# AssemblyAI-Community/MinImagen

Measured on AMD Instinct MI355X. Metric: denoising-steps/sec (images/sec x T), base 64^2 + SR 64->256 cascade, higher is better.
Workload: dtype f32; 1 GPU; cascade64_256: unet_0 params @64x64 + unet_1 params (lowres_cond) @256x256, T=100/stage, cond_scale=3.0 (2 U-Net evals/step), dynamic thresholding 0.9, fp32 storage / accumulate / softmax / statistics, contractions as 3-term fp16-split (hi*hi + hi*lo + lo*hi) MFMA products; per_gpu_batch=32, global_batch=32, parallelism=dp1

## Files before the change

include/minimagen_hip.h:

```cpp
#ifndef MINIMAGEN_HIP_H
#define MINIMAGEN_HIP_H

#include <stdint.h>

#ifdef __cplusplus
extern "C" {
#endif

#define MI_ABI_VERSION 12

enum mi_status {
    MI_OK = 0,
    MI_ERR_INVALID = -1,
    MI_ERR_LAUNCH = -2,
    MI_ERR_UNSUPPORTED = -3
};

int mi_abi_version(void);
const char* mi_last_error(void);
const char* mi_backend(void);
int mi_struct_size(int which);

typedef struct mi_act {
    const float* data;
    int C;
    const double* stats;
    int nt;
    float scale;
    int bmod;
    int st;
} mi_act;

typedef struct mi_conv_params {
    int B, H, W;
    mi_act in0, in1;
    int Cout;
    int ksize, stride, up2;
    const float* w;
    const float* bias;
    int gn_groups;
    const float* gn_gamma;
    const float* gn_beta;
    float gn_eps;
    const float* scale_shift;
    int ss_stride, ss_off;
    mi_act res0, res1;
    const float* res_w;
    const float* res_b;
    float* out;
    int out_st;
    double* out_stats;
    int tile_cfg;
    const void* w_rp;
    const void* res_w_rp;
    int w_rp_exp, res_w_rp_exp;
    float* gn_coef;
    int* gn_exps;
    void* act_prep; long long act_prep_bytes;
} mi_conv_params;
#define MI_CONV_SPLIT16 0x100
#define MI_CONV_SPLIT8  0x800
#define MI_CONV_HALF    0x400
#define MI_CONV_REVERSE 0x200
#define MI_CONV_RP_FIRST 6

int mi_conv_tile_shape(int tile_cfg, int* th, int* tw);
int mi_conv_stripe_rows(const mi_conv_params* p);
int mi_conv_prep_fwd(const mi_conv_params* p, void* stream);
long long mi_conv_prep_bytes(int B, int Cin, int Cres, int H, int W);
int mi_conv_cout_tile(int Cout);
int mi_conv_fwd(const mi_conv_params* p, void* stream);
int mi_gn_coef_fwd(const mi_conv_params* p, void* stream);

typedef struct mi_crossembed_params {
    int B, H, W;
    const float* in0; int C0;
    const float* in1; int C1;
    int in1_batch_mod;
    int in0_batch_mod;
    int n_kernels;
    int ksize[3];
    int cout[3];
    const float* w[3];
    const float* bias[3];
    float* out; double* out_stats;
    int out_st;
    int tile_cfg;
    const float* addend;
    const void* w_mfma;
    int w_mfma_exp[3];
} mi_crossembed_params;
int mi_crossembed_fwd(const mi_crossembed_params* p, void* stream);

typedef struct mi_init_down_params {
    int B, H, W;
    const float* in0; int C0;
    const float* in1; int C1;
    int in0_batch_mod;
    int n_kernels;
    int ksize[3];
    int cout[3];
    int Cout;
    const void* w_tab;
    int w_exp;
    const float* bias9;
    float* out; double* out_stats;
    int out_st;
    int tile_cfg;
    const float* addend;
} mi_init_down_params;
int mi_init_down_tiles(int tile_cfg, int H, int W);
int mi_init_down_fwd(const mi_init_down_params* p, void* stream);

typedef struct mi_linear {
    const float* w; const float* b; int in, out;
} mi_linear;

typedef struct mi_text_cond_params {
    int B2, B, L, E, cd, tcd, max_len;
    const float* text_embeds;
    const uint8_t* text_mask;
    const uint8_t* keep;
    mi_linear text_to_cond;
    const float* null_text_embed;
    const float* ln_w; const float* ln_b;
    mi_linear h1, h2;
    const float* null_text_hidden;
    const float* norm_w; const float* norm_b;
    float* c_text;
    float* text_hiddens;
} mi_text_cond_params;
int mi_text_cond_fwd(const mi_text_cond_params* p, void* stream);

typedef struct mi_cond_step_params {
    int B2, B, dim, cd, tcd, ntok;
    const int64_t* time;
    const int64_t* lowres_time;
    const float* freq;
    mi_linear th, tc, tt;
    mi_linear lth, ltc, ltt;
    const float* text_hiddens;
    const float* norm_w; const float* norm_b;
    mi_linear time_mlps;
    float* ss;
    float* c_time;
    float* t_out;
    float* silu_out;
} mi_cond_step_params;
int mi_cond_step_fwd(const mi_cond_step_params* p, void* stream);

#define MI_ATTN_MAX_BLOCKS 8
typedef struct mi_attn_fold_params {
    int B2, C, cd, heads, JT;
    const float* c_rows;
    int c_stride_b;
    int row0, nrows;
    int write_null;
    int frag_f16;
    int n_blocks;
    struct {
        const float* mg;
        const float* mv;
        const float* g0;
        const float* v0;
        float* gv;
        float* table;
        int g_exp, v_exp;
    } blk[MI_ATTN_MAX_BLOCKS];
    int mode;
    const int* t_state;
    int t_off;
    const float* ss_all; float* ss; int ss_n;
} mi_attn_fold_params;
int mi_attn_fold_rows(const mi_attn_fold_params* p, void* stream);
int mi_attn_fragment_floats(int C);

typedef struct mi_cross_attn_params {
    int B2, C, HW, heads, J;
    mi_act x;
    const float* gv;
    const float* n1_g; const float* n1_b;
    const float* n2_g; const float* n2_b;
    float* out; double* out_stats;
    int out_st;
    int x_exp, g_exp, v_exp;
    int variant;
    const float* head_tab;
} mi_cross_attn_params;
int mi_cross_attn_fwd(const mi_cross_attn_params* p, void* stream);

typedef struct mi_attn_cond_params {
    int B2, cd, JT;
    const float* c_rows;
    int c_stride_b;
    int row0, nrows;
    int write_null;
    int c_exp, i_exp;
    float* frag;
    const int* t_state; int t_off;
    const float* ss_all; float* ss; int ss_n;
} mi_attn_cond_params;
int mi_attn_cond_rows(const mi_attn_cond_params* p, void* stream);
int mi_attn_cond_frag_floats(int JT);
int mi_attn_cond_head_floats(void);
#define MI_ATTN_TOKENS_PER_WG 128

typedef struct mi_cfg_x0_params {
    int B, n;
    const float* pred2;
    int two;
    float cond_scale;
    const float* x_t;
    const float* coef; const int* t_state;
    float* pred_out;
    float* x0;
    unsigned* hist0;
    int t_off;
} mi_cfg_x0_params;
int mi_cfg_x0_fwd(const mi_cfg_x0_params* p, void* stream);

#define MI_Q_BINS 2048
typedef struct mi_quantile_params {
    int B, n;
    const float* x0;
    int k_lo, k_hi; float w;
    unsigned* hist;
    float* s_out;
    float* v_out;
    int pass0_done;
    int self_cleaning;
} mi_quantile_params;
int mi_quantile_fwd(const mi_quantile_params* p, void* stream);

typedef struct mi_posterior_params {
    int B, n, T;
    const float* x0; const float* s_q;
    float* x;
    const float* coef; const int* t_state;
    const float* noise;
    uint64_t seed; int sample0; int stream_base;
    const uint64_t* seed_dev;
    int t_off;
} mi_posterior_params;
int mi_posterior_fwd(const mi_posterior_params* p, void* stream);

#define MI_SAMPLER_SMALL_N 16384
int mi_sampler_step_small_fwd(const mi_cfg_x0_params* c, const mi_quantile_params* q, const mi_posterior_params* pp, void* stream);

int mi_sampler_group_size(int n);
long long mi_sampler_group_sync_bytes(int B, int n);
int mi_sampler_step_group_fwd(const mi_cfg_x0_params* c, const mi_quantile_params* q, const mi_posterior_params* pp, void* sync, void* stream);

int mi_step_advance(int* t_state, int64_t* times, int B, void* stream);
int mi_step_advance_by(int* t_state, int64_t* times, int B, int n, void* stream);
int mi_step_set(int* t_state, int64_t* times, int B, int value, void* stream);

typedef struct mi_sampler_ext_params {
    const int* t_map;
    float* x0_prev;
    long long reserved[2];
} mi_sampler_ext_params;
int mi_posterior_ext_fwd(const mi_posterior_params* p, const mi_sampler_ext_params* e, void* stream);
int mi_sampler_step_small_ext_fwd(const mi_cfg_x0_params* c, const mi_quantile_params* q, const mi_posterior_params* pp, const mi_sampler_ext_params* e, void* stream);
int mi_sampler_step_group_ext_fwd(const mi_cfg_x0_params* c, const mi_quantile_params* q, const mi_posterior_params* pp, const mi_sampler_ext_params* e, void* sync,
                                  void* stream);
int mi_step_set_mapped(int* t_state, int64_t* times, int B, int value, const mi_sampler_ext_params* e, void* stream);
int mi_step_advance_mapped(int* t_state, int64_t* times, int B, const mi_sampler_ext_params* e, void* stream);
int mi_step_advance_by_mapped(int* t_state, int64_t* times, int B, int n, const mi_sampler_ext_params* e, void* stream);

typedef struct mi_inpaint_params {
    const float* known;
    const unsigned char* mask;
    int hw;
    int known_stream;
    const float* known_noise;
    long long reserved[2];
} mi_inpaint_params;
int mi_posterior_inpaint_fwd(const mi_posterior_params* p, const mi_sampler_ext_params* e, const mi_inpaint_params* ip, void* stream);
int mi_sampler_step_small_inpaint_fwd(const mi_cfg_x0_params* c, const mi_quantile_params* q, const mi_posterior_params* pp, const mi_sampler_ext_params* e,
                                      const mi_inpaint_params* ip, void* stream);
int mi_sampler_step_group_inpaint_fwd(const mi_cfg_x0_params* c, const mi_quantile_params* q, const mi_posterior_params* pp, const mi_sampler_ext_params* e,
                                      const mi_inpaint_params* ip, void* sync, void* stream);
int mi_inpaint_blend0_fwd(float* x, int B, int n, const mi_inpaint_params* ip, float a, float b, uint64_t seed, int sample0, void* stream);
int mi_inpaint_prepare_fwd(const float* img, float* known, int B, int n, int normalize, const unsigned char* mask_in, int Hin, int Win, unsigned char* mask_out,
                           int size, void* stream);

int mi_randn_fill(float* out, int B, int n, uint64_t seed, int sample0, int stream_id, void* stream);

int mi_finalize_images(const float* x, float* out, int64_t total, int unnormalize, void* stream);

typedef struct mi_resize_params {
    int planes, Hin, Win, Hout, Wout, KH, KW;
    const float* in; float* out;
    const int* idx_h; const float* w_h;
    const int* idx_w; const float* w_w;
} mi_resize_params;
int mi_resize_fwd(const mi_resize_params* p, void* stream);

int mi_lowres_augment(const float* img, const float* noise, float* out, int64_t total, float a, float b, int normalize, void* stream);

int mi_ln_tokens_fwd(const mi_act* x, int B, int HW, const float* gamma, const float* beta, float* out, void* stream);
typedef struct mi_self_attn_params {
    int B2, C, HW, heads, J;
    mi_act x;
    const float* gv;
    const float* n1_g; const float* n1_b;
    const float* n2_g; const float* n2_b;
    float* out; double* out_stats;
} mi_self_attn_params;
int mi_self_attn_fwd(const mi_self_attn_params* p, void* stream);
typedef struct mi_chan_ff_params {
    int B, C, Chid, HW;
    mi_act x;
    const float* g1; const float* w1;
    const float* g2; const float* w2;
    float* out; double* out_stats;
} mi_chan_ff_params;
int mi_chan_ff_fwd(const mi_chan_ff_params* p, void* stream);

typedef struct mi_flash_attn_params {
    int B, HW, heads, kv_heads;
    const float* q; float q_scale;
    const float* null_k; const float* null_v;
    const float* k0; const float* v0; int n0, ld0; long long bs0;
    const float* k1; const float* v1; int n1, ld1; long long bs1;
    float* out;
    void* kv_prep; long long kv_prep_bytes;
} mi_flash_attn_params;
int mi_flash_attn_fwd(const mi_flash_attn_params* p, void* stream);
long long mi_flash_kv_prep_bytes(int B, int J);
typedef struct mi_tokens_to_nchw_params {
    int B, HW, C;
    const float* tokens;
    const float* gamma; const float* beta; float eps;
    mi_act res;
    float* out; double* out_stats;
} mi_tokens_to_nchw_params;
int mi_tokens_to_nchw_fwd(const mi_tokens_to_nchw_params* p, void* stream);
int mi_ln_rows_fwd(const float* x, const float* gamma, const float* beta, float* y, int rows, int dim, float eps, void* stream);

int mi_gemm_f32(const float* A, const float* W, const float* gate, const float* R, float* Cout, int M, int N, int K, int act, void* stream);
int mi_gemm_rms_f32(const float* A, const float* W, const float* gate, const float* R, float* Cout, int M, int N, int K, int act,
                    const float* rowsq_in, int nparts, float eps, float* rowsq_out, void* stream);
int mi_rmsnorm(const float* x, const float* w, float* y, int rows, int dim, float eps, const uint8_t* zero_mask, void* stream);
int mi_embed_rows(const int64_t* ids, const float* table, float* out, int rows, int dim, void* stream);
int mi_embed_rows_sq(const int64_t* ids, const float* table, float* out, float* rowsq, int nparts, int rows, int dim, void* stream);
// ... 162 lines not shown
```

minimagen_amd/_lib.py:

```python
from __future__ import annotations

import ctypes as C
import os

import torch

_HERE = os.path.dirname(os.path.abspath(__file__))
DEFAULT_LIB = os.environ.get("MINIMAGEN_HIP_LIB") or os.path.join(_HERE, "libminimagen_hip.so")

c_float_p = C.c_void_p


class MiAct(C.Structure):
    _fields_ = [("data", C.c_void_p), ("C", C.c_int), ("stats", C.c_void_p), ("nt", C.c_int), ("scale", C.c_float), ("bmod", C.c_int),
                ("st", C.c_int)]


class MiConvParams(C.Structure):
    _fields_ = [
        ("B", C.c_int), ("H", C.c_int), ("W", C.c_int),
        ("in0", MiAct), ("in1", MiAct),
        ("Cout", C.c_int), ("ksize", C.c_int), ("stride", C.c_int), ("up2", C.c_int),
        ("w", C.c_void_p), ("bias", C.c_void_p),
        ("gn_groups", C.c_int), ("gn_gamma", C.c_void_p), ("gn_beta", C.c_void_p), ("gn_eps", C.c_float),
        ("scale_shift", C.c_void_p), ("ss_stride", C.c_int), ("ss_off", C.c_int),
        ("res0", MiAct), ("res1", MiAct), ("res_w", C.c_void_p), ("res_b", C.c_void_p),
        ("out", C.c_void_p), ("out_st", C.c_int), ("out_stats", C.c_void_p), ("tile_cfg", C.c_int),
        ("w_rp", C.c_void_p), ("res_w_rp", C.c_void_p), ("w_rp_exp", C.c_int), ("res_w_rp_exp", C.c_int),
        ("gn_coef", C.c_void_p), ("gn_exps", C.c_void_p),
        ("act_prep", C.c_void_p), ("act_prep_bytes", C.c_longlong),
    ]


class MiCrossEmbedParams(C.Structure):
    _fields_ = [
        ("B", C.c_int), ("H", C.c_int), ("W", C.c_int),
        ("in0", C.c_void_p), ("C0", C.c_int), ("in1", C.c_void_p), ("C1", C.c_int),
        ("in1_batch_mod", C.c_int), ("in0_batch_mod", C.c_int), ("n_kernels", C.c_int),
        ("ksize", C.c_int * 3), ("cout", C.c_int * 3), ("w", C.c_void_p * 3), ("bias", C.c_void_p * 3),
        ("out", C.c_void_p), ("out_stats", C.c_void_p), ("out_st", C.c_int), ("tile_cfg", C.c_int), ("addend", C.c_void_p),
        ("w_mfma", C.c_void_p), ("w_mfma_exp", C.c_int * 3),
    ]


class MiInitDownParams(C.Structure):
    _fields_ = [
        ("B", C.c_int), ("H", C.c_int), ("W", C.c_int),
        ("in0", C.c_void_p), ("C0", C.c_int), ("in1", C.c_void_p), ("C1", C.c_int),
        ("in0_batch_mod", C.c_int), ("n_kernels", C.c_int), ("ksize", C.c_int * 3), ("cout", C.c_int * 3), ("Cout", C.c_int),
        ("w_tab", C.c_void_p), ("w_exp", C.c_int), ("bias9", C.c_void_p),
        ("out", C.c_void_p), ("out_stats", C.c_void_p), ("out_st", C.c_int), ("tile_cfg", C.c_int), ("addend", C.c_void_p),
    ]


class MiLinear(C.Structure):
    _fields_ = [("w", C.c_void_p), ("b", C.c_void_p), ("in_", C.c_int), ("out", C.c_int)]


class MiTextCondParams(C.Structure):
    _fields_ = [
        ("B2", C.c_int), ("B", C.c_int), ("L", C.c_int), ("E", C.c_int), ("cd", C.c_int), ("tcd", C.c_int), ("max_len", C.c_int),
        ("text_embeds", C.c_void_p), ("text_mask", C.c_void_p), ("keep", C.c_void_p),
        ("text_to_cond", MiLinear), ("null_text_embed", C.c_void_p), ("ln_w", C.c_void_p), ("ln_b", C.c_void_p),
        ("h1", MiLinear), ("h2", MiLinear), ("null_text_hidden", C.c_void_p), ("norm_w", C.c_void_p), ("norm_b", C.c_void_p),
        ("c_text", C.c_void_p), ("text_hiddens", C.c_void_p),
    ]


class MiCondStepParams(C.Structure):
    _fields_ = [
        ("B2", C.c_int), ("B", C.c_int), ("dim", C.c_int), ("cd", C.c_int), ("tcd", C.c_int), ("ntok", C.c_int),
        ("time", C.c_void_p), ("lowres_time", C.c_void_p), ("freq", C.c_void_p),
        ("th", MiLinear), ("tc", MiLinear), ("tt", MiLinear), ("lth", MiLinear), ("ltc", MiLinear), ("ltt", MiLinear),
        ("text_hiddens", C.c_void_p), ("norm_w", C.c_void_p), ("norm_b", C.c_void_p), ("time_mlps", MiLinear),
        ("ss", C.c_void_p), ("c_time", C.c_void_p), ("t_out", C.c_void_p), ("silu_out", C.c_void_p),
    ]


class MiAttnFoldBlk(C.Structure):
    _fields_ = [("mg", C.c_void_p), ("mv", C.c_void_p), ("g0", C.c_void_p), ("v0", C.c_void_p), ("gv", C.c_void_p), ("table", C.c_void_p),
                ("g_exp", C.c_int), ("v_exp", C.c_int)]


class MiAttnFoldParams(C.Structure):
    _fields_ = [
        ("B2", C.c_int), ("C", C.c_int), ("cd", C.c_int), ("heads", C.c_int), ("JT", C.c_int),
        ("c_rows", C.c_void_p), ("c_stride_b", C.c_int), ("row0", C.c_int), ("nrows", C.c_int), ("write_null", C.c_int), ("frag_f16", C.c_int),
        ("n_blocks", C.c_int), ("blk", MiAttnFoldBlk * 8),
        ("mode", C.c_int), ("t_state", C.c_void_p), ("t_off", C.c_int), ("ss_all", C.c_void_p), ("ss", C.c_void_p), ("ss_n", C.c_int),
    ]


class MiCrossAttnParams(C.Structure):
    _fields_ = [
        ("B2", C.c_int), ("C", C.c_int), ("HW", C.c_int), ("heads", C.c_int), ("J", C.c_int),
        ("x", MiAct), ("gv", C.c_void_p), ("n1_g", C.c_void_p), ("n1_b", C.c_void_p), ("n2_g", C.c_void_p), ("n2_b", C.c_void_p),
        ("out", C.c_void_p), ("out_stats", C.c_void_p), ("out_st", C.c_int), ("x_exp", C.c_int), ("g_exp", C.c_int), ("v_exp", C.c_int), ("variant", C.c_int),
        ("head_tab", C.c_void_p),
    ]


class MiAttnCondParams(C.Structure):
    _fields_ = [
        ("B2", C.c_int), ("cd", C.c_int), ("JT", C.c_int), ("c_rows", C.c_void_p), ("c_stride_b", C.c_int), ("row0", C.c_int), ("nrows", C.c_int),
        ("write_null", C.c_int), ("c_exp", C.c_int), ("i_exp", C.c_int), ("frag", C.c_void_p),
        ("t_state", C.c_void_p), ("t_off", C.c_int), ("ss_all", C.c_void_p), ("ss", C.c_void_p), ("ss_n", C.c_int),
    ]


class MiSelfAttnParams(C.Structure):
    _fields_ = [("B2", C.c_int), ("C", C.c_int), ("HW", C.c_int), ("heads", C.c_int), ("J", C.c_int), ("x", MiAct), ("gv", C.c_void_p),
                ("n1_g", C.c_void_p), ("n1_b", C.c_void_p), ("n2_g", C.c_void_p), ("n2_b", C.c_void_p), ("out", C.c_void_p), ("out_stats", C.c_void_p)]


class MiChanFFParams(C.Structure):
    _fields_ = [("B", C.c_int), ("C", C.c_int), ("Chid", C.c_int), ("HW", C.c_int), ("x", MiAct), ("g1", C.c_void_p), ("w1", C.c_void_p),
                ("g2", C.c_void_p), ("w2", C.c_void_p), ("out", C.c_void_p), ("out_stats", C.c_void_p)]


class MiFlashAttnParams(C.Structure):
    _fields_ = [("B", C.c_int), ("HW", C.c_int), ("heads", C.c_int), ("kv_heads", C.c_int), ("q", C.c_void_p), ("q_scale", C.c_float),
                ("null_k", C.c_void_p), ("null_v", C.c_void_p),
                ("k0", C.c_void_p), ("v0", C.c_void_p), ("n0", C.c_int), ("ld0", C.c_int), ("bs0", C.c_longlong),
                ("k1", C.c_void_p), ("v1", C.c_void_p), ("n1", C.c_int), ("ld1", C.c_int), ("bs1", C.c_longlong), ("out", C.c_void_p),
                ("kv_prep", C.c_void_p), ("kv_prep_bytes", C.c_longlong)]


class MiTokensToNchwParams(C.Structure):
    _fields_ = [("B", C.c_int), ("HW", C.c_int), ("C", C.c_int), ("tokens", C.c_void_p), ("gamma", C.c_void_p), ("beta", C.c_void_p),
                ("eps", C.c_float), ("res", MiAct), ("out", C.c_void_p), ("out_stats", C.c_void_p)]


class MiCfgX0Params(C.Structure):
    _fields_ = [("B", C.c_int), ("n", C.c_int), ("pred2", C.c_void_p), ("two", C.c_int), ("cond_scale", C.c_float),
                ("x_t", C.c_void_p), ("coef", C.c_void_p), ("t_state", C.c_void_p), ("pred_out", C.c_void_p), ("x0", C.c_void_p),
                ("hist0", C.c_void_p), ("t_off", C.c_int)]


class MiQuantileParams(C.Structure):
    _fields_ = [("B", C.c_int), ("n", C.c_int), ("x0", C.c_void_p), ("k_lo", C.c_int), ("k_hi", C.c_int), ("w", C.c_float),
                ("hist", C.c_void_p), ("s_out", C.c_void_p), ("v_out", C.c_void_p), ("pass0_done", C.c_int), ("self_cleaning", C.c_int)]


class MiPosteriorParams(C.Structure):
    _fields_ = [("B", C.c_int), ("n", C.c_int), ("T", C.c_int), ("x0", C.c_void_p), ("s_q", C.c_void_p), ("x", C.c_void_p),
                ("coef", C.c_void_p), ("t_state", C.c_void_p), ("noise", C.c_void_p),
                ("seed", C.c_uint64), ("sample0", C.c_int), ("stream_base", C.c_int), ("seed_dev", C.c_void_p), ("t_off", C.c_int)]


class MiSamplerExtParams(C.Structure):
    _fields_ = [("t_map", C.c_void_p), ("x0_prev", C.c_void_p), ("reserved", C.c_longlong * 2)]


class MiInpaintParams(C.Structure):
    _fields_ = [("known", C.c_void_p), ("mask", C.c_void_p), ("hw", C.c_int), ("known_stream", C.c_int), ("known_noise", C.c_void_p),
                ("reserved", C.c_longlong * 2)]


class MiResizeParams(C.Structure):
    _fields_ = [("planes", C.c_int), ("Hin", C.c_int), ("Win", C.c_int), ("Hout", C.c_int), ("Wout", C.c_int), ("KH", C.c_int), ("KW", C.c_int),
                ("in_", C.c_void_p), ("out", C.c_void_p), ("idx_h", C.c_void_p), ("w_h", C.c_void_p), ("idx_w", C.c_void_p), ("w_w", C.c_void_p)]


class MiConvWgradParams(C.Structure):
    _fields_ = [("B", C.c_int), ("Cin", C.c_int), ("Cout", C.c_int), ("H", C.c_int), ("W", C.c_int), ("a", C.c_void_p), ("dy", C.c_void_p),
                ("dw", C.c_void_p), ("db", C.c_void_p), ("partial", C.c_void_p), ("nwg", C.c_int),
                ("a_stats", C.c_void_p), ("a_nt", C.c_int), ("gamma", C.c_void_p), ("beta", C.c_void_p), ("groups", C.c_int), ("eps", C.c_float),
                ("ss", C.c_void_p), ("ss_stride", C.c_int), ("ss_off", C.c_int)]


class MiBlockBwdParams(C.Structure):
    _fields_ = [("B", C.c_int), ("C", C.c_int), ("HW", C.c_int), ("groups", C.c_int), ("nt", C.c_int), ("nchunk", C.c_int), ("eps", C.c_float),
                ("x", C.c_void_p), ("da", C.c_void_p), ("x_stats", C.c_void_p), ("gamma", C.c_void_p), ("beta", C.c_void_p),
                ("ss", C.c_void_p), ("ss_stride", C.c_int), ("ss_off", C.c_int), ("uv", C.c_void_p), ("dx", C.c_void_p),
                ("dgamma", C.c_void_p), ("dbeta", C.c_void_p), ("dss", C.c_void_p), ("dx_stats", C.c_void_p)]


class MiCrossEmbedWgradParams(C.Structure):
    _fields_ = [("B", C.c_int), ("Cin", C.c_int), ("H", C.c_int), ("W", C.c_int), ("x", C.c_void_p), ("dy", C.c_void_p),
                ("n_kernels", C.c_int), ("ksize", C.c_int * 3), ("cout", C.c_int * 3), ("dw", C.c_void_p * 3), ("db", C.c_void_p * 3),
                ("partial", C.c_void_p), ("nwg", C.c_int)]


class MiFoldedAttnParams(C.Structure):
    _fields_ = [("B", C.c_int), ("n", C.c_int), ("H", C.c_int), ("J", C.c_int), ("C", C.c_int), ("nchunk", C.c_int), ("q", C.c_void_p),
                ("kf", C.c_void_p), ("vf", C.c_void_p), ("mask", C.c_void_p), ("out", C.c_void_p), ("lse", C.c_void_p), ("dout", C.c_void_p),
                ("dsum", C.c_void_p), ("dq", C.c_void_p), ("dkf", C.c_void_p), ("dvf", C.c_void_p), ("oh", C.c_void_p)]


class MiFlashAttnTrainParams(C.Structure):
    _fields_ = [("B", C.c_int), ("n", C.c_int), ("heads", C.c_int), ("kv_heads", C.c_int), ("J", C.c_int), ("q", C.c_void_p), ("q_scale", C.c_float),
                ("k", C.c_void_p), ("v", C.c_void_p), ("mask", C.c_void_p), ("out", C.c_void_p), ("lse", C.c_void_p), ("dout", C.c_void_p),
                ("dq", C.c_void_p), ("dk", C.c_void_p), ("dv", C.c_void_p), ("work", C.c_void_p), ("work_bytes", C.c_longlong)]


class MiAdamTensor(C.Structure):
    _fields_ = [("p", C.c_void_p), ("g", C.c_void_p), ("m", C.c_void_p), ("v", C.c_void_p), ("n", C.c_longlong)]


class MiAdamParams(C.Structure):
    _fields_ = [("tensors", C.c_void_p), ("chunk_tensor", C.c_void_p), ("chunk_off", C.c_void_p), ("nchunks", C.c_int), ("chunk", C.c_int),
                ("lr", C.c_float), ("beta1", C.c_float), ("beta2", C.c_float), ("eps", C.c_float), ("weight_decay", C.c_float),
                ("bias_correction1", C.c_float), ("bias_correction2", C.c_float), ("one_minus_beta1", C.c_float), ("one_minus_beta2", C.c_float),
                ("grad_scale", C.c_void_p)]


class MiEmaTensor(C.Structure):
    _fields_ = [("e", C.c_void_p), ("p", C.c_void_p), ("n", C.c_longlong)]


class MiEmaParams(C.Structure):
    _fields_ = [("tensors", C.c_void_p), ("chunk_tensor", C.c_void_p), ("chunk_off", C.c_void_p), ("nchunks", C.c_int), ("chunk", C.c_int),
                ("w", C.c_float), ("reserved", C.c_int)]


class MiDiffuseParams(C.Structure):
    _fields_ = [("B", C.c_int), ("n", C.c_int), ("T", C.c_int), ("normalize", C.c_int), ("target_kind", C.c_int),
                ("x", C.c_void_p), ("noise", C.c_void_p), ("times", C.c_void_p), ("table", C.c_void_p), ("x_t", C.c_void_p), ("target", C.c_void_p),
                ("reserved", C.c_longlong * 2)]


class MiObjectiveLossParams(C.Structure):
    _fields_ = [("B", C.c_int), ("n", C.c_int), ("loss_type", C.c_int), ("T", C.c_int),
                ("pred", C.c_void_p), ("target", C.c_void_p), ("times", C.c_void_p), ("weights", C.c_void_p), ("partials", C.c_void_p),
                ("loss", C.c_void_p), ("grad", C.c_void_p), ("reserved", C.c_longlong * 2)]


class MiPackConv3Desc(C.Structure):
    _fields_ = [("w", C.c_void_p), ("frag", C.c_void_p), ("generic", C.c_void_p), ("Cout", C.c_int), ("Cin", C.c_int), ("adjoint", C.c_int),
                ("exp", C.c_int), ("cout_pad", C.c_int), ("reserved", C.c_int)]


_STRUCTS = {0: MiAct, 1: MiConvParams, 2: MiCrossEmbedParams, 3: MiLinear, 4: MiTextCondParams, 5: MiCondStepParams,
            6: MiAttnFoldParams, 7: MiCrossAttnParams, 8: MiCfgX0Params, 9: MiQuantileParams, 10: MiPosteriorParams,
            11: MiResizeParams, 12: MiSelfAttnParams, 13: MiChanFFParams, 14: MiFlashAttnParams, 15: MiTokensToNchwParams, 16: MiConvWgradParams, 17: MiBlockBwdParams, 18: MiCrossEmbedWgradParams, 19: MiFoldedAttnParams, 20: MiAdamTensor, 21: MiAdamParams, 22: MiPackConv3Desc,
            23: MiFlashAttnTrainParams, 24: MiSamplerExtParams, 25: MiInpaintParams, 26: MiInitDownParams, 27: MiAttnCondParams,
            28: MiEmaTensor, 29: MiEmaParams, 31: MiDiffuseParams, 32: MiObjectiveLossParams}

_lib = None
_backend = None


class MinImagenHipError(RuntimeError):
    pass


def _bind(lib):
    lib.mi_abi_version.restype = C.c_int
    lib.mi_last_error.restype = C.c_char_p
    lib.mi_backend.restype = C.c_char_p
    lib.mi_struct_size.argtypes = [C.c_int]
    vp, i32, i64, u64, f32 = C.c_void_p, C.c_int, C.c_int64, C.c_uint64, C.c_float
    for name in ("mi_conv_fwd", "mi_gn_coef_fwd", "mi_crossembed_fwd", "mi_text_cond_fwd", "mi_cond_step_fwd", "mi_attn_fold_rows", "mi_cross_attn_fwd",
                 "mi_cfg_x0_fwd", "mi_quantile_fwd", "mi_posterior_fwd", "mi_resize_fwd", "mi_self_attn_fwd", "mi_chan_ff_fwd",
                 "mi_flash_attn_fwd", "mi_conv_prep_fwd", "mi_tokens_to_nchw_fwd", "mi_conv_wgrad", "mi_block_bwd", "mi_crossembed_wgrad", "mi_folded_attn_fwd", "mi_folded_attn_bwd", "mi_adam_step",
                 "mi_flash_attn_train_fwd", "mi_flash_attn_train_bwd", "mi_init_down_fwd", "mi_attn_cond_rows", "mi_ema_update", "mi_ema_swap"):
        getattr(lib, name).argtypes = [vp, vp]
        getattr(lib, name).restype = i32
    lib.mi_adam_ema_step.argtypes = [vp, vp, vp]
    lib.mi_adam_ema_step.restype = i32
    lib.mi_grad_sumsq.argtypes = [vp, vp, vp]
    lib.mi_grad_clip_coef.argtypes = [vp, C.c_longlong, vp, f32, vp, vp]
    lib.mi_grad_scale.argtypes = [vp, vp]
    for name in ("mi_grad_sumsq", "mi_grad_clip_coef", "mi_grad_scale"):
        getattr(lib, name).restype = i32
    lib.mi_diffuse_fwd.argtypes = [vp, vp]
    lib.mi_objective_loss_fwd.argtypes = [vp, vp]
    lib.mi_objective_loss_bwd.argtypes = [vp, vp, vp, C.c_longlong, vp]
    lib.mi_objective_chunks.argtypes = [i32]
    for name in ("mi_diffuse_fwd", "mi_objective_loss_fwd", "mi_objective_loss_bwd", "mi_objective_chunks"):
        getattr(lib, name).restype = i32
    lib.mi_conv_prep_bytes.argtypes = [i32, i32, i32, i32, i32]
    lib.mi_conv_prep_bytes.restype = C.c_longlong
    lib.mi_flash_kv_prep_bytes.argtypes = [i32, i32]
    lib.mi_flash_kv_prep_bytes.restype = C.c_longlong
    lib.mi_flash_attn_train_workspace.argtypes = [i32, i32, i32, i32, i32, i32]
    lib.mi_flash_attn_train_workspace.restype = C.c_longlong
    lib.mi_step_advance.argtypes = [vp, vp, i32, vp]
    lib.mi_step_advance_by.argtypes = [vp, vp, i32, i32, vp]
    lib.mi_sampler_step_small_fwd.argtypes = [vp, vp, vp, vp]
    lib.mi_sampler_step_small_fwd.restype = i32
    lib.mi_sampler_step_group_fwd.argtypes = [vp, vp, vp, vp, vp]
    lib.mi_sampler_step_group_fwd.restype = i32
    lib.mi_sampler_group_size.argtypes = [i32]
    lib.mi_sampler_group_sync_bytes.argtypes = [i32, i32]
    lib.mi_sampler_group_sync_bytes.restype = C.c_longlong
    lib.mi_step_set.argtypes = [vp, vp, i32, i32, vp]
    lib.mi_posterior_ext_fwd.argtypes = [vp, vp, vp]
    lib.mi_sampler_step_small_ext_fwd.argtypes = [vp, vp, vp, vp, vp]
    lib.mi_sampler_step_group_ext_fwd.argtypes = [vp, vp, vp, vp, vp, vp]
    lib.mi_step_set_mapped.argtypes = [vp, vp, i32, i32, vp, vp]
    lib.mi_step_advance_mapped.argtypes = [vp, vp, i32, vp, vp]
    lib.mi_step_advance_by_mapped.argtypes = [vp, vp, i32, i32, vp, vp]
    lib.mi_posterior_inpaint_fwd.argtypes = [vp, vp, vp, vp]
    lib.mi_sampler_step_small_inpaint_fwd.argtypes = [vp, vp, vp, vp, vp, vp]
    lib.mi_sampler_step_group_inpaint_fwd.argtypes = [vp, vp, vp, vp, vp, vp, vp]
    lib.mi_inpaint_blend0_fwd.argtypes = [vp, i32, i32, vp, f32, f32, u64, i32, vp]
    lib.mi_inpaint_prepare_fwd.argtypes = [vp, vp, i32, i32, i32, vp, i32, i32, vp, i32, vp]
    lib.mi_randn_fill.argtypes = [vp, i32, i32, u64, i32, i32, vp]
    lib.mi_finalize_images.argtypes = [vp, vp, i64, i32, vp]
    lib.mi_lowres_augment.argtypes = [vp, vp, vp, i64, f32, f32, i32, vp]
    lib.mi_gemm_f32.argtypes = [vp, vp, vp, vp, vp, i32, i32, i32, i32, vp]
    lib.mi_rmsnorm.argtypes = [vp, vp, vp, i32, i32, f32, vp, vp]
    lib.mi_embed_rows.argtypes = [vp, vp, vp, i32, i32, vp]
    lib.mi_embed_rows_sq.argtypes = [vp, vp, vp, vp, i32, i32, i32, vp]
    lib.mi_gemm_rms_f32.argtypes = [vp, vp, vp, vp, vp, i32, i32, i32, i32, vp, i32, f32, vp, vp]
    lib.mi_t5_attention.argtypes = [vp, vp, vp, vp, i32, i32, i32, vp]
    lib.mi_ln_tokens_fwd.argtypes = [vp, i32, i32, vp, vp, vp, vp]
    lib.mi_ln_rows_fwd.argtypes = [vp, vp, vp, vp, i32, i32, f32, vp]
    lib.mi_graph_begin.argtypes = [vp]
    lib.mi_graph_end.argtypes = [vp, C.POINTER(vp)]
    lib.mi_graph_launch.argtypes = [vp, vp]
    lib.mi_graph_destroy.argtypes = [vp]
    lib.mi_conv_tile_shape.argtypes = [i32, C.POINTER(i32), C.POINTER(i32)]
    lib.mi_conv_stripe_rows.argtypes = [vp]
    lib.mi_conv_stripe_rows.restype = i32
    lib.mi_conv_cout_tile.argtypes = [i32]
    lib.mi_init_down_tiles.argtypes = [i32, i32, i32]
    lib.mi_init_down_tiles.restype = i32
    lib.mi_conv_wgrad_workspace.argtypes = [i32, i32, i32]
    lib.mi_conv_wgrad_workspace.restype = C.c_longlong
    lib.mi_crossembed_wgrad_workspace.argtypes = [i32, i32, i32]
    lib.mi_crossembed_wgrad_workspace.restype = C.c_longlong
    lib.mi_chan_stats_fwd.argtypes = [vp, vp, i32, i32, vp]
    lib.mi_layernorm_fwd.argtypes = [vp, vp, vp, vp, vp, i32, i32, C.c_float, vp]
    lib.mi_layernorm_bwd_nwg.argtypes = [i32, i32]
    lib.mi_layernorm_bwd_nwg.restype = i32
# ... 70 lines not shown
```

minimagen_amd/csrc/conv.hip:

```cpp
#include "common.hip.h"

#ifdef MI_TRACE
__device__ unsigned long long mi_trace_conv_buf[1024 * 8];
extern "C" int mi_debug_read_trace_conv(void* dst, size_t bytes) { return (int)hipMemcpyFromSymbol(dst, HIP_SYMBOL(mi_trace_conv_buf), bytes); }
#define MI_TSTART() unsigned long long mi_t_last = clock64(), mi_t_acc[8] = {0, 0, 0, 0, 0, 0, 0, 0}
#define MI_TPHASE(k) do { const unsigned long long mi_t_now = clock64(); mi_t_acc[k] += mi_t_now - mi_t_last; mi_t_last = mi_t_now; } while (0)
#define MI_TEND() do { if (threadIdx.x == 0) { const int wg = blockIdx.y * gridDim.x + blockIdx.x; if (wg < 1024) for (int k = 0; k < 8; ++k) mi_trace_conv_buf[wg * 8 + k] = mi_t_acc[k]; } } while (0)
#else
#define MI_TSTART() do { } while (0)
#define MI_TPHASE(k) do { } while (0)
#define MI_TEND() do { } while (0)
#endif

namespace {

template <int NT_, int TW_, int COUT_T_, int KS_, int S_, bool UP2_, bool VEC_, bool GN_>
struct ConvCfg {
    static constexpr int NT = NT_, TW = TW_, COUT_T = COUT_T_, KS = KS_, S = S_;
    static constexpr bool UP2 = UP2_, VEC = VEC_, GN = GN_;
    static constexpr int TXN = TW / 4;
    static constexpr int TH = NT / TXN;
    static constexpr int IH = TH * S + KS - S;
    static constexpr int IW = TW * S + KS - S;
    static constexpr int SW = UP2_ ? TW_ / 2 + 8 : TW_ * S_ + 8;
// ... 94 lines not shown
                    } else {
                        o[e] = xe[e] * P.x;
                    }
                }
                if constexpr (S == 2) {
                    if (mdst[u] >= 0) {
                        *reinterpret_cast<float2*>(&smem[mdst[u] + 2]) = make_float2(o[0], o[2]);
                        smem[mdst[u] + CFG::PE + 3] = o[1];
                        smem[mdst[u] + CFG::PE + 4] = o[3];
                    }
                } else {
                    if (mdst[u] >= 0) *reinterpret_cast<float4*>(&smem[mdst[u]]) = make_float4(o[0], o[1], o[2], o[3]);
                }
            }
        } else {
            constexpr int TOT = CK * IH * IW, U = 8;
#pragma unroll 1
            for (int it = 0; it < TOT; it += U * NT) {
                float xs[U];
#pragma unroll
                for (int u = 0; u < U; ++u) {
                    const int idx = it + tid + u * NT;
                    const int ix = idx % IW, r = idx / IW;
                    const int iy = r % IH, ck = r / IH;
                    const int c = c0 + ck;
                    const int gy = iy0 + iy, gx = ix0 + ix;
                    const bool inimg = idx < TOT && c < Cin && gy >= 0 && gy < Hv && gx >= 0 && gx < Wv;
                    const int sy = UP2 ? (gy >> 1) : gy, sx = UP2 ? (gx >> 1) : gx;
                    const bool second = inimg && c >= C0;
                    const float* base = second ? p.in1.data : p.in0.data;
                    const int cc = second ? (b1 * C1 + (c - C0)) : (b0 * C0 + c);
                    const unsigned off = inimg ? (unsigned)((cc * Hin + sy) * Win + sx) : 0u;
                    xs[u] = mi_ldg(base + off);
                }
#pragma unroll
                for (int u = 0; u < U; ++u) {
                    const int idx = it + tid + u * NT;
                    const int ix = idx % IW, r = idx / IW;
                    const int iy = r % IH, ck = r / IH;
                    const int c = c0 + ck;
                    const int gy = iy0 + iy, gx = ix0 + ix;
                    const bool inimg = idx < TOT && c < Cin && gy >= 0 && gy < Hv && gx >= 0 && gx < Wv;
                    float v = 0.0f;
                    if (inimg) { const float4 P = chP[c]; v = gn ? mi_silu(fmaf(xs[u], P.x, P.y)) : xs[u] * P.x; }
                    if (idx < TOT) smem[(ck * IH + iy) * IWP + ix] = v;
                }
            }
        }
    };

    MI_TPHASE(0);
    stage_load(0);
    MI_TPHASE(1);

    if constexpr (CFG::GN) {
        __syncthreads();
        const int cpg = Cin / p.gn_groups;
        for (int g = tid; g < p.gn_groups; g += NT)
            mi_gn_group_moments(chS, chQ, g * cpg, (g + 1) * cpg, (double)cpg * (double)Hin * (double)Win, p.gn_eps, gMean[g], gRstd[g]);
        __syncthreads();
        for (int c = tid; c < Cin; c += NT) {
            const int g = c / cpg;
            float A = gRstd[g] * p.gn_gamma[c];
            float Bc = p.gn_beta[c] - gMean[g] * A;
            if (p.scale_shift) {
                const float* ss = p.scale_shift + (size_t)b * p.ss_stride + p.ss_off;
                const float sc = ss[c] + 1.0f, sh = ss[Cin + c];
                A *= sc;
                Bc = Bc * sc + sh;
            }
            if (c >= C0) A *= p.in1.scale; else A *= p.in0.scale;
            chP[c] = make_float4(A, Bc, A * -1.44269504088896340736f, Bc * -1.44269504088896340736f);
        }
    } else {
        for (int c = tid; c < Cin; c += NT) chP[c] = make_float4((c >= C0) ? p.in1.scale : p.in0.scale, 0.0f, 0.0f, 0.0f);
    }
    if (tid == 0) chP[MI_MAX_CIN] = make_float4(0.0f, 0.0f, 0.0f, 0.0f);

    for (int c0 = 0; c0 < Cin; c0 += CK) {
        MI_TPHASE(c0 == 0 ? 2 : 5);
        __syncthreads();
        MI_TPHASE(3);
        stage_write(c0);
        MI_TPHASE(4);
        __syncthreads();
        MI_TPHASE(3);
        if (c0 + CK < Cin) stage_load(c0 + CK);
        MI_TPHASE(1);
        const int nck = (Cin - c0) < CK ? (Cin - c0) : CK;
        for (int ck = 0; ck < nck; ++ck) {
            const float* wc = wts + (size_t)(c0 + ck) * KS * KS * CoutPad + co0;
#pragma unroll
            for (int ky = 0; ky < KS; ++ky) {
                float in[NIN];
                if constexpr (VEC && UP2) {
                    const float* row = &smem[(ck * IHS + ((ty + ky - 1) >> 1) + 1) * IWP + 2 * tx + 3];
                    const float s0 = row[0];
                    const float2 s12 = *reinterpret_cast<const float2*>(row + 1);
                    const float s3 = row[3];
                    in[0] = s0; in[1] = s12.x; in[2] = s12.x; in[3] = s12.y; in[4] = s12.y; in[5] = s3;
                } else if constexpr (VEC && S == 2) {
                    const float* rowE = &smem[(ck * IHS + ty * 2 + ky) * IWP + 4 * tx + 4];
                    const float* rowO = rowE + CFG::PE;
                    const float4 e4 = *reinterpret_cast<const float4*>(rowE), o4 = *reinterpret_cast<const float4*>(rowO);
                    in[0] = o4.x; in[1] = e4.x; in[2] = o4.y; in[3] = e4.y; in[4] = o4.z; in[5] = e4.z; in[6] = o4.w; in[7] = e4.w;
                    in[8] = rowO[4];
                    in[9] = rowE[4];
                } else if constexpr (VEC) {
                    const float* row = &smem[(ck * IHS + ty + ky) * IWP + tx * 4 + XOFF];
                    in[0] = row[0];
                    const float4 m4 = *reinterpret_cast<const float4*>(row + 1);
                    in[1] = m4.x; in[2] = m4.y; in[3] = m4.z; in[4] = m4.w;
                    in[5] = row[5];
                } else {
                    const float* row = &smem[(ck * IH + ty * S + ky) * IWP + tx * 4 * S];
#pragma unroll
                    for (int j = 0; j < NIN; ++j) in[j] = row[j];
                }
#pragma unroll
                for (int kx = 0; kx < KS; ++kx) {
                    const float* wk = wc + (ky * KS + kx) * CoutPad;
                    float wv[COUT_T];
#pragma unroll
                    for (int co = 0; co < COUT_T; ++co) wv[co] = wk[co];
#pragma unroll
                    for (int px = 0; px < 4; ++px)
#pragma unroll
                        for (int co = 0; co < COUT_T; ++co) acc[px][co] = fmaf(in[px * S + kx], wv[co], acc[px][co]);
                }
            }
        }
    }

    MI_TPHASE(5);
    const int oy = oy0 + ty, ox = ox0 + tx * 4;
    const bool row_ok = oy < p.H;
    const int Cres0 = p.res0.data ? p.res0.C : 0, Cres1 = (p.res0.data && p.res1.data) ? p.res1.C : 0;
#pragma unroll
    for (int co = 0; co < COUT_T; ++co) {
        const float bv = (p.bias && (co0 + co) < p.Cout) ? p.bias[co0 + co] : 0.0f;
#pragma unroll
        for (int px = 0; px < 4; ++px) acc[px][co] += bv;
    }
    if (p.res0.data && row_ok) {
        if (p.res_w) {
            for (int cr = 0; cr < Cres0 + Cres1; ++cr) {
                const bool second = cr >= Cres0;
                const float* src = second ? p.res1.data + ((size_t)(br1 * Cres1 + (cr - Cres0)) * p.H + oy) * p.W
                                          : p.res0.data + ((size_t)(br0 * Cres0 + cr) * p.H + oy) * p.W;
                const float sc = second ? p.res1.scale : p.res0.scale;
                float rv[4];
                if (ox + 3 < p.W && (p.W & 3) == 0) {
                    const float4 t4 = mi_ldg4(src + ox);
                    rv[0] = t4.x * sc; rv[1] = t4.y * sc; rv[2] = t4.z * sc; rv[3] = t4.w * sc;
                } else {
#pragma unroll
                    for (int px = 0; px < 4; ++px) rv[px] = (ox + px < p.W) ? mi_ldg(src + ox + px) * sc : 0.0f;
                }
                const float* wr = res_wts + (size_t)cr * CoutPad + co0;
#pragma unroll
                for (int co = 0; co < COUT_T; ++co) {
                    const float wv = wr[co];
#pragma unroll
                    for (int px = 0; px < 4; ++px) acc[px][co] = fmaf(rv[px], wv, acc[px][co]);
                }
            }
#pragma unroll
            for (int co = 0; co < COUT_T; ++co) {
                const float bv = (p.res_b && (co0 + co) < p.Cout) ? p.res_b[co0 + co] : 0.0f;
#pragma unroll
                for (int px = 0; px < 4; ++px) acc[px][co] += bv;
            }
        } else {
#pragma unroll
            for (int co = 0; co < COUT_T; ++co) {
                if (co0 + co < p.Cout) {
                    const float* src = p.res0.data + ((size_t)(br0 * Cres0 + co0 + co) * p.H + oy) * p.W;
                    if (ox + 3 < p.W && (p.W & 3) == 0) {
                        const float4 t4 = mi_ldg4(src + ox);
                        acc[0][co] += t4.x * p.res0.scale; acc[1][co] += t4.y * p.res0.scale;
                        acc[2][co] += t4.z * p.res0.scale; acc[3][co] += t4.w * p.res0.scale;
                    } else {
#pragma unroll
                        for (int px = 0; px < 4; ++px)
                            if (ox + px < p.W) acc[px][co] += mi_ldg(src + ox + px) * p.res0.scale;
                    }
                }
            }
        }
    }
    double ssum[COUT_T], ssq[COUT_T];
#pragma unroll
    for (int co = 0; co < COUT_T; ++co) {
        double s = 0.0, q = 0.0;
        if (row_ok && (co0 + co) < p.Cout) {
            float* dst = p.out + ((size_t)(b * p.Cout + co0 + co) * p.H + oy) * p.W + ox;
            if (ox + 3 < p.W && (p.W & 3) == 0) {
                mi_stg4(dst, make_float4(acc[0][co], acc[1][co], acc[2][co], acc[3][co]));
#pragma unroll
                for (int px = 0; px < 4; ++px) { const double v = (double)acc[px][co]; s += v; q = fma(v, v, q); }
            } else {
#pragma unroll
                for (int px = 0; px < 4; ++px)
                    if (ox + px < p.W) { mi_stg(dst + px, acc[px][co]); const double v = (double)acc[px][co]; s += v; q = fma(v, v, q); }
            }
        }
        ssum[co] = s;
        ssq[co] = q;
    }
    if (p.out_stats) {
        static_assert(NT % 64 == 0 && 2 * COUT_T <= NT, "statistics reduction: whole waves");
        constexpr int NW = NT / 64;
        static_assert(2 * COUT_T * NW * 2 <= CFG::SMEM_FLOATS, "statistics staging fits the tile buffer");
        __syncthreads();
        double* const redd = reinterpret_cast<double*>(smem);
#pragma unroll
        for (int co = 0; co < COUT_T; ++co) {
            double s = ssum[co], q = ssq[co];
#pragma unroll
            for (int o = 32; o > 0; o >>= 1) { s += __shfl_xor(s, o); q += __shfl_xor(q, o); }
            if ((tid & 63) == 0) { redd[(2 * co) * NW + (tid >> 6)] = s; redd[(2 * co + 1) * NW + (tid >> 6)] = q; }
        }
        __syncthreads();
        if (tid < 2 * COUT_T) {
            double a = 0.0;
            for (int w = 0; w < NW; ++w) a += redd[tid * NW + w];
            const int co = co0 + (tid >> 1);
            if (co < p.Cout) {
                const int nt = gridDim.x;
                p.out_stats[((size_t)(b * p.Cout + co) * nt + tile) * 2 + (tid & 1)] = a;
            }
        }
    }
    MI_TPHASE(6);
    MI_TEND();
}

template <int NT, int TW, int COUT_T, int KS, int S, bool UP2, bool VEC, bool GN>
int launch_conv_g(const mi_conv_params& p, hipStream_t st) {
    using CFG = ConvCfg<NT, TW, COUT_T, KS, S, UP2, VEC, GN>;
    const int tiles = ((p.H + CFG::TH - 1) / CFG::TH) * ((p.W + TW - 1) / TW);
    const int cz = (p.Cout + COUT_T - 1) / COUT_T;
    hipLaunchKernelGGL(HIP_KERNEL_NAME(conv_tile_kernel<CFG>), dim3(tiles, p.B, cz), dim3(NT), 0, st, p, cz * COUT_T, p.w, p.res_w);
    return mi_check_launch("conv_tile_kernel");
}

template <int NT, int TW, int COUT_T, int KS, int S, bool UP2, bool VEC>
int launch_conv_v(const mi_conv_params& p, hipStream_t st) {
    if constexpr (KS == 3 && S == 1 && !UP2) {
        if (p.gn_groups > 0) return launch_conv_g<NT, TW, COUT_T, KS, S, UP2, VEC, true>(p, st);
    } else {
        if (p.gn_groups > 0) { mi_set_error("mi_conv_fwd: GroupNorm prologue is only built for the k3 s1 family"); return MI_ERR_UNSUPPORTED; }
    }
    return launch_conv_g<NT, TW, COUT_T, KS, S, UP2, VEC, false>(p, st);
}

template <int NT, int TW, int COUT_T, int KS, int S, bool UP2>
int launch_conv(const mi_conv_params& p, hipStream_t st) {
    const int Cin = p.in0.C + (p.in1.data ? p.in1.C : 0);
    const int Win = UP2 ? p.W / 2 : p.W * S;
    constexpr int CKv = (S == 2) ? 2 : 4;
    if ((Win & 3) == 0 && (Cin % CKv) == 0 && (p.in0.C % CKv) == 0 &&
        (size_t)p.B * (p.in0.C > p.in1.C ? p.in0.C : p.in1.C) * p.H * p.W * S * S < (1ull << 31))
        return launch_conv_v<NT, TW, COUT_T, KS, S, UP2, true>(p, st);
    return launch_conv_v<NT, TW, COUT_T, KS, S, UP2, false>(p, st);
}

template <int COUT_T, int KS, int S, bool UP2>
int dispatch_tile(const mi_conv_params& p, hipStream_t st) {
    switch (p.tile_cfg & 0xff) {
        case 0: return launch_conv<256, 64, COUT_T, KS, S, UP2>(p, st);
        case 1: return launch_conv<256, 32, COUT_T, KS, S, UP2>(p, st);
        case 2: return launch_conv<64, 32, COUT_T, KS, S, UP2>(p, st);
    }
    mi_set_error("mi_conv_fwd: bad tile_cfg %d", p.tile_cfg);
    return MI_ERR_INVALID;
}

}

extern "C" int mi_conv_tile_shape(int tile_cfg, int* th, int* tw) {
    switch (tile_cfg & 0xff) {
        case 6: *th = 8; *tw = 64; return MI_OK;
        case 7: *th = 8; *tw = 32; return MI_OK;
        case 10: *th = 16; *tw = 16; return MI_OK;
        case 11: *th = 8; *tw = 16; return MI_OK;
        case 0: *th = 16; *tw = 64; return MI_OK;
        case 1: *th = 32; *tw = 32; return MI_OK;
        case 2: *th = 8; *tw = 32; return MI_OK;
        case 8: *th = 32; *tw = 64; return MI_OK;
        case 9: *th = 16; *tw = 32; return MI_OK;
    }
    return MI_ERR_INVALID;
}

extern "C" int mi_conv_cout_tile(int Cout) { return Cout <= 4 ? 4 : (Cout % 16 == 0 ? 16 : 8); }

extern "C" int mi_conv_fwd(const mi_conv_params* pp, void* stream) {
    const mi_conv_params& p = *pp;
    hipStream_t st = (hipStream_t)stream;
    const int Cin = p.in0.C + (p.in1.data ? p.in1.C : 0);
    const bool any16 = p.in0.st || (p.in1.data && p.in1.st) || (p.res0.data && p.res0.st) || (p.res1.data && p.res1.st) || p.out_st;
    if (any16 && !(p.w_rp && (p.tile_cfg & 0x400))) { mi_set_error("mi_conv_fwd: bf16 activation storage is read / written by the single-term row-paired kernels only (w_rp, tile_cfg | 0x400)"); return MI_ERR_UNSUPPORTED; }
    if (p.w_rp) {
        if (p.gn_groups > MI_MAX_GROUPS || (p.gn_groups > 0 && (Cin % p.gn_groups) != 0)) { mi_set_error("mi_conv_fwd: Cin %d / groups %d", Cin, p.gn_groups); return MI_ERR_INVALID; }
        if (p.gn_groups > 0 && (!p.in0.stats || (p.in1.data && !p.in1.stats))) { mi_set_error("mi_conv_fwd: GroupNorm input without channel statistics"); return MI_ERR_INVALID; }
        if (p.res0.data && !p.res_w && p.res0.C != p.Cout) { mi_set_error("mi_conv_fwd: identity residual needs Cres == Cout"); return MI_ERR_INVALID; }
        if (p.B <= 0 || p.H <= 0 || p.W <= 0 || p.Cout <= 0) { mi_set_error("mi_conv_fwd: empty problem"); return MI_ERR_INVALID; }
        if ((p.tile_cfg & 0xff) == 11) return mi_conv_wide_launch(p, st);
        if ((p.tile_cfg & 0xff) == 12) return mi_conv_stripe_launch(p, st);
        return mi_conv_rp_launch(p, st);
    }
    if (Cin > MI_MAX_CIN || p.gn_groups > MI_MAX_GROUPS) { mi_set_error("mi_conv_fwd: Cin %d / groups %d too large for the direct-conv family", Cin, p.gn_groups); return MI_ERR_UNSUPPORTED; }
    if (p.gn_groups > 0 && (Cin % p.gn_groups) != 0) { mi_set_error("mi_conv_fwd: Cin %d not divisible by groups %d", Cin, p.gn_groups); return MI_ERR_INVALID; }
    if (p.gn_groups > 0 && (!p.in0.stats || (p.in1.data && !p.in1.stats))) { mi_set_error("mi_conv_fwd: GroupNorm input without channel statistics"); return MI_ERR_INVALID; }
    if (p.res0.data && !p.res_w && p.res0.C != p.Cout) { mi_set_error("mi_conv_fwd: identity residual needs Cres == Cout"); return MI_ERR_INVALID; }
    if (p.B <= 0 || p.H <= 0 || p.W <= 0 || p.Cout <= 0) { mi_set_error("mi_conv_fwd: empty problem"); return MI_ERR_INVALID; }
    if (p.up2 && ((p.H | p.W) & 1)) { mi_set_error("mi_conv_fwd: up2 needs even output size"); return MI_ERR_INVALID; }
    const int ct = mi_conv_cout_tile(p.Cout);
    const bool split8 = (p.tile_cfg & MI_CONV_SPLIT8) && ct == 8 && p.Cout == 8;
    if (p.ksize == 3 && p.stride == 1 && !p.up2) {
        if (ct == 4 || split8) return dispatch_tile<4, 3, 1, false>(p, st);
        if (ct == 8 || (p.tile_cfg & MI_CONV_SPLIT16)) return dispatch_tile<8, 3, 1, false>(p, st);
        return dispatch_tile<16, 3, 1, false>(p, st);
    }
    if (p.ksize == 3 && p.stride == 1 && p.up2) {
        if (ct == 16) return dispatch_tile<16, 3, 1, true>(p, st);
        if (ct == 8 && !split8) return dispatch_tile<8, 3, 1, true>(p, st);
        return dispatch_tile<4, 3, 1, true>(p, st);
    }
    if (p.ksize == 4 && p.stride == 2 && !p.up2) {
        if (ct == 16) return dispatch_tile<8, 4, 2, false>(p, st);
        if (ct == 8 && !split8) return dispatch_tile<8, 4, 2, false>(p, st);
        return dispatch_tile<4, 4, 2, false>(p, st);
    }
    mi_set_error("mi_conv_fwd: unsupported conv k%d s%d up%d", p.ksize, p.stride, p.up2);
    return MI_ERR_UNSUPPORTED;
}
```

minimagen_amd/csrc/conv_stripe.hip:

```cpp
#include "rp_common.hip.h"

#ifdef ST_TRACE
__device__ unsigned long long mi_trace_st_buf[1024 * 32];
extern "C" int mi_debug_read_trace_st(void* dst, size_t bytes) { return (int)hipMemcpyFromSymbol(dst, HIP_SYMBOL(mi_trace_st_buf), bytes); }
#define ST_STAMP(k) do { if (lane == 0 && blockIdx.x < 1024) mi_trace_st_buf[blockIdx.x * 32 + (k)] = clock64(); } while (0)
#else
#define ST_STAMP(k) do { } while (0)
#endif

#ifndef ST_ABL
#define ST_ABL 0
#endif
#ifndef ST_BREG
#define ST_BREG 1
#endif
#ifndef ST_HALF_OCTETS
#define ST_HALF_OCTETS 1
#endif
#ifndef ST_NB_HS
#define ST_NB_HS 2
#endif
#ifndef ST_LDG2
#define ST_LDG2 1
#endif
#ifndef ST_LOOKAHEAD
#define ST_LOOKAHEAD 2
#endif
#ifndef ST_RO4
#define ST_RO4 1
#endif
#ifndef ST_LOADER_DELAY
#define ST_LOADER_DELAY 56
#endif

namespace {

template <int W_, int KO_, int NJ_, bool GN_, int OM_, int RO_ = 0>
struct StCfg {
    static constexpr int W = W_, KO = KO_, NJ = NJ_, OM = OM_, RO = RO_;
    static constexpr bool GN = GN_;
    static constexpr bool UP = OM_ == 3, DS = OM_ == 4;
    static constexpr int NTAP = DS ? 4 : 3, NCO = DS ? 16 : 8, OPS = DS ? 1 : 2;
    static constexpr int WS = DS ? 2 * W_ : (UP ? W_ / 2 : W_), RPS = UP ? 1 : 2, NPR = UP ? 3 : 4;
    static constexpr bool HS = W_ < 256 && ST_HALF_OCTETS;
    static constexpr int NCH = HS ? 4 : 8;
    static constexpr int NB = (HS && W_ >= 64) ? ST_NB_HS : 2;
    static constexpr int QPR = WS / 4, UNITS = RPS * QPR * KO * (HS ? 2 : 1), NLWC = (UNITS + 63) / 64;
    static constexpr int LA = W_ <= 128 ? ((NJ_ == 2 && KO_ == 2 && OM_ == 1 && ST_LOOKAHEAD > 1) ? 1 : ST_LOOKAHEAD) : 0;
    static constexpr int LDG = (ST_LDG2 && GN_ && RO_ == 0 && W_ >= 64 && W_ <= 128 && NLWC <= 2) ? 2 : 1;
    static constexpr int NLC = NLWC * LDG;
    static constexpr int UNITS_R = 2 * QPR * RO, NLWR = (UNITS_R + 63) / 64, NLW = NLC + NLWR;
    static constexpr int NG = W_ / 16, NCW = NG >= 4 ? 4 : NG, GPW = NG / NCW;
    static constexpr int NT = (NLW + NCW) * 64;
    static constexpr int PWH = WS / 2 + 2;
    static constexpr int PW = DS ? 2 * PWH : WS + 8, RING = 6, RINGR = 4, PLANE = (KO * RING + RO * RINGR) * PW;
    static constexpr int SR0 = W_ / 8;
    static constexpr int WCH = NTAP * NJ * 128, WTOT = KO * WCH + RO * NJ * 128;
    static constexpr bool BREG = ST_BREG && KO == 1 && NJ == 1 && RO == 0 && !DS && !(LDG == 2 && OM_ == 1);
    static_assert(RO == 0 || (OM_ == 0 && GN_), "a 1x1 residual conv comes with a Block and replaces the identity residual");
    static constexpr int WPE = ((RO > 0 && W_ == 128) || LDG == 2) ? 4 : 1;
    static constexpr bool PHS = HS && 2 * NPR * QPR * KO <= NCW * 64;
    static constexpr int PCH = PHS ? 4 : 8, PU = NPR * QPR * KO * (PHS ? 2 : 1);
    static_assert(PU <= NCW * 64, "the MFMA waves transform the first four rows in one pass");
    static_assert(!DS || (LA > 0 && !GN_ && RO_ == 0 && W_ <= 128), "the stride-2 member is a plain conv, at most 128 output columns");
};

__device__ __forceinline__ bool st_totals_issue(const mi_act& in0, const mi_act& in1, int C0, int Cin, int b, int lane, int nlanes, bool have, mi_stats_regs& r) {
    int TPC = 1;
    while (TPC < 64 && TPC * 2 * Cin <= nlanes) TPC *= 2;
    const int nt_max = (Cin > C0 && in1.nt > in0.nt) ? in1.nt : in0.nt;
    const bool covers = have && TPC * Cin <= nlanes && nt_max <= MI_STATS_K * TPC;
    const int c = lane / TPC, sub = lane % TPC;
    const bool live = covers && c < Cin;
    const bool second = live && c >= C0;
    const int cc = live ? (second ? c - C0 : c) : 0;
    const int nt = second ? in1.nt : in0.nt, CC = second ? in1.C : in0.C;
    const double* sp = second ? in1.stats : in0.stats;
    const int ba = mi_row_of(b, second ? in1.bmod : in0.bmod);
    const mi_gptr<const double> st = live ? mi_global(sp) + ((size_t)(ba * CC + cc) * nt) * 2 : mi_global(reinterpret_cast<const double*>(in0.data));
#pragma unroll
    for (int k = 0; k < MI_STATS_K; ++k) {
        const int t = sub + k * TPC;
        const bool ok = live && t < nt;
        const double x = st[2 * (ok ? t : 0)], y = st[2 * (ok ? t : 0) + 1];
        r.v[k] = make_double2(ok ? x : 0.0, ok ? y : 0.0);
    }
    r.c = live ? c : -1;
    r.tpc = TPC;
    r.scale = second ? in1.scale : in0.scale;
    return covers;
}

template <class CFG>
__global__ __launch_bounds__(CFG::NT, CFG::WPE) void conv_stripe_kernel(const mi_conv_params p, const uint4* __restrict__ wrp, const uint4* __restrict__ rwrp, const int nblk) {
    constexpr int W = CFG::W, KO = CFG::KO, NJ = CFG::NJ, QPR = CFG::QPR, UNITS = CFG::UNITS, NLT = CFG::NLW, NLWC = CFG::NLWC, NLC = CFG::NLC, LDG = CFG::LDG, RO = CFG::RO, RINGR = CFG::RINGR;
    constexpr int NCW = CFG::NCW, GPW = CFG::GPW, PW = CFG::PW, RING = CFG::RING, SR0 = CFG::SR0, WCH = CFG::WCH, WTOT = CFG::WTOT, PU = CFG::PU;
    constexpr bool GN = CFG::GN, BREG = CFG::BREG, UP = CFG::UP, DS = CFG::DS;
    constexpr int NTAP = CFG::NTAP, NCO = CFG::NCO, OPS = CFG::OPS, PWH = CFG::PWH;
    constexpr int WS = CFG::WS, RPS = CFG::RPS, NPR = CFG::NPR;
    __shared__ __attribute__((aligned(16))) uint4 actH[CFG::PLANE];
    __shared__ __attribute__((aligned(16))) uint4 actL[CFG::PLANE];
    __shared__ __attribute__((aligned(16))) uint4 wl[BREG ? 1 : WTOT];
    __shared__ __attribute__((aligned(16))) float4 chP[RP_MAXC];
    __shared__ double chS[RP_MAXC], chQ[RP_MAXC], chS2[RO ? RP_MAXC : 1], chQ2[RO ? RP_MAXC : 1];
    __shared__ double red[NCW][2 * NCO * NJ];
    __shared__ int sExp[4];

    const int tid = threadIdx.x, wave = tid >> 6, lane = tid & 63, lq = lane & 15, lg = lane >> 4;
    const int H = p.H, HW = H * W;
    const int Hs = UP ? H / 2 : (DS ? 2 * H : H), HWs = UP ? HW / 4 : (DS ? 4 * HW : HW);
    const int nt = H / SR0;
    const int wgs = nt / nblk;
    int b, sidx;
    if ((p.B & 7) == 0 && !(ST_ABL & 1)) {
        const int L = blockIdx.x;
        int k = L >> 3;
        if (p.tile_cfg & MI_CONV_REVERSE) k = (int)(gridDim.x >> 3) - 1 - k;
        b = (L & 7) + 8 * (k / wgs);
        sidx = k % wgs;
    } else {
        b = blockIdx.x / wgs;
        sidx = blockIdx.x % wgs;
    }
    const int blk0 = sidx * nblk, y0 = blk0 * SR0, RS = nblk * SR0, NSTEP = RS / OPS;
    const int ys0 = UP ? y0 / 2 : (DS ? 2 * y0 : y0);
    const int C0 = p.in0.C, C1 = p.in1.data ? p.in1.C : 0, Cin = C0 + C1;
    const bool have_stats = !(ST_ABL & 4) && (GN || p.in0.stats != nullptr);
    const int Cr0 = RO ? p.res0.C : 0, Cr1 = (RO && p.res1.data) ? p.res1.C : 0, Cres = Cr0 + Cr1;
    const bool res_stats = RO > 0 && p.res0.stats != nullptr && (Cr1 == 0 || p.res1.stats != nullptr);
    const float* const img0 = p.in0.data + (size_t)mi_row_of(b, p.in0.bmod) * C0 * HWs;
    const float* const img1 = C1 ? p.in1.data + (size_t)mi_row_of(b, p.in1.bmod) * C1 * HWs : img0;
    auto octet_base = [&](int oct) {
        const int c0 = 8 * oct;
        const float* a0 = img0 + (size_t)c0 * HWs;
        const float* a1 = img1 + (size_t)(c0 - C0) * HWs;
        return mi_global(c0 >= C0 ? a1 : a0);
    };
    auto transform_quad = [&](auto nc_tag, const f32x4* raw, const float4* P, bool inimg, bool live, int oct, int half, int slot, int q) {
        constexpr int NC = decltype(nc_tag)::value;
#pragma unroll
        for (int px = 0; px < 4; ++px) {
            float y[NC];
#pragma unroll
            for (int j = 0; j < NC; ++j) {
                const float x = raw[j][px];
                if constexpr (GN) {
                    const float a = fmaf(x, P[j].x, P[j].y);
                    const float ex = __builtin_amdgcn_exp2f(fmaf(x, P[j].z, P[j].w));
                    y[j] = a * __builtin_amdgcn_rcpf(1.0f + ex);
                } else {
                    y[j] = x * P[j].x;
                }
            }
            unsigned h[NC / 2], l[NC / 2];
#pragma unroll
            for (int i = 0; i < NC / 2; ++i) {
                const rp_f32x2 v = {y[2 * i], y[2 * i + 1]};
                h[i] = __builtin_bit_cast(unsigned, __builtin_convertvector(v, rp_f16x2));
                l[i] = mi_split_lo2(h[i], y[2 * i], y[2 * i + 1]);
            }
            if (!inimg) {
#pragma unroll
                for (int i = 0; i < NC / 2; ++i) { h[i] = 0u; l[i] = 0u; }
            }
            if (live) {
                const int idx = (oct * RING + slot) * PW + (DS ? (px & 1) * PWH + 2 * q + (px >> 1) + 1 : 1 + 4 * q + px);
                if constexpr (NC == 8) {
                    actH[idx] = make_uint4(h[0], h[1], h[2], h[3]);
                    actL[idx] = make_uint4(l[0], l[1], l[2], l[3]);
                } else {
                    reinterpret_cast<uint2*>(&actH[idx])[half] = make_uint2(h[0], h[1]);
                    reinterpret_cast<uint2*>(&actL[idx])[half] = make_uint2(l[0], l[1]);
                }
            }
        }
    };

    if (RO > 0 && wave >= NLC && wave < NLT) {
        const int u = (wave - NLC) * 64 + lane;
        const bool live = u < CFG::UNITS_R;
        const int uu = live ? u : 0;
        const int oct = uu / (2 * QPR), lrow = (uu / QPR) & 1, q = uu % QPR;
        const float* const rimg0 = p.res0.data + (size_t)mi_row_of(b, p.res0.bmod) * Cr0 * HW;
        const float* const rimg1 = Cr1 ? p.res1.data + (size_t)mi_row_of(b, p.res1.bmod) * Cr1 * HW : rimg0;
        const bool second = 8 * oct >= Cr0;
        const mi_gptr<const float> base = mi_global(second ? rimg1 + (size_t)(8 * oct - Cr0) * HW : rimg0 + (size_t)(8 * oct) * HW);
        f32x4 raw[2][8];
        auto issue = [&](int s, auto buf_tag) {
            constexpr int buf = decltype(buf_tag)::value;
            const int y = y0 + 2 * (s < NSTEP ? s : NSTEP - 1) + lrow;
            const unsigned off = (unsigned)(y * W + 4 * q);
#pragma unroll
            for (int j = 0; j < 8; ++j) raw[buf][j] = *reinterpret_cast<mi_gptr<const f32x4>>(base + (size_t)j * HW + off);
        };
        constexpr std::integral_constant<int, 0> B0{};
        constexpr std::integral_constant<int, 1> B1{};
        {
            mi_stats_regs sr2;
            const int rt = (wave - NLC) * 64 + lane;
            const bool fast2 = st_totals_issue(p.res0, p.res1, Cr0, Cres, b, rt, CFG::NLWR * 64, res_stats, sr2);
            if (fast2) mi_gn_totals_finish(sr2, rt, chS2, chQ2);
            else if (res_stats) mi_gn_channel_totals(p.res0, p.res1, Cr0, Cres, b, rt, CFG::NLWR * 64, chS2, chQ2);
        }
        issue(0, B0);
        issue(1, B1);
        if (have_stats) __syncthreads();
        __syncthreads();
        const float rsc = ldexpf(second ? p.res1.scale : p.res0.scale, sExp[1]);
        uint4* const dstH = &actH[(KO * RING + oct * RINGR + lrow) * PW + 1 + 4 * q];
        uint4* const dstL = &actL[(KO * RING + oct * RINGR + lrow) * PW + 1 + 4 * q];
        auto transform = [&](auto buf_tag) {
            constexpr int buf = decltype(buf_tag)::value;
#pragma unroll
            for (int px = 0; px < 4; ++px) {
                float y[8];
#pragma unroll
                for (int j = 0; j < 8; ++j) y[j] = raw[buf][j][px] * rsc;
                uint4 hv, lv;
                rp_split8(y, hv, lv);
                if (live) { dstH[2 * buf * PW + px] = hv; dstL[2 * buf * PW + px] = lv; }
            }
        };
        transform(B0);
        issue(2, B0);
        __syncthreads();
        for (int it = 0; it < NSTEP; it += 2) {
            transform(B1);
            issue(it + 3, B1);
            __syncthreads();
            transform(B0);
            issue(it + 4, B0);
            __syncthreads();
        }
    } else if (wave < NLT) {
        constexpr int NCH = CFG::NCH, HSM = CFG::HS ? 2 : 1;
        const int grp = LDG > 1 ? wave / NLWC : 0;
        const int u = (wave - grp * NLWC) * 64 + lane;
        const bool live = u < UNITS;
        const int uu = live ? u : 0;
        const int oct = uu / (RPS * QPR * HSM), half = HSM == 2 ? (uu / (RPS * QPR)) & 1 : 0, lrow = RPS == 2 ? (uu / QPR) & 1 : 0, q = uu % QPR;
        const mi_gptr<const float> base = octet_base(oct) + (size_t)(NCH * half) * HWs;
        constexpr int NB = CFG::NB;
        f32x4 raw[NB][NCH];
        bool inimg[NB];
        auto issue = [&](int s, auto buf_tag) {
            constexpr int buf = decltype(buf_tag)::value;
            int y = UP ? ys0 + s + 1 : ys0 + 2 * s + 1 + lrow;
            const int ylast = UP ? (y0 + RS) / 2 : (DS ? 2 * (y0 + RS) : y0 + RS);
            y = y > ylast ? ylast : y;
            const bool ok = y < Hs;
            inimg[buf] = ok;
            const unsigned off = ok ? (unsigned)(y * WS + 4 * q) : 0u;
#pragma unroll
            for (int j = 0; j < NCH; ++j) raw[buf][j] = *reinterpret_cast<mi_gptr<const f32x4>>(base + (size_t)j * HWs + off);
        };
        float4 P[NCH];
        auto transform = [&](int s, auto buf_tag) {
            constexpr int buf = decltype(buf_tag)::value;
            transform_quad(std::integral_constant<int, NCH>{}, raw[buf], P, inimg[buf], live, oct, half, (UP ? s + 2 : 2 * s + 2 + lrow) % RING, q);
        };
        auto run = [&](auto grp_tag) {
            constexpr int g = decltype(grp_tag)::value;
            if (wave == 0) ST_STAMP(10);
#if ST_LOADER_DELAY && !defined(HIPEMU)
            if constexpr (W <= 128) __builtin_amdgcn_s_sleep(ST_LOADER_DELAY);
#endif
            rp_for_rounds(std::make_integer_sequence<int, NB>{}, [&](auto j) { issue(1 + g + LDG * decltype(j)::value, j); });
            if (wave == 0) ST_STAMP(11);
            if (have_stats) __syncthreads();
            __syncthreads();
            if (wave == 0) ST_STAMP(12);
#pragma unroll
            for (int j = 0; j < NCH; ++j) P[j] = chP[8 * oct + NCH * half + j];
            __syncthreads();
            if (wave == 0) ST_STAMP(14);
            for (int it = 0; it < NSTEP; it += NB * LDG) {
                rp_for_rounds(std::make_integer_sequence<int, NB * LDG>{}, [&](auto jh) {
                    constexpr int j = decltype(jh)::value / LDG, h = decltype(jh)::value % LDG;
                    if constexpr (h == g) {
                        const int t = it + j * LDG + h;
                        if (wave == 0 && t == 2) ST_STAMP(20);
                        transform(t + 1, std::integral_constant<int, j>{});
                        if (wave == 0 && t == 2) ST_STAMP(21);
                        issue(t + 1 + NB * LDG, std::integral_constant<int, j>{});
                        if (wave == 0 && t == 2) ST_STAMP(22);
                    }
                    __syncthreads();
                    if (wave == 0 && it + j * LDG + h == 2) ST_STAMP(23);
                });
            }
        };
        if (LDG == 1 || grp == 0) run(std::integral_constant<int, 0>{});
        else run(std::integral_constant<int, LDG - 1>{});
        if (wave == 0) ST_STAMP(15);
    } else {
        const int cw = wave - NLT, ct = tid - NLT * 64;
        constexpr int NCT = NCW * 64;
        if (cw == 0) ST_STAMP(0);
        mi_stats_regs sr;
        const bool fast = st_totals_issue(p.in0, p.in1, C0, Cin, b, ct, NCT, have_stats, sr);
        float pg = 0.f, pb = 0.f, ld_s1 = 0.f, ld_s2 = 0.f, ld_b[NJ], ld_rb[RO ? NJ : 1];
        if constexpr (GN) {
            const int c = lane < Cin ? lane : 0;
            pg = p.gn_gamma[c];
            pb = p.gn_beta[c];
            const float* ss = p.scale_shift ? p.scale_shift + (size_t)b * p.ss_stride + p.ss_off : p.gn_gamma;
            ld_s1 = ss[p.scale_shift ? c : 0];
            ld_s2 = ss[p.scale_shift ? Cin + c : 0];
        }
#pragma unroll
        for (int jt = 0; jt < NJ; ++jt) {
            const int co = NCO * jt + (DS ? lq : (lq & 7));
            const bool hb = p.bias != nullptr && co < p.Cout;
            ld_b[jt] = (hb ? p.bias : p.in0.data)[hb ? co : 0];
            if constexpr (RO > 0) { const bool hr = p.res_b != nullptr && co < p.Cout; ld_rb[jt] = (hr ? p.res_b : p.in0.data)[hr ? co : 0]; }
        }
        constexpr int WPER = BREG ? 1 : (WTOT + NCT - 1) / NCT;
        uint4 wreg[WPER];
        rp_f16x8 breg[BREG ? 6 : 1];
        if constexpr (BREG) {
#pragma unroll
            for (int k = 0; k < 6; ++k) breg[k] = __builtin_bit_cast(rp_f16x8, mi_ldg4u(wrp + 128 * (k >> 1) + 2 * lane + (k & 1)));
        } else {
#pragma unroll
            for (int i = 0; i < WPER; ++i) {
                const int k = ct + i * NCT;
                const int kc = k < WTOT ? k : 0;
                wreg[i] = (RO > 0 && kc >= KO * WCH) ? mi_ldg4u(rwrp + (kc - KO * WCH)) : mi_ldg4u(wrp + kc);
            }
        }
        constexpr int PCH = CFG::PCH, PHM = CFG::PHS ? 2 : 1;
        const bool plive = ct < PU;
        const int pu = plive ? ct : 0;
        const int poct = pu / (NPR * QPR * PHM), phalf = PHM == 2 ? (pu / (NPR * QPR)) & 1 : 0, prow = (pu / QPR) % NPR, pq = pu % QPR;
        f32x4 praw[PCH];
        const int py = ys0 - 1 + prow;
        const bool pin = py >= 0 && py < Hs;
        {
            const mi_gptr<const float> pbase = octet_base(poct) + (size_t)(PCH * phalf) * HWs;
            const unsigned off = pin ? (unsigned)(py * WS + 4 * pq) : 0u;
#pragma unroll
            for (int j = 0; j < PCH; ++j) praw[j] = *reinterpret_cast<mi_gptr<const f32x4>>(pbase + (size_t)j * HWs + off);
        }
        for (int k = ct; k < KO * RING * 2; k += NCT) {
            const int r = k >> 1, c = DS ? ((k & 1) ? WS / 2 + 1 : PWH) : ((k & 1) ? WS + 1 : 0);
            actH[r * PW + c] = make_uint4(0u, 0u, 0u, 0u);
            actL[r * PW + c] = make_uint4(0u, 0u, 0u, 0u);
        }
        double inv_n = 1.0;
        if constexpr (GN) inv_n = 1.0 / ((double)(Cin / p.gn_groups) * (double)HW);
        float psc = 1.0f, psh = 0.0f, An = 0.f, Bn = 0.f;
        int ka = 0;
        if constexpr (GN) {
            if (cw == 0) {
                psc = p.scale_shift ? ld_s1 + 1.0f : 1.0f;
                psh = p.scale_shift ? ld_s2 : 0.0f;
                float m = 0.f;
                if (lane < Cin) {
                    An = pg; Bn = pb;
                    if (p.scale_shift) { An *= psc; Bn = Bn * psc + psh; }
                    m = 4.0f * fabsf(An) + fabsf(Bn);
                }
                m = mi_wave_max(m);
                ka = (m > 0.f) ? rp_clamp_exp(4 - rp_exponent(m)) : 0;
            }
        }
        if constexpr (!BREG) {
#pragma unroll
            for (int i = 0; i < WPER; ++i) {
                const int k = ct + i * NCT;
                if (k < WTOT) wl[rp_wl_index(k)] = wreg[i];
            }
        }
        if (fast) mi_gn_totals_finish(sr, ct, chS, chQ);
        else if (have_stats) mi_gn_channel_totals(p.in0, p.in1, C0, Cin, b, ct, NCT, chS, chQ);
        if (cw == 0) ST_STAMP(1);
        if (have_stats) __syncthreads();
        if (cw == 0) ST_STAMP(2);
        int kr = 0, Eall = 0;
        if (cw == 0) {
            const int c = lane;
            if constexpr (RO > 0) {
                float mr = 4.0f;
                if (res_stats) {
                    double qq = (c < Cres) ? chQ2[c] : 0.0;
#pragma unroll
                    for (int o = 32; o > 0; o >>= 1) qq += __shfl_xor(qq, o);
                    mr = 4.0f * sqrtf((float)(qq / ((double)Cres * (double)HW)));
                }
                const int kr_max = (mr > 0.f) ? rp_clamp_exp(4 - rp_exponent(mr)) : 0;
                int E = ka + p.w_rp_exp;
                const int Er = kr_max + p.res_w_rp_exp;
                if (Er < E) E = Er;
                ka = E - p.w_rp_exp;
                kr = E - p.res_w_rp_exp;
                Eall = E;
            }
            if constexpr (GN) {
                if (c < Cin) {
                    const int cpg = Cin / p.gn_groups, g = c / cpg;
                    float mean, rstd;
                    if (ST_ABL & 4) { mean = 0.3f; rstd = 0.6f; }
                    else {
                        double gs = 0.0, gq = 0.0;
                        for (int cc = g * cpg; cc < (g + 1) * cpg; ++cc) { gs += chS[cc]; gq += chQ[cc]; }
                        const double mean_d = gs * inv_n;
                        double var = gq * inv_n - mean_d * mean_d;
                        var = var > 0.0 ? var : 0.0;
                        mean = (float)mean_d;
                        rstd = 1.0f / sqrtf((float)(var + (double)p.gn_eps));
                    }
                    float A = rstd * pg;
                    float Bc = pb - mean * A;
                    if (p.scale_shift) {
                        A *= psc;
                        Bc = Bc * psc + psh;
                    }
                    A *= (c >= C0) ? p.in1.scale : p.in0.scale;
                    chP[c] = make_float4(ldexpf(A, ka), ldexpf(Bc, ka), A * -1.44269504088896340736f, Bc * -1.44269504088896340736f);
                }
            } else {
                float m = 0.f;
                if (have_stats) {
                    double qq = (c < Cin) ? chQ[c] : 0.0;
#pragma unroll
                    for (int o = 32; o > 0; o >>= 1) qq += __shfl_xor(qq, o);
                    m = 4.0f * sqrtf((float)(qq / ((double)Cin * (double)HWs)));
                }
                ka = (m > 0.f) ? rp_clamp_exp(4 - rp_exponent(m)) : 0;
                if (c < Cin) chP[c] = make_float4(ldexpf((c >= C0) ? p.in1.scale : p.in0.scale, ka), 0.f, 0.f, 0.f);
            }
            if (lane == 0) { sExp[0] = ka; sExp[1] = kr; sExp[2] = RO > 0 ? Eall : ka + p.w_rp_exp; }
        }
        if (cw == 0) ST_STAMP(3);
        if (cw == 0) ST_STAMP(4);
        __syncthreads();
        if (cw == 0) ST_STAMP(5);
        {
            float4 PP[PCH];
#pragma unroll
            for (int j = 0; j < PCH; ++j) PP[j] = chP[8 * poct + PCH * phalf + j];
            transform_quad(std::integral_constant<int, PCH>{}, praw, PP, pin, plive, poct, phalf, prow, pq);
        }

        float bvv[NJ];
#pragma unroll
        for (int jt = 0; jt < NJ; ++jt) {
            const int cob = NCO * jt + (DS ? lq : (lq & 7));
            bvv[jt] = (p.bias != nullptr && cob < p.Cout) ? ld_b[jt] : 0.0f;
            if constexpr (RO > 0) bvv[jt] += (p.res_b != nullptr && cob < p.Cout) ? ld_rb[jt] : 0.0f;
        }
        const int perm = ((lg & 1) << 1) | (lg >> 1);
        const int dy = DS ? 0 : lq >> 3;
        constexpr bool idres = CFG::OM == 1, MASKC = CFG::OM == 2 || DS;
        const mi_gptr<float> obuf = mi_global(p.out + (size_t)b * p.Cout * HW);
        const mi_gptr<const float> rbuf = mi_global(idres ? p.res0.data + (size_t)mi_row_of(b, p.res0.bmod) * p.res0.C * HW : p.out);
        const float unscale = ldexpf(1.0f, -sExp[2]);
        const float rs = idres ? p.res0.scale : 0.0f;
        f32x4 rv[2][idres ? GPW : 1][idres ? NJ : 1];
        auto issue_res = [&](int it, auto buf_tag) {
            constexpr int buf = decltype(buf_tag)::value;
            if constexpr (idres) {
                const int itc = it < NSTEP ? it : NSTEP - 1;
#pragma unroll
                for (int g = 0; g < GPW; ++g)
#pragma unroll
                    for (int jt = 0; jt < NJ; ++jt) {
                        const int co = 8 * jt + (lq & 7);
                        const int oy = y0 + 2 * itc + dy, ox = 16 * (cw * GPW + g) + 4 * lg;
                        rv[buf][g][jt] = *reinterpret_cast<mi_gptr<const f32x4>>(rbuf + (unsigned)(co * HW + oy * W + ox));
                    }
            }
        };
        float csum[NJ], csq[NJ], cshift[NJ];
        auto compute = [&](int it, auto buf_tag, bool first_of_block) {
            constexpr int buf = decltype(buf_tag)::value;
            f32x4 acc[GPW][NJ];
#pragma unroll
            for (int g = 0; g < GPW; ++g)
#pragma unroll
                for (int jt = 0; jt < NJ; ++jt) acc[g][jt] = (f32x4){0.f, 0.f, 0.f, 0.f};
            if (cw == 0 && it == 2) ST_STAMP(16);
            const int slot = (UP ? it + 1 + ((perm - 1) >> 1) : (DS ? 2 * it + lg : 2 * it + perm)) % RING;
            if constexpr (CFG::LA > 0) {
                constexpr int LA = CFG::LA, NS = NTAP * KO + RO, NBUF = LA + 1;
                rp_f16x8 sah[NBUF][GPW], sal[NBUF][GPW], sbh[NBUF][NJ], sbl[NBUF][NJ];
                const int rslot = RO > 0 ? 2 * (it & 1) + (perm >> 1) : 0;
                auto load = [&](auto st_tag) {
                    constexpr int st = decltype(st_tag)::value, bi = st % NBUF;
                    if constexpr (st < NTAP * KO) {
                        constexpr int o = st / NTAP, t = st % NTAP;
                        if constexpr (!BREG) {
#pragma unroll
                            for (int jt = 0; jt < NJ; ++jt) {
                                sbh[bi][jt] = __builtin_bit_cast(rp_f16x8, wl[o * WCH + (t * NJ + jt) * 128 + lane]);
                                sbl[bi][jt] = __builtin_bit_cast(rp_f16x8, wl[o * WCH + (t * NJ + jt) * 128 + 64 + lane]);
                            }
                        }
#pragma unroll
                        for (int g = 0; g < GPW; ++g) {
                            const int col = 16 * (cw * GPW + g) + lq + t;
                            const int idx = (o * RING + slot) * PW + (DS ? ((t + 1) & 1) * PWH + 16 * (cw * GPW + g) + lq + ((t + 1) >> 1) : (UP ? ((col - 1) >> 1) + 1 : col));
                            sah[bi][g] = __builtin_bit_cast(rp_f16x8, actH[idx]);
                            sal[bi][g] = __builtin_bit_cast(rp_f16x8, actL[idx]);
                        }
                    } else {
                        constexpr int o = st - NTAP * KO;
#pragma unroll
                        for (int jt = 0; jt < NJ; ++jt) {
                            sbh[bi][jt] = __builtin_bit_cast(rp_f16x8, wl[KO * WCH + (o * NJ + jt) * 128 + lane]);
                            sbl[bi][jt] = __builtin_bit_cast(rp_f16x8, wl[KO * WCH + (o * NJ + jt) * 128 + 64 + lane]);
                        }
#pragma unroll
                        for (int g = 0; g < GPW; ++g) {
                            const int idx = (KO * RING + o * RINGR + rslot) * PW + 16 * (cw * GPW + g) + lq + 1;
                            sah[bi][g] = __builtin_bit_cast(rp_f16x8, actH[idx]);
                            sal[bi][g] = __builtin_bit_cast(rp_f16x8, actL[idx]);
                        }
                    }
                };
                auto mult = [&](auto st_tag) {
                    constexpr int st = decltype(st_tag)::value, bi = st % NBUF;
                    rp_f16x8 bh[NJ], bl[NJ];
#pragma unroll
                    for (int jt = 0; jt < NJ; ++jt) {
                        if constexpr (BREG) { bh[jt] = breg[2 * (st % 3)]; bl[jt] = breg[2 * (st % 3) + 1]; }
                        else { bh[jt] = sbh[bi][jt]; bl[jt] = sbl[bi][jt]; }
                    }
#pragma unroll
                    for (int g = 0; g < GPW; ++g)
#pragma unroll
                        for (int jt = 0; jt < NJ; ++jt) acc[g][jt] = __builtin_amdgcn_mfma_f32_16x16x32_f16(sal[bi][g], bh[jt], acc[g][jt], 0, 0, 0);
#pragma unroll
                    for (int g = 0; g < GPW; ++g)
#pragma unroll
                        for (int jt = 0; jt < NJ; ++jt) acc[g][jt] = __builtin_amdgcn_mfma_f32_16x16x32_f16(sah[bi][g], bl[jt], acc[g][jt], 0, 0, 0);
#pragma unroll
                    for (int g = 0; g < GPW; ++g)
#pragma unroll
                        for (int jt = 0; jt < NJ; ++jt) acc[g][jt] = __builtin_amdgcn_mfma_f32_16x16x32_f16(sah[bi][g], bh[jt], acc[g][jt], 0, 0, 0);
                };
                rp_for_rounds(std::make_integer_sequence<int, (LA < NS ? LA : NS)>{}, load);
                rp_for_rounds(std::make_integer_sequence<int, NS>{}, [&](auto st_tag) {
                    constexpr int st = decltype(st_tag)::value;
                    if constexpr (st + LA < NS) load(std::integral_constant<int, st + LA>{});
                    __builtin_amdgcn_sched_barrier(0);
                    mult(st_tag);
                    __builtin_amdgcn_sched_barrier(0);
                });
            } else {
    #pragma unroll
                for (int o = 0; o < KO; ++o) {
    #pragma unroll
                    for (int s = 0; s < 3; ++s) {
                        rp_f16x8 bh[NJ], bl[NJ];
    #pragma unroll
                        for (int jt = 0; jt < NJ; ++jt) {
                            if constexpr (BREG) { bh[jt] = breg[2 * s]; bl[jt] = breg[2 * s + 1]; }
                            else {
                                bh[jt] = __builtin_bit_cast(rp_f16x8, wl[o * WCH + (s * NJ + jt) * 128 + lane]);
                                bl[jt] = __builtin_bit_cast(rp_f16x8, wl[o * WCH + (s * NJ + jt) * 128 + 64 + lane]);
                            }
                        }
    #pragma unroll
                        for (int g = 0; g < GPW; ++g) {
                            const int col = 16 * (cw * GPW + g) + lq + s;
                            const int idx = (o * RING + slot) * PW + (UP ? ((col - 1) >> 1) + 1 : col);
                            const rp_f16x8 ah = __builtin_bit_cast(rp_f16x8, actH[idx]);
                            const rp_f16x8 al = __builtin_bit_cast(rp_f16x8, actL[idx]);
    #pragma unroll
                            for (int jt = 0; jt < NJ; ++jt) {
                                acc[g][jt] = __builtin_amdgcn_mfma_f32_16x16x32_f16(al, bh[jt], acc[g][jt], 0, 0, 0);
                                acc[g][jt] = __builtin_amdgcn_mfma_f32_16x16x32_f16(ah, bl[jt], acc[g][jt], 0, 0, 0);
                            }
    #pragma unroll
                            for (int jt = 0; jt < NJ; ++jt) acc[g][jt] = __builtin_amdgcn_mfma_f32_16x16x32_f16(ah, bh[jt], acc[g][jt], 0, 0, 0);
                        }
                    }
                }
                if constexpr (RO > 0) {
                    const int rslot = 2 * (it & 1) + (perm >> 1);
    #pragma unroll
                    for (int o = 0; o < RO; ++o) {
                        rp_f16x8 bh[NJ], bl[NJ];
    #pragma unroll
                        for (int jt = 0; jt < NJ; ++jt) {
                            bh[jt] = __builtin_bit_cast(rp_f16x8, wl[KO * WCH + (o * NJ + jt) * 128 + lane]);
                            bl[jt] = __builtin_bit_cast(rp_f16x8, wl[KO * WCH + (o * NJ + jt) * 128 + 64 + lane]);
                        }
    #pragma unroll
                        for (int g = 0; g < GPW; ++g) {
                            const int idx = (KO * RING + o * RINGR + rslot) * PW + 16 * (cw * GPW + g) + lq + 1;
                            const rp_f16x8 ah = __builtin_bit_cast(rp_f16x8, actH[idx]);
                            const rp_f16x8 al = __builtin_bit_cast(rp_f16x8, actL[idx]);
    #pragma unroll
                            for (int jt = 0; jt < NJ; ++jt) {
                                acc[g][jt] = __builtin_amdgcn_mfma_f32_16x16x32_f16(al, bh[jt], acc[g][jt], 0, 0, 0);
                                acc[g][jt] = __builtin_amdgcn_mfma_f32_16x16x32_f16(ah, bl[jt], acc[g][jt], 0, 0, 0);
                            }
    #pragma unroll
                            for (int jt = 0; jt < NJ; ++jt) acc[g][jt] = __builtin_amdgcn_mfma_f32_16x16x32_f16(ah, bh[jt], acc[g][jt], 0, 0, 0);
                        }
                    }
                }
            }
#ifdef ST_TRACE
            if (cw == 0 && it == 2) { if (acc[0][0][0] == 123.456f) ST_STAMP(31); ST_STAMP(17); }
#endif
#pragma unroll
            for (int jt = 0; jt < NJ; ++jt) {
                const int co = NCO * jt + (DS ? lq : (lq & 7));
                const float bv = bvv[jt];
                f32x4 yv[GPW];
#pragma unroll
                for (int g = 0; g < GPW; ++g) {
                    f32x4 y;
                    y[0] = fmaf(acc[g][jt][0], unscale, bv); y[1] = fmaf(acc[g][jt][1], unscale, bv);
                    y[2] = fmaf(acc[g][jt][2], unscale, bv); y[3] = fmaf(acc[g][jt][3], unscale, bv);
                    if constexpr (idres) { const f32x4 r = rv[buf][g][jt]; y[0] = fmaf(r[0], rs, y[0]); y[1] = fmaf(r[1], rs, y[1]); y[2] = fmaf(r[2], rs, y[2]); y[3] = fmaf(r[3], rs, y[3]); }
                    yv[g] = y;
                }
                if (first_of_block) {
                    cshift[jt] = __shfl(yv[0][0], DS ? lq : (lq & 7));
                    csum[jt] = 0.f; csq[jt] = 0.f;
                }
                const float cs_ = cshift[jt];
                const bool ok = !MASKC || co < p.Cout;
#pragma unroll
                for (int g = 0; g < GPW; ++g) {
                    const int oy = y0 + OPS * it + dy, ox = 16 * (cw * GPW + g) + 4 * lg;
                    const f32x4 y = yv[g];
                    if constexpr (MASKC) { if (ok) *reinterpret_cast<mi_gptr<f32x4>>(obuf + (unsigned)(co * HW + oy * W + ox)) = y; }
                    else *reinterpret_cast<mi_gptr<f32x4>>(obuf + (unsigned)(co * HW + oy * W + ox)) = y;
                    const float d0 = y[0] - cs_, d1 = y[1] - cs_, d2 = y[2] - cs_, d3 = y[3] - cs_;
                    csum[jt] += ok ? (d0 + d1) + (d2 + d3) : 0.0f;
                    csq[jt] += ok ? fmaf(d0, d0, fmaf(d1, d1, fmaf(d2, d2, d3 * d3))) : 0.0f;
                }
            }
            if (cw == 0 && it == 2) ST_STAMP(18);
        };
        auto flush = [&]() {
            if (!p.out_stats || (ST_ABL & 2)) return;
#pragma unroll
            for (int jt = 0; jt < NJ; ++jt) {
                float s_ = csum[jt], q_ = csq[jt];
                if constexpr (!DS) { s_ += __shfl_xor(s_, 8); q_ += __shfl_xor(q_, 8); }
                s_ += __shfl_xor(s_, 16); q_ += __shfl_xor(q_, 16);
                s_ += __shfl_xor(s_, 32); q_ += __shfl_xor(q_, 32);
                if (lane < NCO) {
                    mi_stat_acc a; a.c = cshift[jt]; a.s = s_; a.q = q_; a.n = GPW * 16 * SR0;
                    mi_stat_finish(a, red[cw][2 * (NCO * jt + lane)], red[cw][2 * (NCO * jt + lane) + 1]);
                }
            }
        };
        auto publish = [&](int blk) {
            if (!p.out_stats || cw != 0 || (ST_ABL & 2)) return;
            if (lane < 2 * NCO * NJ && (lane >> 1) < p.Cout) {
                double v = red[0][lane];
                if constexpr (NCW == 2) v = red[0][lane] + red[1][lane];
                if constexpr (NCW == 4) v = (red[0][lane] + red[1][lane]) + (red[2][lane] + red[3][lane]);
                p.out_stats[((size_t)(b * p.Cout + (lane >> 1)) * nt + blk) * 2 + (lane & 1)] = v;
            }
        };
        issue_res(0, std::integral_constant<int, 0>{});
        __syncthreads();
        if (cw == 0) ST_STAMP(6);
        constexpr int SPB = SR0 / OPS;
#pragma unroll 1
        for (int kb = 0; kb < nblk; ++kb) {
            const int it0 = kb * SPB;
#pragma unroll 1
            for (int i = 0; i < SPB; i += 2) {
                issue_res(it0 + i + 1, std::integral_constant<int, 1>{});
                compute(it0 + i, std::integral_constant<int, 0>{}, i == 0);
                if (cw == 0 && kb == 0 && i == 0) ST_STAMP(7);
                __syncthreads();
                if (cw == 0 && it0 + i == 2) ST_STAMP(19);
                issue_res(it0 + i + 2, std::integral_constant<int, 0>{});
                compute(it0 + i + 1, std::integral_constant<int, 1>{}, false);
                if (i + 2 == SPB) flush();
                __syncthreads();
            }
            if (cw == 0 && kb + 1 == nblk) ST_STAMP(8);
            publish(blk0 + kb);
        }
        if (cw == 0) ST_STAMP(9);
    }
}

template <int W, int KO, int NJ, bool GN, int OM, int RO = 0>
int launch_stripe(const mi_conv_params& p, hipStream_t st) {
    using CFG = StCfg<W, KO, NJ, GN, OM, RO>;
    const int nt = p.H / CFG::SR0;
    int nblk = (p.tile_cfg >> 12) & 0xf;
    if (nblk == 0) nblk = ((W <= 64 || OM == 2) && nt % 2 == 0 && (long long)p.B * (nt / 2) >= 256) ? 2 : 1;
    if (nblk > nt || nt % nblk) nblk = 1;
    hipLaunchKernelGGL(HIP_KERNEL_NAME(conv_stripe_kernel<CFG>), dim3(p.B * (nt / nblk)), dim3(CFG::NT), 0, st, p, (const uint4*)p.w_rp, (const uint4*)p.res_w_rp, nblk);
    return mi_check_launch("conv_stripe_kernel");
}

template <int W>
int launch_stripe_w(const mi_conv_params& p, hipStream_t st, int ko, int nj, bool gn) {
    const int om = p.ksize == 4 ? 4 : (p.up2 ? 3 : (p.Cout < 8 * nj ? 2 : ((p.res0.data && !p.res_w) ? 1 : 0)));
#define ST_BLOCK(KO, NJ) if (gn && ko == KO && nj == NJ) return om == 1 ? launch_stripe<W, KO, NJ, true, 1>(p, st) : launch_stripe<W, KO, NJ, true, 0>(p, st)
#define ST_PLAIN(KO, NJ, OMV) if (!gn && ko == KO && nj == NJ && om == OMV) return launch_stripe<W, KO, NJ, false, OMV>(p, st)
    if constexpr (W == 64 || W == 128) {
        if (gn && ko == 1 && nj == 1 && om == 0 && p.res0.data && p.res_w) return launch_stripe<W, 1, 1, true, 0, 2>(p, st);
    }
    if constexpr (W == 64) {
        if (gn && ko == 2 && nj == 2 && om == 0 && p.res0.data && p.res_w) return launch_stripe<W, 2, 2, true, 0, 4>(p, st);
    }
    if (om <= 1) {
        ST_BLOCK(1, 1);
        if constexpr (W <= 128) { ST_BLOCK(2, 1); }
        if constexpr (W <= 64) { ST_BLOCK(2, 2); ST_BLOCK(4, 2); ST_BLOCK(3, 2); }
    }
    ST_PLAIN(1, 1, 0);
    ST_PLAIN(1, 1, 2);
    if constexpr (W <= 64) { ST_PLAIN(1, 2, 0); }
    if constexpr (W >= 64 && W <= 128) { ST_PLAIN(1, 1, 3); ST_PLAIN(2, 1, 3); }
    if constexpr (W >= 64 && W <= 128) { ST_PLAIN(1, 1, 4); }
#undef ST_BLOCK
#undef ST_PLAIN
    return MI_ERR_UNSUPPORTED;
}

int stripe_block_rows(const mi_conv_params& p, int* ko_, int* nj_) {
    const bool ds = p.ksize == 4 && p.stride == 2;
    if (!((p.ksize == 3 && p.stride == 1) || ds) || !p.w_rp || p.gn_coef || (p.tile_cfg & MI_CONV_HALF) || p.out_st) return 0;
    if (p.in0.st || (p.in1.data && p.in1.st) || (p.res0.data && p.res0.st)) return 0;
    if (!(p.W == 32 || p.W == 64 || p.W == 128 || p.W == 256)) return 0;
    const int sr0 = p.W / 8;
    if (p.H % sr0 || p.H < sr0 || (size_t)p.H * p.W * 64 >= (1ull << 31)) return 0;
    const int C0 = p.in0.C, C1 = p.in1.data ? p.in1.C : 0;
    if ((C0 & 7) || (C1 & 7) || C0 + C1 > RP_MAXC || p.Cout > 16) return 0;
    const bool rconv = p.res0.data && p.res_w;
    if (rconv) {
        const int cres = p.res0.C + (p.res1.data ? p.res1.C : 0);
        const bool m8 = cres == 16 && C0 + C1 == 8 && p.Cout == 8 && (p.W == 64 || p.W == 128), m16 = ST_RO4 && cres == 32 && C0 + C1 == 16 && p.Cout == 16 && p.W == 64;
        if (!p.res_w_rp || (p.res0.C & 7) || (p.res1.data && (p.res1.C & 7)) || (p.res1.data && p.res1.st) || !(m8 || m16) || !p.gn_groups || p.up2) return 0;
    } else if (p.res0.data && p.res0.C != p.Cout) return 0;
    if (p.gn_groups > MI_MAX_GROUPS || (p.gn_groups > 0 && ((C0 + C1) % p.gn_groups))) return 0;
    if (p.gn_groups > 0 && (!p.in0.stats || (p.in1.data && !p.in1.stats))) return 0;
    const int ko = (C0 + C1) >> 3, nj = ds ? (p.Cout + 15) >> 4 : (p.Cout + 7) >> 3;
    const bool gn = p.gn_groups > 0;
    if (ds) {
        if (gn || p.res0.data || p.up2 || C1 || ko != 1 || nj != 1 || !(p.W == 64 || p.W == 128)) return 0;
        if (ko_) { *ko_ = ko; *nj_ = nj; }
        return sr0;
    }
    const int om = p.up2 ? 3 : (p.Cout < 8 * nj ? 2 : ((p.res0.data && !rconv) ? 1 : 0));
    if (om == 3) {
        if (gn || p.res0.data || nj != 1 || p.Cout != 8 || ko > 2 || p.W < 64 || p.W > 128 || (p.H & 1)) return 0;
        if (ko_) { *ko_ = ko; *nj_ = nj; }
        return sr0;
    }
    if ((om == 1 && !gn) || (om == 2 && (gn || nj != 1))) return 0;
    const bool common = (ko == 1 && nj == 1) || (p.W <= 128 && ko == 2 && nj == 1 && gn);
    const bool small = p.W <= 64 && ((ko == 2 && nj == 2 && gn) || (ko == 4 && nj == 2 && gn) || (ko == 1 && nj == 2 && !gn) || (ko == 3 && nj == 2 && gn));
    if (!common && !small) return 0;
    if (ko_) { *ko_ = ko; *nj_ = nj; }
    return sr0;
}

}

extern "C" int mi_conv_stripe_rows(const mi_conv_params* pp) { return stripe_block_rows(*pp, nullptr, nullptr); }

int mi_conv_stripe_launch(const mi_conv_params& p, hipStream_t st) {
    int ko = 0, nj = 0;
    if (!stripe_block_rows(p, &ko, &nj)) { mi_set_error("mi_conv_fwd: tile_cfg 12 (full-width stripes) does not take this launch (see mi_conv_stripe_rows)"); return MI_ERR_UNSUPPORTED; }
    const bool gn = p.gn_groups > 0;
    int rc = MI_ERR_UNSUPPORTED;
    switch (p.W) {
        case 32: rc = launch_stripe_w<32>(p, st, ko, nj, gn); break;
        case 64: rc = launch_stripe_w<64>(p, st, ko, nj, gn); break;
        case 128: rc = launch_stripe_w<128>(p, st, ko, nj, gn); break;
        case 256: rc = launch_stripe_w<256>(p, st, ko, nj, gn); break;
    }
    if (rc == MI_ERR_UNSUPPORTED) mi_set_error("mi_conv_fwd: stripe kernel not instantiated for this shape");
    return rc;
}
```

minimagen_amd/engine.py:

```python
from __future__ import annotations

import ctypes as C
import os
from types import SimpleNamespace
from typing import List, Optional

import torch
from torch import nn

from . import _lib as L
from . import packing as P
from .layers import Attention, CrossAttention, EinopsToAndFrom, Identity, Parallel, ResnetBlock, TransformerBlock

MAX_TEXT_LEN = 256
CONV_SPLIT8 = int(os.environ.get("MINIMAGEN_CONV_SPLIT8", "64"))
CONV_RP = int(os.environ.get("MINIMAGEN_CONV_RP", "2"))
CONV_WIDE_GEMM = os.environ.get("MINIMAGEN_CONV_WIDE_GEMM", "1") != "0"
COND_GEMM = int(os.environ.get("MINIMAGEN_COND_GEMM", "2048"))
FLASH_KV_PREP = os.environ.get("MINIMAGEN_FLASH_KV_PREP", "1") != "0"
CE_MFMA = os.environ.get("MINIMAGEN_CE_MFMA", "1") != "0"
ATTN_COND = os.environ.get("MINIMAGEN_ATTN_COND", "1") != "0"
INIT_DOWN = os.environ.get("MINIMAGEN_INIT_DOWN", "1") != "0"
CONV_REVERSE = int(os.environ.get("MINIMAGEN_CONV_REVERSE", "1"))
RP_NTILE = int(os.environ.get("MINIMAGEN_RP_NTILE", "0"))
RP_NTILE_BY = {k: int(os.environ.get("MINIMAGEN_RP_NTILE_" + k, "0")) for k in ("L", "M", "S")}
RP_NTILE_PIPE = {k: int(os.environ.get("MINIMAGEN_RP_NTILE_PIPE_" + k, d)) for k, d in (("L", "0"), ("M", "4"), ("S", "2"))}
CONV_STRIPE = os.environ.get("MINIMAGEN_CONV_STRIPE", "LMS").upper().replace("0", "").replace("1", "LMS")
ST_NBLK = {k: int(os.environ.get("MINIMAGEN_ST_NBLK_" + k, "0")) for k in ("L", "M", "S")}
ST_NBLK_PIPE = {k: int(os.environ.get("MINIMAGEN_ST_NBLK_PIPE_" + k, d)) for k, d in (("L", "0"), ("M", "0"), ("S", "4"))}
WEIGHT_FINGERPRINT = os.environ.get("MINIMAGEN_WEIGHT_FINGERPRINT", "1") != "0"
JT = 17


class Act:
    __slots__ = ("t", "stats", "nt", "C", "H", "W", "batch", "uses", "rev")

    def __init__(self, t, stats, nt, C_, H, W, batch):
        self.t, self.stats, self.nt, self.C, self.H, self.W, self.batch = t, stats, nt, C_, H, W, batch
        self.uses = 0
        self.rev = False

    @property
    def st(self) -> int:
        return 1 if self.t.dtype == torch.bfloat16 else 0

    def c(self, consumer_batch: int, scale: float = 1.0) -> L.MiAct:
        bmod = self.batch if self.batch != consumer_batch else 0
        self.uses += 1
        return L.MiAct(L.ptr(self.t), self.C, L.ptr(self.stats), self.nt, scale, bmod, self.st)


class _Store16Unsupported(Exception):
    """raised while a launch plan is built with bf16 activation storage and a layer needs a kernel that only reads fp32"""


def _lin(m: Optional[nn.Linear]) -> L.MiLinear:
    if m is None:
        return L.MiLinear(0, 0, 0, 0)
    return L.MiLinear(L.ptr(m.weight), L.ptr(m.bias) if m.bias is not None else 0, m.in_features, m.out_features)


class Workspace:

    def __init__(self):
        self.sampler_state = {}
        self.step_tables = {}
        self.prog_stage = None
        self.prog_stage_off = {}
        self.resize_tabs = {}


def _close_workspace(ws):
    for st in ws.sampler_state.values():
        st.close(ws.dev)


class UnetEngine:
    def __init__(self, unet):
        self.unet = unet
        self._pack = None
        self._pack_key = None
        self._pack_fp = None
        self._ws = {}
        self.precision = os.environ.get("MINIMAGEN_PRECISION", "fp32")

    def _param_key(self):
        ts = self._tensors()
        return (str(ts[0].device), tuple(t.data_ptr() for t in ts), sum(t._version for t in ts))

    def _tensors(self):
        ts = self.__dict__.get("_tensor_list")
        if ts is None:
            ts = self._tensor_list = list(self.unet.parameters()) + list(self.unet.buffers())
        return ts

    def _fingerprint(self):
        ts = [t.detach() for t in self._tensors() if t.is_floating_point()]
        return torch.stack(torch._foreach_norm(ts, 1) + torch._foreach_norm(ts, 2))

    def invalidate(self):
        for ws in self._ws.values():
            _close_workspace(ws)
        self._ws = {}
        self._pack = self._pack_key = self._pack_fp = None
        self.__dict__.pop("_tensor_list", None)

    def _check_params(self):
        for name, t in list(self.unet.named_parameters()) + list(self.unet.named_buffers()):
            if t.dtype != torch.float32:
                raise L.MinImagenHipError(f"parameter {name} is {t.dtype}; the HIP path computes in fp32 like the reference")
            if not t.is_contiguous():
                raise L.MinImagenHipError(f"parameter {name} is not contiguous")
        L.require_device(next(self.unet.parameters()))

    def pack(self):
        key = self._param_key()
        if not WEIGHT_FINGERPRINT:
            if self._pack is not None and key == self._pack_key:
                return self._pack
            fp = None
        else:
            fp = self._fingerprint()
            if self._pack is not None and key == self._pack_key and torch.equal(fp, self._pack_fp):
                return self._pack
        return self._repack(key, fp)

    def pack_identity(self):
        if self._pack is None or self._param_key() != self._pack_key:
            self.pack()

    def pack_begin(self):
        fresh = list(self.unet.parameters()) + list(self.unet.buffers())
        cached = self._tensors()
        if len(fresh) != len(cached) or any(a is not b for a, b in zip(fresh, cached)):
            self.__dict__.pop("_tensor_list", None)
            return (None, None, None)
        if not WEIGHT_FINGERPRINT or self._pack is None or self._pack_fp is None:
            return None
        fp = self._fingerprint()
        flag = self.__dict__.get("_fp_flag")
        if flag is None or flag.device != torch.device("cpu"):
            flag = self._fp_flag = torch.zeros(1, dtype=torch.int32).pin_memory() if fp.is_cuda else torch.zeros(1, dtype=torch.int32)
        flag.copy_((fp != self._pack_fp).any().to(torch.int32).reshape(1), non_blocking=True)
        ev = torch.cuda.current_stream(fp.device).record_event() if fp.is_cuda else None
        return (flag, ev, fp)

    def pack_changed(self, token) -> bool:
        if token is None:
            return False
        flag, ev, _ = token
        if flag is None:
            return True
        if ev is not None:
            ev.synchronize()
        return bool(flag.item())

    def _repack(self, key, fp):
        self.invalidate()
        self._pack_fp = fp
        self._check_params()
        u = self.unet
        dev = next(u.parameters()).device
        lib = L.lib()
        pk = SimpleNamespace()
        pk.keep = []
        pk.freq = P.sinusoid_freq(u.dim, dev)
        pk.conv = {}
        pk.conv_rp = {}
        pk.conv_ig = {}
        pk.attn = {}
        pk.attn_exp = {}
        pk.attn_cond = {}

        def conv_pack(mod: nn.Conv2d, w=None, b=None):
            w = mod.weight if w is None else w
            ct = lib.mi_conv_cout_tile(w.shape[0])
            wp = P.pack_conv_weight(w.to(dev), ct)
            pk.keep.append(wp)
            if w.shape[-1] in (3, 4) and w.shape[1] % 8 == 0:
                pk.conv_rp[id(wp)] = P.pack_conv_weight_rp(w.to(dev))
            if CONV_WIDE_GEMM and w.shape[-1] == 3 and w.shape[1] % 32 == 0 and w.shape[0] % 64 == 0:
                pk.conv_ig[id(wp)] = P.pack_conv_weight_ig(w.to(dev))
            return wp

        resblocks: List[ResnetBlock] = [m for m in u.modules() if isinstance(m, ResnetBlock)]
        rows, biases, off = [], [], 0
        pk.ss_off = {}
        for rb in resblocks:
            if rb.time_mlp is not None:
                lin = rb.time_mlp[1]
                pk.ss_off[id(rb)] = off
                rows.append(lin.weight.detach())
                biases.append(lin.bias.detach())
                off += lin.out_features
        pk.R = off
        pk.tm_w = torch.cat(rows, 0).contiguous() if rows else torch.zeros(1, u.time_cond_dim, device=dev)
        pk.tm_b = torch.cat(biases, 0).contiguous() if rows else torch.zeros(1, device=dev)
        for rb in resblocks:
            pk.conv[id(rb.block1.project)] = conv_pack(rb.block1.project)
            pk.conv[id(rb.block2.project)] = conv_pack(rb.block2.project)
            if isinstance(rb.res_conv, nn.Conv2d):
                ct = lib.mi_conv_cout_tile(rb.res_conv.weight.shape[0])
                rw = P.pack_conv_weight(rb.res_conv.weight, ct).reshape(rb.res_conv.weight.shape[1], -1).contiguous()
                pk.keep.append(rw)
                if rb.res_conv.weight.shape[1] % 8 == 0:
                    pk.conv_rp[id(rw)] = P.pack_conv_weight_rp(rb.res_conv.weight)
                if CONV_WIDE_GEMM and rb.res_conv.weight.shape[1] % 32 == 0 and rb.res_conv.weight.shape[0] % 64 == 0:
                    pk.conv_ig[id(rw)] = P.pack_conv_weight_ig(rb.res_conv.weight)
                pk.conv[id(rb.res_conv)] = rw
            if rb.cross_attn is not None:
                ca: CrossAttention = rb.cross_attn.fn
                Cc = ca.to_q.in_features
                if ca.dim_head != 64:
                    raise NotImplementedError("cross-attention with dim_head != 64")
                if Cc not in (8, 16, 32):
                    if Cc % 16 or u.cond_dim % 16:
                        raise NotImplementedError(f"cross-attention over {Cc} channels / {u.cond_dim}-wide context: the wide path needs multiples of 16")
                    continue
                if not isinstance(ca.norm_context, Identity):
                    raise NotImplementedError("norm_context=True cross-attention is not on the MinImagen hot path")
                mg, mv, g0, v0 = P.fold_cross_attention(ca.to_q.weight, ca.to_kv.weight, ca.to_out[0].weight, ca.null_kv, ca.heads, ca.dim_head)
                pk.attn[id(ca)] = (mg, mv, g0, v0)
                pk.attn_exp[id(ca)] = P.attn_f16_exponents(mg, mv, g0, v0, cmax=P.layernorm_bound(u.norm_cond.weight, u.norm_cond.bias, u.cond_dim),
                                                           xmax=P.layernorm_bound(ca.norm.gamma, ca.norm.beta, Cc))
                if ATTN_COND and Cc in (8, 16) and u.cond_dim <= 8 and ca.heads == 8:
                    ex = P.attn_cond_exponents(mg, mv, g0, v0, cmax=P.layernorm_bound(u.norm_cond.weight, u.norm_cond.bias, u.cond_dim),
                                               xmax=P.layernorm_bound(ca.norm.gamma, ca.norm.beta, Cc))
                    if ex is not None:
                        pk.attn_cond[id(ca)] = (ex, P.pack_cross_attn_cond(mg, mv, g0, v0, ex["f_exp"], ex["g0_exp"], ex["mv_exp"]))
        for m in u.modules():
            if isinstance(m, Attention):
                Cc = m.to_q.in_features
                dh = m.to_kv.out_features // 2
                if dh != 64:
                    raise NotImplementedError("self-attention with dim_head != 64")
                if Cc not in (8, 16, 32):
                    if Cc % 16:
                        raise NotImplementedError(f"self-attention over {Cc} channels: the wide path needs a multiple of 16")
                    continue
                kv = m.to_kv.weight.detach()
                kv_full = torch.cat((kv[:dh].repeat(m.heads, 1), kv[dh:].repeat(m.heads, 1)), 0)
                pk.attn[id(m)] = P.fold_cross_attention(m.to_q.weight, kv_full, m.to_out[0].weight, m.null_kv, m.heads, dh)
        for level in u.downs:
            pre, _, _, _, post = level
            if isinstance(pre, nn.Conv2d):
                pk.conv[id(pre)] = conv_pack(pre)
            if isinstance(post, nn.Conv2d):
                pk.conv[id(post)] = conv_pack(post)
            elif isinstance(post, Parallel):
                w, b = P.fold_parallel_1x1(post.fns[0].weight, post.fns[0].bias, post.fns[1].weight, post.fns[1].bias)
                b = b.contiguous()
                pk.keep.append(b)
                pk.conv[id(post)] = (conv_pack(None, w=w), b)
        for level in u.ups:
            up = level[3]
            if isinstance(up, nn.Sequential):
                pk.conv[id(up[1])] = conv_pack(up[1])
        pk.conv[id(u.final_conv)] = conv_pack(u.final_conv)
        pk.ce_w = [c.weight.detach().permute(1, 2, 3, 0).contiguous() for c in u.init_conv.convs]
        pk.ce_mfma = {}
        cvs = u.init_conv.convs
        if CE_MFMA and [c.kernel_size[0] for c in cvs] == [3, 7, 15] and [c.out_channels for c in cvs] == [4, 2, 2] and u.channels <= 4:
            for chan0 in range(0, cvs[0].in_channels, u.channels):
                pk.ce_mfma[chan0] = P.pack_crossembed_mfma([c.weight for c in cvs], chan0, u.channels)
        pk.init_down = {}
        pre0 = u.downs[0][0]
        pk.init_down_ok = INIT_DOWN and CE_MFMA and isinstance(pre0, nn.Conv2d) and pre0.kernel_size == (4, 4) and pre0.stride == (2, 2) \
            and pre0.padding == (1, 1) and pre0.out_channels == 8 and len(cvs) <= 3 and all(c.kernel_size[0] % 2 == 1 and c.kernel_size[0] <= 15 for c in cvs) \
            and sum(c.out_channels for c in cvs) <= 16 and u.channels <= 4 and not u.init_conv_to_final_conv_residual
        self._pack, self._pack_key = pk, key
        return pk

    def _init_down_tables(self, pk):
        if not pk.init_down:
            u = self.unet
            cvs, pre0 = u.init_conv.convs, u.downs[0][0]
            dev = pre0.weight.device
            for chan0 in range(0, cvs[0].in_channels, u.channels):
                x_half = chan0 == 0
                w9, b9 = P.compose_init_down([c.weight for c in cvs], [c.bias for c in cvs] if x_half else None, pre0.weight, pre0.bias, chan0, u.channels)
                tab, exp, b32 = P.pack_init_down_mfma(w9, b9)
                pk.init_down[chan0] = (tab.to(dev), exp, b32.to(dev) if x_half else None)
        return pk.init_down

    def packed(self):
        return self._pack if self._pack is not None else self.pack()

    def workspace(self, B: int, B2: int, H: int, W: int, precision: Optional[str] = None, has_text: bool = True, lane: int = 0,
                  pipelined: bool = False) -> Workspace:
        pk = self.packed()
        dev = next(self.unet.parameters()).device
        precision = self.precision if precision is None else precision
        assert precision in ("fp32", "half"), precision
        key = (B, B2, H, W, str(dev), precision, has_text) + ((lane,) if lane else ()) + (("pipe",) if pipelined else ())
        ws = self._ws.get(key)
        if ws is not None:
            return ws
        u = self.unet
        ws = Workspace()
        ws.B, ws.B2, ws.H, ws.W, ws.dev = B, B2, H, W, dev
        ws.pipelined = pipelined
        ws.half = precision == "half"
        f = lambda *shape: torch.zeros(*shape, dtype=torch.float32, device=dev)
        ws.x = f(B, u.channels, H, W)
        ws.lowres = f(B, u.channels, H, W) if u.lowres_cond else None
        ws.times = torch.zeros(B, dtype=torch.int64, device=dev)
        ws.lowres_times = torch.zeros(B, dtype=torch.int64, device=dev) if u.lowres_cond else None
        ws.keep = torch.ones(B2, dtype=torch.uint8, device=dev)
        ws.c_text = f(B2, MAX_TEXT_LEN, u.cond_dim)
        ws.text_hiddens = f(B2, u.time_cond_dim)
        ws.ntot = u.num_time_tokens * (2 if u.lowres_cond else 1)
        ws.has_text = has_text
        ws.J = 1 + ws.ntot + (MAX_TEXT_LEN if has_text else 0)
        ws.JT = -(-ws.J // 16)
        ws.ss = f(B2, max(pk.R, 1))
        ws.c_time = f(B2, ws.ntot, u.cond_dim)
        ws.t_out = f(B2, u.time_cond_dim)
        ws.gv = {}
        ws.tensors = []
        ws.text_L = None
        for store16 in ((True, False) if ws.half else (False,)):
            ws.store16 = store16
            ws.cfrag = None
            ws.gv, ws.tensors, ws.prog, ws.prog_text, ws.wide_attn = {}, [], [], [], False
            ws.ig_convs = []
            try:
                self._build_program(ws, pk)
                break
            except _Store16Unsupported:
                continue
        if ws.ig_convs:
            nbytes = max(n for _, n in ws.ig_convs)
            ws.ig_prep = torch.empty((nbytes + 3) // 4, dtype=torch.float32, device=dev)
            for p_, _ in ws.ig_convs:
                p_.act_prep, p_.act_prep_bytes = L.ptr(ws.ig_prep), nbytes
        self._ws[key] = ws
        return ws

    def _tile_cfg(self, H, W, batch=None, cz=1):
        lib = L.lib()
        best = 0 if (W >= 64 and H * W > 64 * 64) else 2
        th, tw = C.c_int(), C.c_int()
        lib.mi_conv_tile_shape(best, C.byref(th), C.byref(tw))
        return best, -(-H // th.value) * -(-W // tw.value)

    def _stripe_rows(self, batch, Ho, Wo, in0, in1, Cout, gn, res, up2=0, ksize=3, stride=1) -> int:
        q = L.MiConvParams()
        q.B, q.H, q.W, q.Cout, q.ksize, q.stride, q.up2 = batch, Ho, Wo, Cout, ksize, stride, int(bool(up2))
        q.in0 = L.MiAct(1, in0.C, 1 if in0.stats is not None else 0, in0.nt, 1.0, 0)
        if in1 is not None:
            q.in1 = L.MiAct(1, in1.C, 1 if in1.stats is not None else 0, in1.nt, 1.0, 0)
        q.w_rp = 1
        if gn is not None:
            q.gn_groups = gn.num_groups
        if res is not None:
            r0, r1, rw, _ = res
            q.res0 = L.MiAct(1, r0.C, 1 if r0.stats is not None else 0, r0.nt, 1.0, 0)
            if r1 is not None:
                q.res1 = L.MiAct(1, r1.C, 1 if r1.stats is not None else 0, r1.nt, 1.0, 0)
            if rw is not None:
                q.res_w, q.res_w_rp = 1, 1
        return int(L.lib().mi_conv_stripe_rows(C.byref(q)))

    def _new_act(self, ws, batch, Cc, H, W, nt, fp32: bool = False) -> Act:
        t = torch.empty(batch, Cc, H, W, dtype=torch.float32 if (fp32 or not ws.store16) else torch.bfloat16, device=ws.dev)
        st = torch.zeros(batch, Cc, max(nt, 1), 2, dtype=torch.float64, device=ws.dev) if nt else None
        ws.tensors += [t, st]
        return Act(t, st, nt, Cc, H, W, batch)

    def _emit_conv(self, ws, pk, in0: Act, in1: Optional[Act], *, wpack, bias, Cout, ksize=3, stride=1, up2=0,
                   gn: Optional[nn.GroupNorm] = None, ss_off: Optional[int] = None, res=None, conditioned=False,
                   want_stats=True, skip_scale=1.0, out_fp32=False) -> Act:
        lib = L.lib()
        Ho = in0.H * 2 if up2 else in0.H // stride
        Wo = in0.W * 2 if up2 else in0.W // stride
        if stride == 2 and ((in0.H | in0.W) & 1):
            raise NotImplementedError("stride-2 conv on an odd-sized image")
        ins = [a for a in (in0, in1) if a is not None] + ([r for r in res[:2] if r is not None] if res else [])
        batch = ws.B2 if (conditioned or any(a.batch == ws.B2 for a in ins)) else ws.B
        ct = lib.mi_conv_cout_tile(Cout)
        cfg, nt = self._tile_cfg(Ho, Wo, batch, -(-Cout // ct))
        cin_tot = in0.C + (in1.C if in1 is not None else 0)
        cres = 0 if (res is None or res[2] is None) else res[0].C + (res[1].C if res[1] is not None else 0)
        rp = bool(CONV_RP) and ((ksize == 3 and stride == 1) or (ksize == 4 and stride == 2 and not up2 and CONV_RP >= 2)) \
            and (not up2 or CONV_RP >= 2) and Wo % 4 == 0 and id(wpack) in pk.conv_rp \
            and in0.C % 8 == 0 and (in1 is None or in1.C % 8 == 0) \
            and (res is None or res[2] is None or (id(res[2]) in pk.conv_rp and res[0].C % 8 == 0 and (res[1] is None or res[1].C % 8 == 0)))
        narrow = cin_tot <= 64 and cres <= 64 and Cout <= (16 if stride == 2 else (8 if up2 else 32))
        wide = rp and not narrow
        stripe = False
        if rp:
            cfg = 6
            if Ho * Wo <= 64 * 64 and (Wo <= 32 or Cout <= 8):
                cfg = 7
            if Cout > 16:
                cfg = 7
            if up2:
                cfg = 6
            if stride == 2 or wide:
                cfg = 7
            if wide and stride == 1 and not up2 and Wo % 64 == 0 and Cout >= 32 and not ws.half:
                cfg = 6
            if wide and stride == 1 and not up2 and Wo <= 16 and Ho > 8 and Cout >= 32 and not ws.half:
                cfg = 10
            gemm = wide and ksize == 3 and stride == 1 and (not up2 or res is None) and not ws.half and cin_tot % 32 == 0 and cres % 32 == 0 and Cout % 64 == 0 \
                and id(wpack) in pk.conv_ig and (cres == 0 or id(res[2]) in pk.conv_ig)
            if gemm:
                cfg = 11
            th, tw = {6: (8, 64), 7: (8, 32), 10: (16, 16), 11: (8, 16)}[cfg]
            nt = -(-Ho // th) * -(-Wo // tw)
            cls = "L" if Ho * Wo > 128 * 128 else ("M" if Ho * Wo > 64 * 64 else "S")
            if narrow and ((ksize == 3 and stride == 1) or (ksize == 4 and stride == 2)) and not ws.half and cls in CONV_STRIPE:
                rows = self._stripe_rows(batch, Ho, Wo, in0, in1, Cout, gn, res, up2, ksize, stride)
                if rows:
                    cfg, nt, stripe = 12, Ho // rows, True
        if ws.store16 and (not rp or wide):
            raise _Store16Unsupported()
        out = self._new_act(ws, batch, Cout, Ho, Wo, nt if want_stats else 0, fp32=out_fp32)
        p = L.MiConvParams()
        p.B, p.H, p.W = batch, Ho, Wo
        p.in0 = in0.c(batch)
        if in1 is not None:
            p.in1 = in1.c(batch, skip_scale)
        p.Cout, p.ksize, p.stride, p.up2 = Cout, ksize, stride, up2
        p.w, p.bias = L.ptr(wpack), L.ptr(bias)
        if gn is not None:
            p.gn_groups, p.gn_gamma, p.gn_beta, p.gn_eps = gn.num_groups, L.ptr(gn.weight), L.ptr(gn.bias), gn.eps
            if ss_off is not None:
                p.scale_shift, p.ss_stride, p.ss_off = L.ptr(ws.ss), ws.ss.shape[1], ss_off
        if res is not None:
            r0, r1, rw, rb = res
            p.res0 = r0.c(batch)
            if r1 is not None:
                p.res1 = r1.c(batch, skip_scale)
            p.res_w, p.res_b = L.ptr(rw), L.ptr(rb)
        p.out_st = out.st
        p.out, p.out_stats, p.tile_cfg = L.ptr(out.t), L.ptr(out.stats), cfg | 0x100 | (0x400 if ws.half else 0) | (0x800 if (CONV_SPLIT8 and Ho * Wo <= CONV_SPLIT8 * CONV_SPLIT8) else 0)
        if wide:
            coef = torch.zeros(batch, cin_tot, 4, dtype=torch.float32, device=ws.dev)
            exps = torch.zeros(batch, 2, dtype=torch.int32, device=ws.dev)
            ws.tensors += [coef, exps]
            p.gn_coef, p.gn_exps = L.ptr(coef), L.ptr(exps)
        if rp:
            out.rev = bool(CONV_REVERSE) and batch % 8 == 0 and not in0.rev
            if out.rev:
                p.tile_cfg |= 0x200
            cls = "L" if Ho * Wo > 128 * 128 else ("M" if Ho * Wo > 64 * 64 else "S")
            nt_knob = RP_NTILE_BY[cls] or RP_NTILE
            if not nt_knob and ws.pipelined and RP_NTILE_PIPE[cls] and batch * nt // RP_NTILE_PIPE[cls] >= 256:
                nt_knob = RP_NTILE_PIPE[cls]
            if stripe:
                nt_knob = ST_NBLK[cls]
                if ws.pipelined and ST_NBLK_PIPE[cls] and nt % ST_NBLK_PIPE[cls] == 0 and batch * nt // ST_NBLK_PIPE[cls] >= 128 \
                        and self.unet.lowres_cond:
                    nt_knob = ST_NBLK_PIPE[cls]
                if nt_knob and (nt % nt_knob or nt_knob > 15):
                    nt_knob = 0
            p.tile_cfg |= (nt_knob & 0xf) << 12
            frags = pk.conv_ig if gemm else pk.conv_rp
            frag, p.w_rp_exp = frags[id(wpack)]
            p.w_rp = L.ptr(frag)
            if res is not None and res[2] is not None:
                rfrag, p.res_w_rp_exp = frags[id(res[2])]
                p.res_w_rp = L.ptr(rfrag)
        if wide:
            ws.prog.append((lib.mi_gn_coef_fwd, p, "gn_coef"))
            if gemm:
                ws.ig_convs.append((p, lib.mi_conv_prep_bytes(batch, cin_tot, cres, Ho, Wo)))
                ws.prog.append((lib.mi_conv_prep_fwd, p, "conv_prep"))
        ws.prog.append((lib.mi_conv_fwd, p, "conv"))
        return out

    def _emit_resnet(self, ws, pk, rb: ResnetBlock, in0: Act, in1: Optional[Act]) -> Act:
        u = self.unet
        s = u.skip_connect_scale
        Cout = rb.block1.project.out_channels
        has_cross = rb.cross_attn is not None
        h = self._emit_conv(ws, pk, in0, in1, wpack=pk.conv[id(rb.block1.project)], bias=rb.block1.project.bias, Cout=Cout,
                            gn=rb.block1.groupnorm, want_stats=not has_cross, skip_scale=s)
        if has_cross:
            h = self._emit_cross_attn(ws, pk, rb.cross_attn.fn, h)
        ss_off = pk.ss_off.get(id(rb))
        if isinstance(rb.res_conv, nn.Conv2d):
            res = (in0, in1, pk.conv[id(rb.res_conv)], rb.res_conv.bias)
        else:
            assert in1 is None
            res = (in0, None, None, None)
        return self._emit_conv(ws, pk, h, None, wpack=pk.conv[id(rb.block2.project)], bias=rb.block2.project.bias, Cout=Cout,
                               gn=rb.block2.groupnorm, ss_off=ss_off, res=res, conditioned=ss_off is not None, skip_scale=s)

    @staticmethod
    def _call(fn, name, *args):
        return (lambda _p, st, fn=fn, args=args: fn(*args, st)), None, name

    def _buf(self, ws, *shape):
        t = torch.empty(*shape, dtype=torch.float32, device=ws.dev)
        ws.tensors.append(t)
        return t

    def _emit_tokens_out(self, ws, tokens, batch, Cc, H, W, ln, res: Act, want_stats: bool) -> Act:
        if ws.store16:
            raise _Store16Unsupported()
        lib = L.lib()
        HW = H * W
        out = self._new_act(ws, batch, Cc, H, W, -(-HW // 64) if want_stats else 0)
        p = L.MiTokensToNchwParams()
        p.B, p.HW, p.C, p.tokens = batch, HW, Cc, L.ptr(tokens)
        if ln is not None:
            p.gamma, p.beta, p.eps = L.ptr(ln.gamma), L.ptr(ln.beta), 1e-5
        p.res = res.c(batch)
        p.out, p.out_stats = L.ptr(out.t), L.ptr(out.stats)
        ws.prog.append((lib.mi_tokens_to_nchw_fwd, p, "tokens_to_nchw"))
        return out

    def _emit_cross_attn_wide(self, ws, ca: CrossAttention, h: Act) -> Act:
        if ws.store16:
            raise _Store16Unsupported()
        lib, u = L.lib(), self.unet
        Cc, HW, B2, inner = h.C, h.H * h.W, ws.B2, ca.heads * 64
        xh, q, o, t = self._buf(ws, B2, HW, Cc), self._buf(ws, B2, HW, inner), self._buf(ws, B2, HW, inner), self._buf(ws, B2, HW, Cc)
        kv_time = self._buf(ws, B2, ws.ntot, 2 * inner)
        kv_text = self._buf(ws, B2, MAX_TEXT_LEN, 2 * inner) if ws.has_text else None
        xa = h.c(B2)
        ws.tensors.append(xa)
        ws.prog.append(self._call(lib.mi_ln_tokens_fwd, "ln_tokens", C.byref(xa), B2, HW, L.ptr(ca.norm.gamma), L.ptr(ca.norm.beta), L.ptr(xh)))
        ws.prog.append(self._call(lib.mi_gemm_f32, "gemm_q", L.ptr(xh), L.ptr(ca.to_q.weight), 0, 0, L.ptr(q), B2 * HW, inner, Cc, 0))
        ws.prog.append(self._call(lib.mi_gemm_f32, "gemm_kv_time", L.ptr(ws.c_time), L.ptr(ca.to_kv.weight), 0, 0, L.ptr(kv_time), B2 * ws.ntot, 2 * inner, u.cond_dim, 0))
        if ws.has_text:
            ws.prog_text.append(self._call(lib.mi_gemm_f32, "gemm_kv_text", L.ptr(ws.c_text), L.ptr(ca.to_kv.weight), 0, 0, L.ptr(kv_text), B2 * MAX_TEXT_LEN, 2 * inner, u.cond_dim, 0))
        p = L.MiFlashAttnParams()
        p.B, p.HW, p.heads, p.kv_heads, p.q, p.q_scale = B2, HW, ca.heads, ca.heads, L.ptr(q), 64 ** -0.5 * P.LOG2E
        p.null_k, p.null_v = L.ptr(ca.null_kv), L.ptr(ca.null_kv) + 4 * 64
        p.k0, p.v0, p.n0, p.ld0, p.bs0 = L.ptr(kv_time), L.ptr(kv_time) + 4 * inner, ws.ntot, 2 * inner, ws.ntot * 2 * inner
        if ws.has_text:
            p.k1, p.v1, p.n1, p.ld1, p.bs1 = L.ptr(kv_text), L.ptr(kv_text) + 4 * inner, MAX_TEXT_LEN, 2 * inner, MAX_TEXT_LEN * 2 * inner
        p.out = L.ptr(o)
        if FLASH_KV_PREP:
            nbytes = lib.mi_flash_kv_prep_bytes(B2 * ca.heads, 1 + ws.ntot + (MAX_TEXT_LEN if ws.has_text else 0))
            prep = self._buf(ws, (nbytes + 3) // 4)
            p.kv_prep, p.kv_prep_bytes = L.ptr(prep), nbytes
        ws.prog.append((lib.mi_flash_attn_fwd, p, "flash_attn"))
        ws.prog.append(self._call(lib.mi_gemm_f32, "gemm_out", L.ptr(o), L.ptr(ca.to_out[0].weight), 0, 0, L.ptr(t), B2 * HW, Cc, inner, 0))
        ws.wide_attn = True
        return self._emit_tokens_out(ws, t, B2, Cc, h.H, h.W, ca.to_out[1], h, True)

    def _emit_self_attn_wide(self, ws, at: Attention, x: Act, want_stats: bool) -> Act:
        if ws.store16:
            raise _Store16Unsupported()
        lib = L.lib()
        Cc, HW, batch, inner = x.C, x.H * x.W, x.batch, at.heads * 64
        xh, q, kv = self._buf(ws, batch, HW, Cc), self._buf(ws, batch, HW, inner), self._buf(ws, batch, HW, 128)
        o, t = self._buf(ws, batch, HW, inner), self._buf(ws, batch, HW, Cc)
        xa = x.c(batch)
        ws.tensors.append(xa)
        ws.prog.append(self._call(lib.mi_ln_tokens_fwd, "ln_tokens", C.byref(xa), batch, HW, L.ptr(at.norm.gamma), L.ptr(at.norm.beta), L.ptr(xh)))
        ws.prog.append(self._call(lib.mi_gemm_f32, "gemm_q", L.ptr(xh), L.ptr(at.to_q.weight), 0, 0, L.ptr(q), batch * HW, inner, Cc, 0))
        ws.prog.append(self._call(lib.mi_gemm_f32, "gemm_kv", L.ptr(xh), L.ptr(at.to_kv.weight), 0, 0, L.ptr(kv), batch * HW, 128, Cc, 0))
        p = L.MiFlashAttnParams()
        p.B, p.HW, p.heads, p.kv_heads, p.q, p.q_scale = batch, HW, at.heads, 1, L.ptr(q), 64 ** -0.5 * P.LOG2E
        p.null_k, p.null_v = L.ptr(at.null_kv), L.ptr(at.null_kv) + 4 * 64
        p.k0, p.v0, p.n0, p.ld0, p.bs0 = L.ptr(kv), L.ptr(kv) + 4 * 64, HW, 128, HW * 128
        p.out = L.ptr(o)
        if FLASH_KV_PREP and at.heads % 4 == 0:
            nbytes = lib.mi_flash_kv_prep_bytes(batch, HW + 1)
            prep = self._buf(ws, (nbytes + 3) // 4)
            p.kv_prep, p.kv_prep_bytes = L.ptr(prep), nbytes
        ws.prog.append((lib.mi_flash_attn_fwd, p, "flash_attn"))
        ws.prog.append(self._call(lib.mi_gemm_f32, "gemm_out", L.ptr(o), L.ptr(at.to_out[0].weight), 0, 0, L.ptr(t), batch * HW, Cc, inner, 0))
        return self._emit_tokens_out(ws, t, batch, Cc, x.H, x.W, at.to_out[1], x, want_stats)

    def _emit_chan_ff_wide(self, ws, tb: TransformerBlock, y: Act) -> Act:
        if ws.store16:
            raise _Store16Unsupported()
        lib = L.lib()
        Cc, HW, batch, Chid = y.C, y.H * y.W, y.batch, tb.ff[1].out_channels
        t0, h1, h2, t = self._buf(ws, batch, HW, Cc), self._buf(ws, batch, HW, Chid), self._buf(ws, batch, HW, Chid), self._buf(ws, batch, HW, Cc)
        zeros = torch.zeros(Cc, dtype=torch.float32, device=ws.dev)
        ya = y.c(batch)
        ws.tensors += [zeros, ya]
        ws.prog.append(self._call(lib.mi_ln_tokens_fwd, "ln_tokens", C.byref(ya), batch, HW, L.ptr(tb.ff[0].g), L.ptr(zeros), L.ptr(t0)))
        ws.prog.append(self._call(lib.mi_gemm_f32, "gemm_ff1", L.ptr(t0), L.ptr(tb.ff[1].weight), 0, 0, L.ptr(h1), batch * HW, Chid, Cc, 3))
        ws.prog.append(self._call(lib.mi_ln_rows_fwd, "ln_rows", L.ptr(h1), L.ptr(tb.ff[3].g), 0, L.ptr(h2), batch * HW, Chid, 1e-5))
        ws.prog.append(self._call(lib.mi_gemm_f32, "gemm_ff2", L.ptr(h2), L.ptr(tb.ff[4].weight), 0, 0, L.ptr(t), batch * HW, Cc, Chid, 0))
        return self._emit_tokens_out(ws, t, batch, Cc, y.H, y.W, None, y, True)

    def _emit_cross_attn(self, ws, pk, ca: CrossAttention, h: Act) -> Act:
        lib = L.lib()
        Cc, HW = h.C, h.H * h.W
        if Cc not in (8, 16, 32):
            return self._emit_cross_attn_wide(ws, ca, h)
        cond = pk.attn_cond.get(id(ca)) if (not ws.half and ws.JT == 17) else None
        if cond is not None:
            if ws.cfrag is None:
                ws.cfrag = torch.zeros(ws.B2, lib.mi_attn_cond_frag_floats(ws.JT), dtype=torch.float32, device=ws.dev)
                ws.cfrag_exp = (cond[0]["c_exp"], cond[0]["i_exp"])
            assert ws.cfrag_exp == (cond[0]["c_exp"], cond[0]["i_exp"])
            gv = ws.cfrag
        else:
            FR = lib.mi_attn_fragment_floats(Cc)
            jts = ws.JT + (ws.JT & 1)
            gv = torch.zeros(ws.B2, ca.heads, jts, 64, FR, dtype=torch.float32, device=ws.dev)
            ws.gv[id(ca)] = gv
        nt = -(-HW // 64)
        out = self._new_act(ws, ws.B2, Cc, h.H, h.W, nt)
        p = L.MiCrossAttnParams()
        p.B2, p.C, p.HW, p.heads, p.J = ws.B2, Cc, HW, ca.heads, ws.J
        p.x = h.c(ws.B2)
        p.gv = L.ptr(gv)
        p.n1_g, p.n1_b = L.ptr(ca.norm.gamma), L.ptr(ca.norm.beta)
        p.n2_g, p.n2_b = L.ptr(ca.to_out[1].gamma), L.ptr(ca.to_out[1].beta)
        p.out_st = out.st
        p.out, p.out_stats, p.variant = L.ptr(out.t), L.ptr(out.stats), (7 if ws.half else 6)
        p.x_exp, p.g_exp, p.v_exp = pk.attn_exp[id(ca)]
        if cond is not None:
            ex, tab = cond
            p.variant, p.head_tab = 8, L.ptr(tab)
            p.x_exp, p.g_exp, p.v_exp = ex["x_exp"], ex["f_exp"] + ex["c_exp"], ex["c_exp"] + ex["mv_exp"]
        ws.prog.append((lib.mi_cross_attn_fwd, p, "cross_attn"))
        return out

    def _emit_self_attn(self, ws, pk, at: Attention, x: Act, want_stats: bool) -> Act:
        if ws.store16:
            raise _Store16Unsupported()
        lib = L.lib()
        Cc, HW, batch = x.C, x.H * x.W, x.batch
        if Cc not in (8, 16, 32):
            return self._emit_self_attn_wide(ws, at, x, want_stats)
        xh = torch.empty(batch, HW, Cc, dtype=torch.float32, device=ws.dev)
        J = HW + 1
        jt = -(-J // 16)
        FR = lib.mi_attn_fragment_floats(Cc)
        gv = torch.zeros(batch, at.heads, jt, 64, FR, dtype=torch.float32, device=ws.dev)
        ws.tensors += [xh, gv]
        xa = x.c(batch)
        ws.tensors.append(xa)

        def ln_call(_p, st, xa=xa, xh=xh):
            return lib.mi_ln_tokens_fwd(C.byref(xa), batch, HW, L.ptr(at.norm.gamma), L.ptr(at.norm.beta), L.ptr(xh), st)
        ws.prog.append((lambda p_, st: ln_call(p_, st), None, "ln_tokens"))
        mg, mv, g0, v0 = pk.attn[id(at)]
        fp = L.MiAttnFoldParams()
        fp.B2, fp.C, fp.cd, fp.heads, fp.JT = batch, Cc, Cc, at.heads, jt
        fp.c_rows, fp.c_stride_b, fp.row0, fp.nrows, fp.write_null, fp.n_blocks = L.ptr(xh), HW * Cc, 1, HW, 1, 1
        fp.blk[0].mg, fp.blk[0].mv, fp.blk[0].g0, fp.blk[0].v0, fp.blk[0].gv = L.ptr(mg), L.ptr(mv), L.ptr(g0), L.ptr(v0), L.ptr(gv)
        ws.prog.append((lib.mi_attn_fold_rows, fp, "self_fold"))
        out = self._new_act(ws, batch, Cc, x.H, x.W, -(-HW // 64) if want_stats else 0)
        p = L.MiSelfAttnParams()
        p.B2, p.C, p.HW, p.heads, p.J = batch, Cc, HW, at.heads, J
        p.x, p.gv = xa, L.ptr(gv)
        p.n1_g, p.n1_b = L.ptr(at.norm.gamma), L.ptr(at.norm.beta)
        p.n2_g, p.n2_b = L.ptr(at.to_out[1].gamma), L.ptr(at.to_out[1].beta)
        p.out, p.out_stats = L.ptr(out.t), L.ptr(out.stats)
        ws.prog.append((lib.mi_self_attn_fwd, p, "self_attn"))
        return out

    def _emit_transformer_block(self, ws, pk, tb: TransformerBlock, x: Act) -> Act:
        if ws.store16:
            raise _Store16Unsupported()
        lib = L.lib()
        y = self._emit_self_attn(ws, pk, tb.attn.fn, x, want_stats=False)
        if y.C not in (8, 16, 32):
            return self._emit_chan_ff_wide(ws, tb, y)
        HW = y.H * y.W
        out = self._new_act(ws, y.batch, y.C, y.H, y.W, -(-HW // 256))
        p = L.MiChanFFParams()
        p.B, p.C, p.Chid, p.HW = y.batch, y.C, tb.ff[1].out_channels, HW
        p.x = y.c(y.batch)
        p.g1, p.w1, p.g2, p.w2 = L.ptr(tb.ff[0].g), L.ptr(tb.ff[1].weight), L.ptr(tb.ff[3].g), L.ptr(tb.ff[4].weight)
        p.out, p.out_stats = L.ptr(out.t), L.ptr(out.stats)
        ws.prog.append((lib.mi_chan_ff_fwd, p, "chan_ff"))
        return out

    def _fold_params(self, ws, pk, rows_t, stride_b, row0, nrows, write_null):
        lib = L.lib()
        calls = []
        cas = {id(m): m for m in self.unet.modules() if isinstance(m, CrossAttention)}
        by_c = {}
        for ca_id in ws.gv:
            if ca_id in cas:
                by_c.setdefault(cas[ca_id].to_q.in_features, []).append(ca_id)
        for _, ids in by_c.items():
            for i0 in range(0, len(ids), 8):
                chunk = ids[i0:i0 + 8]
                ca0 = cas[chunk[0]]
                p = L.MiAttnFoldParams()
                p.B2, p.C, p.cd, p.heads, p.JT = ws.B2, ca0.to_q.in_features, self.unet.cond_dim, ca0.heads, ws.JT
                p.c_rows, p.c_stride_b, p.row0, p.nrows, p.write_null = L.ptr(rows_t), stride_b, row0, nrows, write_null
                p.frag_f16 = 1
                p.n_blocks = len(chunk)
                for k, cid in enumerate(chunk):
                    mg, mv, g0, v0 = pk.attn[cid]
                    _, p.blk[k].g_exp, p.blk[k].v_exp = pk.attn_exp[cid]
                    p.blk[k].mg, p.blk[k].mv, p.blk[k].g0, p.blk[k].v0 = L.ptr(mg), L.ptr(mv), L.ptr(g0), L.ptr(v0)
                    p.blk[k].gv = L.ptr(ws.gv[cid])
                calls.append((lib.mi_attn_fold_rows, p, "fold"))
        if ws.cfrag is not None:
            p = L.MiAttnCondParams()
            p.B2, p.cd, p.JT = ws.B2, self.unet.cond_dim, ws.JT
            p.c_rows, p.c_stride_b, p.row0, p.nrows, p.write_null = L.ptr(rows_t), stride_b, row0, nrows, write_null
            p.c_exp, p.i_exp = ws.cfrag_exp
            p.frag = L.ptr(ws.cfrag)
            calls.append((lib.mi_attn_cond_rows, p, "fold_cond"))
        return calls

    def _build_program(self, ws, pk):
        u = self.unet
        lib = L.lib()
        B, B2, H, W = ws.B, ws.B2, ws.H, ws.W
        cp = L.MiCondStepParams()
        cp.B2, cp.B, cp.dim, cp.cd, cp.tcd, cp.ntok = B2, B, u.dim, u.cond_dim, u.time_cond_dim, u.num_time_tokens
        cp.time, cp.lowres_time, cp.freq = L.ptr(ws.times), L.ptr(ws.lowres_times), L.ptr(pk.freq)
        cp.th, cp.tc, cp.tt = _lin(u.to_time_hiddens[1]), _lin(u.to_time_cond[0]), _lin(u.to_time_tokens[0])
        if u.lowres_cond:
            cp.lth, cp.ltc, cp.ltt = _lin(u.to_lowres_time_hiddens[1]), _lin(u.to_lowres_time_cond[0]), _lin(u.to_lowres_time_tokens[0])
        cp.text_hiddens = L.ptr(ws.text_hiddens) if ws.has_text else 0
        cp.norm_w, cp.norm_b = L.ptr(u.norm_cond.weight), L.ptr(u.norm_cond.bias)
        cp.time_mlps = L.MiLinear(L.ptr(pk.tm_w), L.ptr(pk.tm_b), u.time_cond_dim, pk.R)
        cp.ss, cp.c_time, cp.t_out = L.ptr(ws.ss), L.ptr(ws.c_time), L.ptr(ws.t_out)
        ws.cond_params = cp
        ws.prog_cond = [(lib.mi_cond_step_fwd, cp, "cond_step")]
        if COND_GEMM and pk.R >= COND_GEMM and u.time_cond_dim % 32 == 0:
            cg = L.MiCondStepParams.from_buffer_copy(cp)
            ws.silu_t = self._buf(ws, B2, u.time_cond_dim)
            ws.tm_bias = pk.tm_b.unsqueeze(0).expand(B2, -1).contiguous()
            ws.tensors.append(ws.tm_bias)
            cg.ss, cg.silu_out = 0, L.ptr(ws.silu_t)
            ws.prog_cond = [(lib.mi_cond_step_fwd, cg, "cond_step"),
                            self._call(lib.mi_gemm_f32, "gemm_time_mlps", L.ptr(ws.silu_t), L.ptr(pk.tm_w), 0, L.ptr(ws.tm_bias), L.ptr(ws.ss), B2, pk.R, u.time_cond_dim, 0)]

        cin = u.init_conv.convs[0].in_channels
        assert cin == u.channels * (2 if u.lowres_cond else 1)
        cfg, nt = self._tile_cfg(H, W, B)
        ce_mfma = bool(pk.ce_mfma) and W % 4 == 0
        if ws.store16 and not ce_mfma:
            raise _Store16Unsupported()
        if ce_mfma:
            cfg = 8 if H * W >= 128 * 128 else 9
            th, tw = C.c_int(), C.c_int()
            lib.mi_conv_tile_shape(cfg, C.byref(th), C.byref(tw))
            nt = -(-H // th.value) * -(-W // tw.value)
        ctot = sum(u.init_conv.dim_scales)
        if len(u.init_conv.convs) > 3:
            raise NotImplementedError("CrossEmbedLayer with more than 3 kernel sizes")
        init_down = pk.init_down_ok and not ws.half and not ws.store16 and H >= 4 and W >= 4 and H % 2 == 0 and W % 4 == 0

        def ce_params(src, chan0, with_bias, out_t, out_stats, addend):
            ce = L.MiCrossEmbedParams()
            ce.B, ce.H, ce.W = B, H, W
            ce.in0, ce.C0 = L.ptr(src), u.channels
            ce.n_kernels = len(u.init_conv.convs)
            for i, cv in enumerate(u.init_conv.convs):
                k, co = cv.kernel_size[0], cv.out_channels
                ce.ksize[i], ce.cout[i] = k, co
                ce.w[i] = L.ptr(pk.ce_w[i]) + 4 * chan0 * k * k * co
                ce.bias[i] = L.ptr(cv.bias) if with_bias else 0
            ce.out, ce.out_stats, ce.tile_cfg, ce.addend = L.ptr(out_t), L.ptr(out_stats), cfg, L.ptr(addend)
            ce.out_st = 1 if ws.store16 else 0
            if ce_mfma:
                tab, exps = pk.ce_mfma[chan0]
                ce.w_mfma, ce.tile_cfg = L.ptr(tab), cfg | (0x400 if ws.half else 0)
                for i in range(3):
                    ce.w_mfma_exp[i] = exps[i]
            return ce

        def id_params(src, chan0, out_t, out_stats, addend, id_cfg):
            q = L.MiInitDownParams()
            q.B, q.H, q.W = B, H, W
            q.in0, q.C0 = L.ptr(src), u.channels
            q.n_kernels = len(u.init_conv.convs)
            for i, cv in enumerate(u.init_conv.convs):
                q.ksize[i], q.cout[i] = cv.kernel_size[0], cv.out_channels
            tab, q.w_exp, b9 = pk.init_down[chan0]
            q.Cout, q.w_tab, q.bias9 = 8, L.ptr(tab), L.ptr(b9)
            q.out, q.out_stats, q.tile_cfg, q.addend = L.ptr(out_t), L.ptr(out_stats), id_cfg, L.ptr(addend)
            return q

        ws.prog_pre = []
        if init_down:
            self._init_down_tables(pk)
            id_cfg = 0 if W // 2 >= 64 else 1
            cur = self._new_act(ws, B, 8, H // 2, W // 2, lib.mi_init_down_tiles(id_cfg, H, W))
            fn = lib.mi_init_down_fwd
            if u.lowres_cond:
                ws.ce_lr = torch.zeros(B, 8, H // 2, W // 2, dtype=torch.float32, device=ws.dev)
                ws.prog_pre.append((fn, id_params(ws.lowres, u.channels, ws.ce_lr, None, None, id_cfg), "crossembed_lowres"))
            ws.prog.append((fn, id_params(ws.x, 0, cur.t, cur.stats, ws.ce_lr if u.lowres_cond else None, id_cfg), "crossembed"))
        else:
            cur = self._new_act(ws, B, ctot, H, W, nt)
            if u.lowres_cond:
                ws.ce_lr = torch.zeros(B, ctot, H, W, dtype=torch.bfloat16 if ws.store16 else torch.float32, device=ws.dev)
                ws.prog_pre.append((lib.mi_crossembed_fwd, ce_params(ws.lowres, u.channels, False, ws.ce_lr, None, None), "crossembed_lowres"))
                ws.prog.append((lib.mi_crossembed_fwd, ce_params(ws.x, 0, True, cur.t, cur.stats, ws.ce_lr), "crossembed"))
            else:
                ws.prog.append((lib.mi_crossembed_fwd, ce_params(ws.x, 0, True, cur.t, cur.stats, None), "crossembed"))

        hiddens: List[Act] = []
        for level, (pre, init_block, resnet_blocks, attn_block, post) in enumerate(u.downs):
            if isinstance(pre, nn.Conv2d) and not (init_down and level == 0):
                cur = self._emit_conv(ws, pk, cur, None, wpack=pk.conv[id(pre)], bias=pre.bias, Cout=pre.out_channels, ksize=4, stride=2)
            cur = self._emit_resnet(ws, pk, init_block, cur, None)
            for rb in resnet_blocks:
                cur = self._emit_resnet(ws, pk, rb, cur, None)
                hiddens.append(cur)
            if isinstance(attn_block, TransformerBlock):
                cur = self._emit_transformer_block(ws, pk, attn_block, cur)
            hiddens.append(cur)
            if isinstance(post, nn.Conv2d):
                cur = self._emit_conv(ws, pk, cur, None, wpack=pk.conv[id(post)], bias=post.bias, Cout=post.out_channels, ksize=4, stride=2)
            elif isinstance(post, Parallel):
                wp, bsum = pk.conv[id(post)]
                cur = self._emit_conv(ws, pk, cur, None, wpack=wp, bias=bsum, Cout=post.fns[0].out_channels)
        cur = self._emit_resnet(ws, pk, u.mid_block1, cur, None)
        if u.mid_attn is not None:
            cur = self._emit_self_attn(ws, pk, u.mid_attn.fn.fn, cur, want_stats=True)
        cur = self._emit_resnet(ws, pk, u.mid_block2, cur, None)
        for init_block, resnet_blocks, attn_block, upsample in u.ups:
            cur = self._emit_resnet(ws, pk, init_block, cur, hiddens.pop())
            for rb in resnet_blocks:
                cur = self._emit_resnet(ws, pk, rb, cur, hiddens.pop())
            if isinstance(attn_block, TransformerBlock):
                cur = self._emit_transformer_block(ws, pk, attn_block, cur)
            if isinstance(upsample, nn.Sequential):
                cv = upsample[1]
                cur = self._emit_conv(ws, pk, cur, None, wpack=pk.conv[id(cv)], bias=cv.bias, Cout=cv.out_channels, up2=1)
        cur = self._emit_resnet(ws, pk, u.final_res_block, cur, None)
        out = self._emit_conv(ws, pk, cur, None, wpack=pk.conv[id(u.final_conv)], bias=u.final_conv.bias, Cout=u.channels_out,
                              want_stats=False, conditioned=True, out_fp32=True)
        ws.pred = out.t
        if (out.H, out.W) != (H, W):
            raise L.MinImagenHipError(f"U-Net output is {out.H}x{out.W} for a {H}x{W} input (image size must be divisible by the down-sampling factor)")
        if ws.gv or ws.cfrag is not None:
            ws.prog_cond += self._fold_params(ws, pk, ws.c_time, ws.ntot * u.cond_dim, 1, ws.ntot, 0)

    def set_text(self, ws, text_embeds: torch.Tensor, text_mask: Optional[torch.Tensor], keep: torch.Tensor):
        u, pk, lib = self.unet, self.packed(), L.lib()
        st = L.current_stream()
        if text_embeds is None:
            assert not ws.has_text, "workspace was built for a text-conditioned call"
            for fn, fp, name in self._fold_params(ws, pk, ws.c_time, ws.ntot * u.cond_dim, 1, 0, 1):
                L.check(fn(C.byref(fp), st), name)
            return
        assert ws.has_text, "workspace was built for a call without text"
        text_embeds = text_embeds.to(device=ws.dev, dtype=torch.float32).contiguous()
        assert text_embeds.shape[0] == ws.B and text_embeds.shape[-1] == u.text_embed_dim
        mask8 = None if text_mask is None else text_mask.to(device=ws.dev).to(torch.uint8).contiguous()
        k8 = keep.to(device='cpu', dtype=torch.uint8)
        if getattr(ws, "keep_host", None) is None or not torch.equal(ws.keep_host, k8):
            ws.keep.copy_(k8)
            ws.keep_host = k8.clone()
        ws.text_keepalive = (text_embeds, mask8)
        L.require_device(text_embeds, mask8)
        p = L.MiTextCondParams()
        p.B2, p.B, p.L, p.E, p.cd, p.tcd, p.max_len = ws.B2, ws.B, text_embeds.shape[1], u.text_embed_dim, u.cond_dim, u.time_cond_dim, MAX_TEXT_LEN
        p.text_embeds, p.text_mask, p.keep = L.ptr(text_embeds), L.ptr(mask8), L.ptr(ws.keep)
        p.text_to_cond = _lin(u.text_to_cond)
        p.null_text_embed = L.ptr(u.null_text_embed)
        ln = u.to_text_non_attn_cond[0]
        p.ln_w, p.ln_b = L.ptr(ln.weight), L.ptr(ln.bias)
        p.h1, p.h2 = _lin(u.to_text_non_attn_cond[1]), _lin(u.to_text_non_attn_cond[3])
        p.null_text_hidden = L.ptr(u.null_text_hidden)
        p.norm_w, p.norm_b = L.ptr(u.norm_cond.weight), L.ptr(u.norm_cond.bias)
        p.c_text, p.text_hiddens = L.ptr(ws.c_text), L.ptr(ws.text_hiddens)
        L.check(lib.mi_text_cond_fwd(C.byref(p), st), "mi_text_cond_fwd")
        for fn, fp, name in self._fold_params(ws, pk, ws.c_text, MAX_TEXT_LEN * u.cond_dim, 1 + ws.ntot, MAX_TEXT_LEN, 1):
            L.check(fn(C.byref(fp), st), name)
        for fn, fp, name in ws.prog_text:
            L.check(fn(None, st), name)

    def prepare_lowres(self, ws, stream=None):
        st = L.current_stream() if stream is None else stream
        for fn, p, name in ws.prog_pre:
            L.check(fn(C.byref(p), st), name)

    def prepare_step_tables(self, ws, T: int, t_state: torch.Tensor, stream=None, t_map=None):
        u, pk, lib = self.unet, self.packed(), L.lib()
        st = L.current_stream() if stream is None else stream
        B2, dev = ws.B2, ws.dev
        if ws.wide_attn:
            ws.prog_stage = ws.prog_cond
            return
        key = (T, t_state.data_ptr()) if t_map is None else (T, t_state.data_ptr(), tuple(int(v) for v in t_map))
        tb = ws.step_tables.get(key)
        if tb is None:
            tb = SimpleNamespace()
            steps_t = torch.arange(T, dtype=torch.int64, device=dev) if t_map is None else t_map.to(dev, torch.int64).contiguous()
            assert steps_t.numel() == T
            n = T * B2
            tb.times = steps_t.repeat_interleave(B2).contiguous()
            tb.lowres_times = torch.zeros(n, dtype=torch.int64, device=dev) if u.lowres_cond else None
            tb.text_hiddens = torch.empty(n, u.time_cond_dim, dtype=torch.float32, device=dev)
            tb.ss = torch.empty(n, max(pk.R, 1), dtype=torch.float32, device=dev)
            cp = L.MiCondStepParams.from_buffer_copy(ws.cond_params)
            cp.B2 = cp.B = n
            cp.time, cp.lowres_time = L.ptr(tb.times), L.ptr(tb.lowres_times)
            cp.text_hiddens, cp.ss, cp.c_time, cp.t_out = (L.ptr(tb.text_hiddens) if ws.has_text else 0), L.ptr(tb.ss), 0, 0
            tb.cond = cp
            tb.times_t = steps_t
            tb.lowres_t = torch.zeros(T, dtype=torch.int64, device=dev) if u.lowres_cond else None
            tb.c_time_t = torch.empty(T, ws.ntot, u.cond_dim, dtype=torch.float32, device=dev)
            ct = L.MiCondStepParams.from_buffer_copy(ws.cond_params)
            ct.B2 = ct.B = T
            ct.time, ct.lowres_time = L.ptr(tb.times_t), L.ptr(tb.lowres_t)
            ct.text_hiddens, ct.ss, ct.c_time, ct.t_out = 0, 0, L.ptr(tb.c_time_t), 0
            tb.cond_t = ct
            tb.fold, tb.tables = [], []
            stage_blocks = []
            for fn, fp, name in self._fold_params(ws, pk, tb.c_time_t, ws.ntot * u.cond_dim, 1, ws.ntot, 0):
                if isinstance(fp, L.MiAttnCondParams):
                    f2 = L.MiAttnCondParams.from_buffer_copy(fp)
                    f2.t_state = L.ptr(t_state)
                    stage_blocks.append(f2)
                    continue
                f1 = L.MiAttnFoldParams.from_buffer_copy(fp)
                f1.B2, f1.mode = T, 1
                for k in range(fp.n_blocks):
                    t = torch.empty(T, ws.ntot, fp.heads, fp.C, 2, dtype=torch.float32, device=dev)
                    tb.tables.append(t)
                    f1.blk[k].table = L.ptr(t)
                tb.fold.append(f1)
                f2 = L.MiAttnFoldParams.from_buffer_copy(f1)
                f2.B2, f2.mode, f2.t_state = B2, 3, L.ptr(t_state)
                stage_blocks.append(f2)
            if not stage_blocks:
                f2 = L.MiAttnFoldParams()
                f2.B2, f2.mode, f2.t_state, f2.n_blocks = B2, 3, L.ptr(t_state), 0
                stage_blocks.append(f2)
            stage_blocks[0].ss_all, stage_blocks[0].ss, stage_blocks[0].ss_n = L.ptr(tb.ss), L.ptr(ws.ss), ws.ss.shape[1]
            tb.stage = [(lib.mi_attn_cond_rows if isinstance(f2, L.MiAttnCondParams) else lib.mi_attn_fold_rows, f2, "stage_step") for f2 in stage_blocks]
            tb.keep = t_state
            ws.step_tables[key] = tb
        tb.text_hiddens.view(T, B2, -1).copy_(ws.text_hiddens.unsqueeze(0).expand(T, -1, -1))
        if u.lowres_cond:
            tb.lowres_times.view(T, B2)[:, :ws.B].copy_(ws.lowres_times.unsqueeze(0).expand(T, -1))
            if B2 != ws.B:
                tb.lowres_times.view(T, B2)[:, ws.B:].copy_(ws.lowres_times.unsqueeze(0).expand(T, -1))
            tb.lowres_t.copy_(ws.lowres_times[:1].expand(T))
        L.check(lib.mi_cond_step_fwd(C.byref(tb.cond), st), "mi_cond_step_fwd (all steps: scale/shift rows)")
        L.check(lib.mi_cond_step_fwd(C.byref(tb.cond_t), st), "mi_cond_step_fwd (all steps: time tokens)")
        for f1 in tb.fold:
            L.check(lib.mi_attn_fold_rows(C.byref(f1), st), "mi_attn_fold_rows (all steps)")
        ws.prog_stage = tb.stage

    def drop_step_tables(self, ws, t_state: torch.Tensor):
        for key in [k for k in ws.step_tables if k[1] == t_state.data_ptr()]:
            tb = ws.step_tables.pop(key)
            for k in [k for k in ws.prog_stage_off if k[0] == id(tb.stage)]:
                del ws.prog_stage_off[k]
            if ws.prog_stage is tb.stage:
                ws.prog_stage = ws.prog_cond

    def stage_prog(self, ws, t_off: int = 0):
        if t_off == 0:
            return ws.prog_stage
        assert ws.prog_stage is not ws.prog_cond, "the step-at-a-time conditioning cannot address a timestep offset"
        cache = ws.prog_stage_off
        key = (id(ws.prog_stage), t_off)
        if key not in cache:
            prog = []
            for fn, p, name in ws.prog_stage:
                q = type(p).from_buffer_copy(p)
                q.t_off = t_off
                prog.append((fn, q, name))
            cache[key] = prog
        return cache[key]

    def step_offsets_supported(self, ws) -> bool:
        return ws.prog_stage is not ws.prog_cond

    def run_step(self, ws, stream=None, t_off: int = 0):
        st = L.current_stream() if stream is None else stream
        for fn, p, name in self.stage_prog(ws, t_off) + ws.prog:
            rc = fn(C.byref(p), st) if p is not None else fn(None, st)
            if rc != 0:
                L.check(rc, name)

    def run(self, ws, stream=None):
        st = L.current_stream() if stream is None else stream
        for fn, p, name in ws.prog_cond + ws.prog:
            rc = fn(C.byref(p), st) if p is not None else fn(None, st)
            if rc != 0:
                L.check(rc, name)

    def forward_once(self, x, time, *, lowres_cond_img, lowres_noise_times, text_embeds, text_mask, keep, cond_scale=None):
        u, lib = self.unet, L.lib()
        self.pack()
        L.require_device(x)
        B, Cc, H, W = x.shape
        assert Cc == u.channels
        two = cond_scale is not None
        ws = self.workspace(B, 2 * B if two else B, H, W, has_text=text_embeds is not None)
        ws.x.copy_(x)
        ws.times.copy_(time.to(torch.int64))
        if u.lowres_cond:
            ws.lowres.copy_(lowres_cond_img)
            ws.lowres_times.copy_(lowres_noise_times.to(torch.int64))
            self.prepare_lowres(ws)
        if two:
            keep = torch.cat((torch.ones(B, dtype=torch.bool), torch.zeros(B, dtype=torch.bool)))
        self.set_text(ws, text_embeds, text_mask, keep)
        self.run(ws)
        if not two:
            return ws.pred.clone()
        out = torch.empty(B, u.channels_out, H, W, dtype=torch.float32, device=ws.dev)
        p = L.MiCfgX0Params(B, u.channels_out * H * W, L.ptr(ws.pred), 1, float(cond_scale), 0, 0, 0, L.ptr(out), 0)
        L.check(lib.mi_cfg_x0_fwd(C.byref(p), L.current_stream()), "mi_cfg_x0_fwd")
        return out
```

minimagen_amd/packing.py:

```python
from __future__ import annotations

import math

import torch

LOG2E = 1.4426950408889634


def pack_conv_weight(w: torch.Tensor, cout_tile: int) -> torch.Tensor:
    cout = w.shape[0]
    pad = (cout + cout_tile - 1) // cout_tile * cout_tile
    out = torch.zeros(w.shape[1], w.shape[2], w.shape[3], pad, dtype=torch.float32, device=w.device)
    out[..., :cout] = w.detach().permute(1, 2, 3, 0)
    return out.contiguous()


def fold_parallel_1x1(w3: torch.Tensor, b3, w1: torch.Tensor, b1):
    w = w3.detach().clone()
    w[:, :, 1, 1] += w1.detach()[:, :, 0, 0]
    return w, (b3.detach() + b1.detach())


def fold_cross_attention(to_q, to_kv, to_out, null_kv, heads: int, dim_head: int = 64):
    dev = to_q.device
    H, D = heads, dim_head
    to_q, to_kv, to_out, null_kv = (t.detach().to('cpu') for t in (to_q, to_kv, to_out, null_kv))
    q = to_q.detach().double().reshape(H, D, -1)
    kv = to_kv.detach().double()
    k = kv[:H * D].reshape(H, D, -1)
    v = kv[H * D:].reshape(H, D, -1)
    o = to_out.detach().double().reshape(-1, H, D).permute(1, 0, 2)
    nk, nv = null_kv.detach().double().unbind(0)
    scale = D ** -0.5
    mg = torch.einsum('hda,hdb->hab', q, k) * (scale * LOG2E)
    mv = torch.einsum('had,hdb->hab', o, v)
    g0 = torch.einsum('hda,d->ha', q, nk) * (scale * LOG2E)
    v0 = torch.einsum('had,d->ha', o, nv)
    f = lambda t: t.float().contiguous().to(dev)
    return f(mg), f(mv), f(g0), f(v0)


def sinusoid_freq(dim: int, device) -> torch.Tensor:
    half = dim // 2
    k = math.log(10000) / (half - 1)
    return torch.exp(torch.arange(half) * -k).float().contiguous().to(device)


RP_PERM = (0, 2, 1, 3)


def rp_weight_exponent(mx: float) -> int:
    exp = 0 if (mx == 0.0 or not math.isfinite(mx)) else 7 - math.floor(math.log2(mx))
    return max(-100, min(100, exp))


def pack_conv_weight_rp(w: torch.Tensor, exp=None):
    cout, cin, kh, kw = w.shape
    assert (kh, kw) in ((3, 3), (1, 1), (4, 4))
    if exp is None:
        wd = w.detach().double().cpu()
        exp = rp_weight_exponent(float(wd.abs().max()))
    else:
        wd = w.detach().double()
    dev = wd.device
    ws = wd * (2.0 ** exp)
    if kh == 4:
        nj, ko = -(-cout // 16), -(-cin // 8)
        wp = torch.zeros(nj * 16, ko * 8, 4, 4, dtype=torch.float64, device=dev)
        wp[:cout, :cin] = ws
        lane = torch.arange(64, device=dev)
        lq, lg = lane & 15, lane >> 4
        co = 16 * torch.arange(nj, device=dev)[:, None] + lq[None, :]
        ci = 8 * torch.arange(ko, device=dev)[:, None] + torch.arange(8, device=dev)[None, :]
        out = wp[co[None, None, :, :, None], ci[:, None, None, None, :], lg[None, None, None, :, None], torch.arange(4, device=dev)[None, :, None, None, None]]
        hi = out.float().half()
        lo = (out - hi.double()).float().half()
        return torch.cat((hi, lo), dim=-1).contiguous().to(w.device), exp
    nj, ko, steps = -(-cout // 8), -(-cin // 8), kw
    wp = torch.zeros(nj * 8, ko * 8, 3, kw, dtype=torch.float64, device=dev)
    if kh == 3:
        wp[:cout, :cin] = ws
    else:
        wp[:cout, :cin, 1, :] = ws[:, :, 0, :]
    lane = torch.arange(64, device=dev)
    lq, lg = lane & 15, lane >> 4
    r = torch.tensor(RP_PERM, device=dev)[lg]
    ky = r - (lq >> 3)
    live = ((ky >= 0) & (ky <= 2)).double()
    kyc = ky.clamp(0, 2)
    co = (8 * torch.arange(nj, device=dev)[:, None] + (lq & 7)[None, :])
    ci = (8 * torch.arange(ko, device=dev)[:, None] + torch.arange(8, device=dev)[None, :])
    out = wp[co[None, None, :, :, None], ci[:, None, None, None, :], kyc[None, None, None, :, None], torch.arange(steps, device=dev)[None, :, None, None, None]]
    out = out * live[None, None, None, :, None]
    hi = out.float().half()
    lo = (out - hi.double()).float().half()
    return torch.cat((hi, lo), dim=-1).contiguous().to(w.device), exp


def pack_conv_weight_ig(w: torch.Tensor, exp=None):
    cout, cin, kh, kw = w.shape
    assert (kh, kw) in ((3, 3), (1, 1)) and cin % 32 == 0 and cout % 16 == 0
    wd = w.detach().double()
    if exp is None:
        exp = rp_weight_exponent(float(wd.abs().max()))
    ws = (wd * (2.0 ** exp)).reshape(cout // 16, 16, cin // 32, 4, 8, kh * kw)
    out = ws.permute(2, 5, 0, 3, 1, 4).reshape(cin // 32, kh * kw, cout // 16, 64, 8)
    hi = out.float().half()
    lo = (out - hi.double()).float().half()
    return torch.stack((hi, lo), dim=3).contiguous().to(w.device), exp


def attn_f16_exponents(mg, mv, g0, v0, cmax: float, xmax: float):
    def k(bound):
        bound = float(bound)
        if not math.isfinite(bound) or bound <= 0.0:
            return 0
        return max(-40, min(40, 12 - math.ceil(math.log2(bound))))
    gb = max(float(mg.abs().sum(-1).max()) * cmax, float(g0.abs().max()))
    vb = max(float(mv.abs().sum(-1).max()) * cmax, float(v0.abs().max()))
    return k(xmax), k(gb), k(vb)


def attn_cond_exponents(mg, mv, g0, v0, cmax: float, xmax: float):
    def k(bound):
        bound = float(bound)
        if not math.isfinite(bound) or bound <= 0.0:
            return 0
        return max(-40, min(40, 12 - math.ceil(math.log2(bound))))
    x_exp, c_exp = k(xmax), k(cmax)
    i_exp = max(-14, min(12, c_exp))
    shift = c_exp - i_exp
    mgd, g0d = mg.detach().double(), g0.detach().double()
    f_exp = min(k(float(mgd.abs().max())), k(float(mgd.abs().sum(1).max()) * xmax) - x_exp)
    g0_exp = min(k(float(g0d.abs().max())), k(float(g0d.abs().sum(-1).max()) * xmax) - x_exp)
    f_exp = min(f_exp, g0_exp - shift)
    g0_exp = f_exp + shift
    mv_exp = k(float(mv.detach().abs().max()))
    if max(abs(e) for e in (x_exp, c_exp, f_exp, g0_exp, mv_exp)) > 60:
        return None
    return dict(x_exp=x_exp, c_exp=c_exp, i_exp=i_exp, f_exp=f_exp, g0_exp=g0_exp, mv_exp=mv_exp)


def pack_cross_attn_cond(mg, mv, g0, v0, f_exp: int, g0_exp: int, mv_exp: int):
    H, Cc, cd = mg.shape
    assert Cc <= 16 and cd <= 8
    dev = mg.device
    F = torch.zeros(H, 12, 16, dtype=torch.float64)
    F[:, :cd, :Cc] = mg.detach().double().cpu().transpose(1, 2) * 2.0 ** f_exp
    F[:, 8, :Cc] = g0.detach().double().cpu() * 2.0 ** g0_exp
    MV = torch.zeros(H, 16, 8, dtype=torch.float64)
    MV[:, :Cc, :cd] = mv.detach().double().cpu() * 2.0 ** mv_exp
    V0 = torch.zeros(H, 16, dtype=torch.float32)
    V0[:, :Cc] = v0.detach().float().cpu()
    lane = torch.arange(64)
    lq, lg = lane & 15, lane >> 4
    el = torch.arange(4)
    a = 4 * lg[:, None] + el[None, :]
    split = lambda t: (t.float().half(), (t - t.float().half().double()).float().half())
    rows = []
    for T in range(2):
        e = 4 * T + (lq & 3)
        lgp = lq >> 2
        d = torch.where(e < 6, 3 * lgp + e % 3, 2 * lgp + e - 6)
        hi, lo = split(F[:, d[:, None], a])
        rows.append(torch.cat((hi, lo), -1))
    hi, lo = split(MV[:, lq[:, None], a % 8])
    rows.append(torch.cat((hi, hi), -1))
    rows.append(torch.cat((lo, torch.zeros_like(lo)), -1))
    rows.append(V0[:, a].contiguous().view(torch.float16))
    tab = torch.stack(rows, 1).contiguous()
    return tab.view(torch.float32).contiguous().to(dev)


def layernorm_bound(weight, bias, n: int) -> float:
    with torch.no_grad():
        if bias is not None:
            w, b = torch.stack((weight.detach().abs().max(), bias.detach().abs().max())).tolist()
        else:
            w, b = float(weight.detach().abs().max()), 0.0
    return w * math.sqrt(max(n - 1, 1)) + b


CE_TILES = ((0, 0), (0, 2), (1, 0), (2, 0))
CE_TABLE_ROWS = 32


def _crossembed_toeplitz(scaled, cin: int):
    tab = torch.zeros(CE_TABLE_ROWS, 2, 2, 2, 4, 8, dtype=torch.float64)
    w3, w7, w15 = scaled
    for lg in range(4):
        for dx in range(2):
            for h in range(2):
                kx = 2 * lg + dx + 8 * h
                if kx < 15:
                    tab[16:31, h, 0, :, lg, 4 * dx:4 * dx + cin] = w15[:, :, :, kx].permute(2, 0, 1)
                kx = 2 * lg + dx + 8 * h - 4
                if 0 <= kx < 7:
                    tab[8:15, h, 0, :, lg, 4 * dx:4 * dx + cin] = w7[:, :, :, kx].permute(2, 0, 1)
            kx = 2 * (lg & 1) + dx
            if kx < 3:
                for t in range(2):
                    for q in range(4):
                        ky = q - 1 + (lg >> 1)
                        if 0 <= ky < 3:
                            tab[4 * t + q, 0, 0, :, lg, 4 * dx:4 * dx + cin] = w3[2 * t:2 * t + 2, :, ky, kx]
    return tab


def pack_crossembed_mfma(ws, chan0: int, cin: int):
    assert cin <= 4 and len(ws) == 3 and [w.shape[-1] for w in ws] == [3, 7, 15] and [w.shape[0] for w in ws] == [4, 2, 2]
    exps, scaled = [], []
    for w in ws:
        wd = w.detach().double().cpu()[:, chan0:chan0 + cin]
        mx = float(wd.abs().max())
        e = 0 if (mx == 0.0 or not math.isfinite(mx)) else 7 - math.floor(math.log2(mx))
        e = max(-100, min(100, e))
        exps.append(e)
        scaled.append(wd * (2.0 ** e))
    tab = _crossembed_toeplitz(scaled, cin)
    hi = tab[:, :, 0].float().half()
    lo = (tab[:, :, 0] - hi.double()).float().half()
    out = torch.stack((hi, lo), dim=2)
    return out.reshape(CE_TABLE_ROWS, 256).contiguous().to(ws[0].device), exps


def crossembed_mfma_gather_index(shapes, chan0: int, cin: int):
    idx_w, off = [], 0
    for sh in shapes:
        n = 1
        for d in sh:
            n *= d
        idx_w.append((torch.arange(n, dtype=torch.float64) + (off + 1)).reshape(sh)[:, chan0:chan0 + cin])
        off += n
    tab = _crossembed_toeplitz(idx_w, cin)[:, :, 0]
    idx = tab.round().long() - 1
    idx[idx < 0] = off
    return idx.reshape(-1).contiguous()


def pack_crossembed_mfma_device(ws, idx: torch.Tensor, exps):
    flat = torch.cat([w.detach().reshape(-1) * (2.0 ** e) for w, e in zip(ws, exps)] + [ws[0].new_zeros(1)])
    t = flat[idx].reshape(CE_TABLE_ROWS, 2, 2, 4, 8)
    hi = t.half()
    lo = (t - hi.float()).half()
    return torch.stack((hi, lo), dim=2).reshape(CE_TABLE_ROWS, 256).contiguous()


ID_TAPS = 18
ID_ROWS = 3 * ID_TAPS + 1
ID_STEPS = 5


def compose_init_down(ce_ws, ce_bs, wd, bd, chan0: int, cin: int):
    ks = [w.shape[-1] for w in ce_ws]
    assert all(k % 2 == 1 and k <= 15 for k in ks) and tuple(wd.shape[2:]) == (4, 4)
    m_tot = sum(w.shape[0] for w in ce_ws)
    assert wd.shape[1] == m_tot
    wc = torch.zeros(m_tot, cin, 15, 15, dtype=torch.float64)
    m0 = 0
    for w, k in zip(ce_ws, ks):
        o = (15 - k) // 2
        wc[m0:m0 + w.shape[0], :, o:o + k, o:o + k] = w.detach().double().cpu()[:, chan0:chan0 + cin]
        m0 += w.shape[0]
    wdd = wd.detach().double().cpu()
    co = wdd.shape[0]
    with_bias = ce_bs is not None
    bc = torch.cat([b.detach().double().cpu() for b in ce_bs]) if with_bias else torch.zeros(m_tot, dtype=torch.float64)
    taps = ((1, 2, 3), (0, 1, 2, 3), (0, 1, 2))
    w9 = torch.zeros(3, 3, co, cin, ID_TAPS, ID_TAPS, dtype=torch.float64)
    b9 = torch.zeros(3, 3, co, dtype=torch.float64)
    for vy in range(3):
        for vx in range(3):
            for a in taps[vy]:
                for b in taps[vx]:
                    w9[vy, vx, :, :, a:a + 15, b:b + 15] += torch.einsum('om,mcyx->ocyx', wdd[:, :, a, b], wc)
                    b9[vy, vx] += wdd[:, :, a, b] @ bc
            if with_bias and bd is not None:
                b9[vy, vx] += bd.detach().double().cpu()
    return w9, b9


def pack_init_down_mfma(w9: torch.Tensor, b9: torch.Tensor):
    co, cin = w9.shape[2], w9.shape[3]
    assert co == 8 and cin <= 4 and tuple(w9.shape[4:]) == (ID_TAPS, ID_TAPS)
    wp = torch.zeros(3, 3, co, 4, ID_TAPS, 24, dtype=torch.float64)
    wp[:, :, :, :cin, :, :ID_TAPS] = w9
    exp = rp_weight_exponent(float(wp.abs().max()))
    wp = wp * (2.0 ** exp)
    tab = torch.zeros(ID_ROWS, ID_STEPS, co, 4, 2, 4, dtype=torch.float64)
    f = lambda t, n: t.reshape(3, co, 4, ID_TAPS, n, 4, 2).permute(0, 3, 4, 1, 5, 6, 2)
    main = tab[:3 * ID_TAPS].reshape(3, ID_TAPS, ID_STEPS, co, 4, 2, 4)
    main[:, :, 0:3] = f(wp[:, 1], 3)
    main[:, :, 3] = f((wp[:, 0] - wp[:, 1])[..., 8:16], 1)[:, :, 0]
    main[:, :, 4] = f((wp[:, 2] - wp[:, 1])[..., 2:10], 1)[:, :, 0]
    t = tab.reshape(ID_ROWS, ID_STEPS, co, 4, 8)
    hi = t.float().half()
    lo = (t - hi.double()).float().half()
    out = torch.stack((hi, lo), dim=2)
    return out.reshape(ID_ROWS, -1).contiguous(), exp, b9.float().contiguous()
```

minimagen_amd/sampler.py:

```python
from __future__ import annotations

import ctypes as C
import os

import torch

from . import _lib as L
from .helpers import cubic_taps, quantile_rank

def _drain(dev):
    if L.backend() == "hip-gfx950" and torch.cuda.is_available():
        torch.cuda.synchronize(dev)


def destroy_graph(entry, dev):
    if entry.get("graph") is not None:
        _drain(dev)
        L.lib().mi_graph_destroy(entry["graph"])
        entry["graph"] = None


def cubic_resize(ws, img, image_size: int, stream):
    B, Cc, Hin, Win = img.shape
    if Hin == image_size:
        return img
    cache = ws.resize_tabs
    if (Hin, Win) not in cache:
        _, idx_h, w_h = cubic_taps(Hin, image_size)
        _, idx_w, w_w = cubic_taps(Win, image_size)
        cache[(Hin, Win)] = ([t.to(ws.dev) for t in (idx_h, w_h, idx_w, w_w)], idx_h.shape[1], idx_w.shape[1])
    tabs, kh, kw = cache[(Hin, Win)]
    up = torch.empty(B, Cc, image_size, image_size, dtype=torch.float32, device=ws.dev)
    rp = L.MiResizeParams(B * Cc, Hin, Win, image_size, image_size, kh, kw, L.ptr(img), L.ptr(up),
                          L.ptr(tabs[0]), L.ptr(tabs[1]), L.ptr(tabs[2]), L.ptr(tabs[3]))
    L.check(L.lib().mi_resize_fwd(C.byref(rp), stream), "mi_resize_fwd")
    ws.resize_keepalive = tabs
    return up


class StageState:
    __slots__ = ("coef", "tau", "t_map", "x0_prev", "ext", "t_state", "x0", "hist", "s_q", "v_q", "seed_dev", "graphs",
                 "group_sync", "group_err_host", "group_failed", "group_heal", "known", "mask", "ip", "known_noise")

    def __init__(self, sched, B: int, n: int, dev, solver=None, hw: int = None, objective: str = 'noise'):
        self.tau = self.t_map = self.x0_prev = None
        self.known = self.mask = self.ip = self.known_noise = None
        known = {} if hw is None else dict(known=True)
        if objective != 'noise':
            known['objective'] = objective
        if hw is not None:
            self.known = torch.zeros(B, n, dtype=torch.float32, device=dev)
            self.mask = torch.zeros(B, hw, dtype=torch.uint8, device=dev)
        if solver is None:
            self.coef = sched.sampler_coef_table(**known).to(dev).contiguous()
        else:
            self.tau, coef = sched.sampler_tables(solver[0], solver[1], solver[2] if solver[1] == 'ddim' else None, **known)
            self.coef = coef.to(dev).contiguous()
            self.t_map = self.tau.to(torch.int32).to(dev).contiguous()
            if solver[1] == 'dpmpp_2m':
                self.x0_prev = torch.zeros(B, n, dtype=torch.float32, device=dev)
            self.ext = L.MiSamplerExtParams(L.ptr(self.t_map), L.ptr(self.x0_prev))
        self.t_state = torch.zeros(1, dtype=torch.int32, device=dev)
        self.x0 = torch.empty(B, n, dtype=torch.float32, device=dev)
        self.hist = torch.zeros(3 * B * 2 * 2048, dtype=torch.int32, device=dev)
        self.s_q = torch.zeros(B, dtype=torch.float32, device=dev)
        self.v_q = torch.zeros(B, 2, dtype=torch.float32, device=dev)
        self.seed_dev = None
        self.graphs = {}
        self.group_err_host = None
        self.group_failed = self.group_heal = False

    def close(self, dev):
        _drain(dev)
        for entry in self.graphs.values():
            destroy_graph(entry, dev)
        self.graphs.clear()


def stage_state(ws, sched, B: int, n: int, solver=None, eng=None, max_states: int = 8, hw: int = None, objective: str = 'noise') -> StageState:
    store = ws.sampler_state
    key = sched.num_timesteps if solver is None else (sched.num_timesteps,) + tuple(solver)
    if objective != 'noise':
        key = (key if isinstance(key, tuple) else (key,)) + (objective,)
    if hw is not None:
        key = (key if isinstance(key, tuple) else (key,)) + ("inpaint",)
    bounded = isinstance(key, tuple)
    st = store.get(key)
    if st is not None and bounded:
        store[key] = store.pop(key)
    if st is None and bounded:
        solver_keys = [k for k in store if isinstance(k, tuple)]
        while len(solver_keys) >= max_states:
            old = store.pop(solver_keys.pop(0))
            old.close(ws.dev)
            if eng is not None:
                eng.drop_step_tables(ws, old.t_state)
    if st is None:
        st = store[key] = StageState(sched, B, n, ws.dev, solver, hw, objective)
    return st


def known_begin(st: StageState, ws, shape, inpaint, *, sched, known_noise, seed: int, sample0: int, stage: int, stream):
    lib = L.lib()
    images, masks, normalize = inpaint
    B, Cc, H, W = shape
    n = Cc * H * W
    at_size = cubic_resize(ws, images, H, stream)
    L.check(lib.mi_inpaint_prepare_fwd(L.ptr(at_size), L.ptr(st.known), B, n, 1 if normalize else 0, L.ptr(masks), masks.shape[1], masks.shape[2],
                                       L.ptr(st.mask), H, stream), "mi_inpaint_prepare_fwd")
    st.known_noise = known_noise
    st.ip = L.MiInpaintParams(L.ptr(st.known), L.ptr(st.mask), H * W, (stage << 20) | (3 << 18), L.ptr(known_noise))
    a, b = sched.known_start_coefs()
    L.check(lib.mi_inpaint_blend0_fwd(L.ptr(ws.x), B, n, C.byref(st.ip), a, b, int(seed) & 0x7FFFFFFFFFFFFFFF, sample0, stream), "mi_inpaint_blend0_fwd")


def stage_begin(unet, shape, *, noise_scheduler, ws, noise_fn=None, seed: int = 0, sample0: int = 0, stage: int = 0, solver=None, max_states: int = 8,
                inpaint=None, objective: str = 'noise'):
    lib, stream, eng = L.lib(), L.current_stream(), unet.engine()
    B, n = shape[0], shape[1] * shape[2] * shape[3]
    T = noise_scheduler.num_timesteps if solver is None else solver[0]
    st = stage_state(ws, noise_scheduler, B, n, solver, eng, max_states, hw=None if inpaint is None else shape[2] * shape[3], objective=objective)
    noise_dev = known_noise = None
    if noise_fn is not None:
        ws.x.copy_(noise_fn(shape))
        noise_dev = torch.stack([noise_fn(shape) for _ in range(T)]).to(ws.dev).contiguous()
        if inpaint is not None:
            known_noise = torch.stack([noise_fn(shape) for _ in range(T)]).to(ws.dev).contiguous()
    else:
        L.check(lib.mi_randn_fill(L.ptr(ws.x), B, n, seed, sample0, (stage << 20) | (1 << 19) | 1, stream), "mi_randn_fill")
    if inpaint is not None:
        known_begin(st, ws, shape, inpaint, sched=noise_scheduler, known_noise=known_noise, seed=seed, sample0=sample0, stage=stage, stream=stream)
    if st.t_map is None:
        L.check(lib.mi_step_set(L.ptr(st.t_state), L.ptr(ws.times), B, T - 1, stream), "mi_step_set")
    else:
        L.check(lib.mi_step_set_mapped(L.ptr(st.t_state), L.ptr(ws.times), B, T - 1, C.byref(st.ext), stream), "mi_step_set_mapped")
    if st.x0_prev is not None:
        st.x0_prev.zero_()
    eng.prepare_step_tables(ws, T, st.t_state, stream, t_map=st.tau)
    return st, noise_dev


def tail_launcher(st: StageState, ws, kind: str, cp, qp, pp, stream):
    lib, tails = L.lib(), {}
    ext, q_ = (C.byref(st.ext) if st.t_map is not None else None), C.byref(qp)
    state = (L.ptr(st.t_state), L.ptr(ws.times), cp.B)
    form, blocks = ("ext", (ext,)) if st.ip is None else ("inpaint", (ext, C.byref(st.ip)))
    small_fwd, group_fwd, posterior_fwd = (getattr(lib, f"mi_{name}_{form}_fwd") for name in ("sampler_step_small", "sampler_step_group", "posterior"))

    def params(k):
        if k not in tails:
            c_, p_ = L.MiCfgX0Params.from_buffer_copy(cp), L.MiPosteriorParams.from_buffer_copy(pp)
            c_.t_off = p_.t_off = k
            if kind != "separate":
                c_.x0 = c_.hist0 = 0
            tails[k] = (C.byref(c_), q_, C.byref(p_))
        return tails[k]

    def small(k=0):
        L.check(small_fwd(*params(k), *blocks, stream), f"mi_sampler_step_small_{form}_fwd")

    def group(k=0):
        L.check(group_fwd(*params(k), *blocks, L.ptr(st.group_sync), stream), f"mi_sampler_step_group_{form}_fwd")

    def separate(k=0):
        c_, _, p_ = params(k)
        L.check(lib.mi_cfg_x0_fwd(c_, stream), "mi_cfg_x0_fwd")
        L.check(lib.mi_quantile_fwd(q_, stream), "mi_quantile_fwd")
        L.check(posterior_fwd(p_, *blocks, stream), f"mi_posterior_{form}_fwd")

    if st.t_map is None:
        advance = lambda n=1: L.check(lib.mi_step_advance_by(*state, n, stream), "mi_step_advance_by")
    else:
        advance = lambda n=1: L.check(lib.mi_step_advance_by_mapped(*state, n, ext, stream), "mi_step_advance_by_mapped")
    return dict(small=small, group=group, separate=separate)[kind], advance


def p_sample_loop(im, unet, shape, *, noise_scheduler, ws, cond_scale: float, noise_fn=None, seed: int = 0, sample0: int = 0,
                  stage: int = 0, use_graph: bool = True, begun=None, solver=None, group_max: int = 8, max_states: int = 8, inpaint=None,
                  objective: str = 'noise'):
    lib, stream, eng = L.lib(), L.current_stream(), unet.engine()
    B, Cc, H, W = shape
    n = Cc * H * W
    T = noise_scheduler.num_timesteps if solver is None else solver[0]
    two = ws.B2 != ws.B
    if begun is None:
        begun = stage_begin(unet, shape, noise_scheduler=noise_scheduler, ws=ws, noise_fn=noise_fn, seed=seed, sample0=sample0, stage=stage, solver=solver, max_states=max_states,
                            inpaint=inpaint, objective=objective)
    st, noise_dev = begun
    k_lo, k_hi, w = quantile_rank(n, im.dynamic_thresholding_percentile)
    fused = os.environ.get("MINIMAGEN_SAMPLER_FUSED", "1") != "0"
    grouped = fused and 0 < lib.mi_sampler_group_size(n) <= group_max and not st.group_failed
    kind = "small" if (fused and n <= 16384) else "group" if grouped else "separate"
    group = kind == "group"
    if st.group_heal:
        st.group_sync.zero_()
        st.group_heal = False
    gkey = (float(cond_scale), two, k_lo, k_hi, w, sample0, stage, T, noise_dev is None, group) + (() if solver is None else (tuple(solver),)) + (() if st.ip is None else ("inpaint",))
    entry = st.graphs.get(gkey) if (use_graph and noise_dev is None) else None
    seed = int(seed) & 0x7FFFFFFFFFFFFFFF
    if noise_dev is None:
        if st.seed_dev is None:
            st.seed_dev = torch.zeros(1, dtype=torch.int64, device=ws.dev)
        st.seed_dev.fill_(seed)
    if entry is None:
        cp = L.MiCfgX0Params(B, n, L.ptr(ws.pred), 1 if two else 0, float(cond_scale), L.ptr(ws.x), L.ptr(st.coef), L.ptr(st.t_state), 0, L.ptr(st.x0), L.ptr(st.hist))
        qp = L.MiQuantileParams(B, n, L.ptr(st.x0), k_lo, k_hi, w, L.ptr(st.hist), L.ptr(st.s_q), L.ptr(st.v_q), 1, 1)
        pp = L.MiPosteriorParams(B, n, T, L.ptr(st.x0), L.ptr(st.s_q), L.ptr(ws.x), L.ptr(st.coef), L.ptr(st.t_state),
                                 L.ptr(noise_dev), seed, sample0, stage << 20, L.ptr(st.seed_dev) if noise_dev is None else 0)
        if group and st.group_err_host is None:
            st.group_sync = torch.zeros(lib.mi_sampler_group_sync_bytes(B, n), dtype=torch.uint8, device=ws.dev)
            st.group_err_host = torch.zeros(1, dtype=torch.int32).pin_memory() if L.backend() == "hip-gfx950" else torch.zeros(1, dtype=torch.int32)
        launch, advance = tail_launcher(st, ws, kind, cp, qp, pp, stream)

        def one_step(k=0, by=1):
            eng.run_step(ws, stream, t_off=k)
            launch(k)
            if by:
                advance(by)
        cap = int(os.environ.get("MINIMAGEN_STEPS_PER_GRAPH", "5"))
        per = next(k for k in (5, 4, 3, 2, 1) if k <= cap and T % k == 0)
        entry = dict(step=one_step, graph=None, per=per)
        if use_graph:
            offsets = eng.step_offsets_supported(ws)
            L.check(lib.mi_graph_begin(stream), "mi_graph_begin")
            try:
                for k in range(per):
                    one_step(k, per if k == per - 1 else 0) if offsets else one_step()
            finally:
                g = C.c_void_p()
                rc = lib.mi_graph_end(stream, C.byref(g))
            L.check(rc, "mi_graph_end")
            entry["graph"] = g
            if noise_dev is None:
                while len(st.graphs) >= 8:
                    destroy_graph(st.graphs.pop(next(iter(st.graphs))), ws.dev)
                st.graphs[gkey] = entry
    if use_graph:
        try:
            for _ in range(T // entry["per"]):
                L.check(lib.mi_graph_launch(entry["graph"], stream), "mi_graph_launch")
        finally:
            if noise_dev is not None:
                destroy_graph(entry, ws.dev)
    else:
        for _ in range(T):
            entry["step"]()
    img = torch.empty(shape, dtype=torch.float32, device=ws.dev)
    L.check(lib.mi_finalize_images(L.ptr(ws.x), L.ptr(img), B * n, 1 if im.auto_normalize_img else 0, stream), "mi_finalize_images")
    if group:
        st.group_err_host.copy_(st.group_sync[8:12].view(torch.int32), non_blocking=True)
        im._status_stages.append((st, stage, (B, H, W)))
    return img
```

Measured before the change: 53200 denoising-steps/s.

## Fold classifier-free guidance combine into final resnet block conv

```diff
diff --git a/include/minimagen_hip.h b/include/minimagen_hip.h
--- a/include/minimagen_hip.h
+++ b/include/minimagen_hip.h
@@ -42,6 +42,7 @@
     const float* gn_gamma;
     const float* gn_beta;
     float gn_eps;
+    int ss_row1;
     const float* scale_shift;
     int ss_stride, ss_off;
     mi_act res0, res1;
diff --git a/minimagen_amd/_lib.py b/minimagen_amd/_lib.py
--- a/minimagen_amd/_lib.py
+++ b/minimagen_amd/_lib.py
@@ -22,7 +22,7 @@
         ("in0", MiAct), ("in1", MiAct),
         ("Cout", C.c_int), ("ksize", C.c_int), ("stride", C.c_int), ("up2", C.c_int),
         ("w", C.c_void_p), ("bias", C.c_void_p),
-        ("gn_groups", C.c_int), ("gn_gamma", C.c_void_p), ("gn_beta", C.c_void_p), ("gn_eps", C.c_float),
+        ("gn_groups", C.c_int), ("gn_gamma", C.c_void_p), ("gn_beta", C.c_void_p), ("gn_eps", C.c_float), ("ss_row1", C.c_int),
         ("scale_shift", C.c_void_p), ("ss_stride", C.c_int), ("ss_off", C.c_int),
         ("res0", MiAct), ("res1", MiAct), ("res_w", C.c_void_p), ("res_b", C.c_void_p),
         ("out", C.c_void_p), ("out_st", C.c_int), ("out_stats", C.c_void_p), ("tile_cfg", C.c_int),
diff --git a/minimagen_amd/csrc/conv.hip b/minimagen_amd/csrc/conv.hip
--- a/minimagen_amd/csrc/conv.hip
+++ b/minimagen_amd/csrc/conv.hip
@@ -420,6 +420,9 @@
     const int Cin = p.in0.C + (p.in1.data ? p.in1.C : 0);
     const bool any16 = p.in0.st || (p.in1.data && p.in1.st) || (p.res0.data && p.res0.st) || (p.res1.data && p.res1.st) || p.out_st;
     if (any16 && !(p.w_rp && (p.tile_cfg & 0x400))) { mi_set_error("mi_conv_fwd: bf16 activation storage is read / written by the single-term row-paired kernels only (w_rp, tile_cfg | 0x400)"); return MI_ERR_UNSUPPORTED; }
+    if (((p.res0.data && p.res1.data && !p.res_w) || p.ss_row1) && !(p.w_rp && (p.tile_cfg & 0xff) == 12)) {
+        mi_set_error("mi_conv_fwd: the weighted two-source identity residual and ss_row1 are read by the stripe kernel only (tile_cfg 12)"); return MI_ERR_UNSUPPORTED;
+    }
     if (p.w_rp) {
         if (p.gn_groups > MI_MAX_GROUPS || (p.gn_groups > 0 && (Cin % p.gn_groups) != 0)) { mi_set_error("mi_conv_fwd: Cin %d / groups %d", Cin, p.gn_groups); return MI_ERR_INVALID; }
         if (p.gn_groups > 0 && (!p.in0.stats || (p.in1.data && !p.in1.stats))) { mi_set_error("mi_conv_fwd: GroupNorm input without channel statistics"); return MI_ERR_INVALID; }
diff --git a/minimagen_amd/csrc/conv_stripe.hip b/minimagen_amd/csrc/conv_stripe.hip
--- a/minimagen_amd/csrc/conv_stripe.hip
+++ b/minimagen_amd/csrc/conv_stripe.hip
@@ -61,7 +61,8 @@
     static constexpr int WPE = ((RO > 0 && W_ == 128) || LDG == 2) ? 4 : 1;
     static constexpr bool PHS = HS && 2 * NPR * QPR * KO <= NCW * 64;
     static constexpr int PCH = PHS ? 4 : 8, PU = NPR * QPR * KO * (PHS ? 2 : 1);
-    static_assert(PU <= NCW * 64, "the MFMA waves transform the first four rows in one pass");
+    static constexpr int PPASS = (PU + NCW * 64 - 1) / (NCW * 64);
+    static_assert(PPASS == 1 || (W_ == 256 && KO_ == 2 && PPASS == 2), "the MFMA waves transform the first four rows in one pass");
     static_assert(!DS || (LA > 0 && !GN_ && RO_ == 0 && W_ <= 128), "the stride-2 member is a plain conv, at most 128 output columns");
 };
 
@@ -304,9 +305,11 @@
             const int c = lane < Cin ? lane : 0;
             pg = p.gn_gamma[c];
             pb = p.gn_beta[c];
-            const float* ss = p.scale_shift ? p.scale_shift + (size_t)b * p.ss_stride + p.ss_off : p.gn_gamma;
-            ld_s1 = ss[p.scale_shift ? c : 0];
-            ld_s2 = ss[p.scale_shift ? Cin + c : 0];
+            const bool split = p.scale_shift && p.ss_row1 != 0, second = split && c >= C0;
+            const int cs = second ? c - C0 : c, nsh = split ? (second ? C1 : C0) : Cin;
+            const float* ss = p.scale_shift ? p.scale_shift + ((long long)b + (second ? p.ss_row1 : 0)) * p.ss_stride + p.ss_off : p.gn_gamma;
+            ld_s1 = ss[p.scale_shift ? cs : 0];
+            ld_s2 = ss[p.scale_shift ? nsh + cs : 0];
         }
 #pragma unroll
         for (int jt = 0; jt < NJ; ++jt) {
@@ -330,17 +333,21 @@
             }
         }
         constexpr int PCH = CFG::PCH, PHM = CFG::PHS ? 2 : 1;
-        const bool plive = ct < PU;
-        const int pu = plive ? ct : 0;
-        const int poct = pu / (NPR * QPR * PHM), phalf = PHM == 2 ? (pu / (NPR * QPR)) & 1 : 0, prow = (pu / QPR) % NPR, pq = pu % QPR;
-        f32x4 praw[PCH];
-        const int py = ys0 - 1 + prow;
-        const bool pin = py >= 0 && py < Hs;
-        {
-            const mi_gptr<const float> pbase = octet_base(poct) + (size_t)(PCH * phalf) * HWs;
-            const unsigned off = pin ? (unsigned)(py * WS + 4 * pq) : 0u;
-#pragma unroll
-            for (int j = 0; j < PCH; ++j) praw[j] = *reinterpret_cast<mi_gptr<const f32x4>>(pbase + (size_t)j * HWs + off);
+        constexpr int PPASS = CFG::PPASS;
+        bool plive[PPASS], pin[PPASS];
+        int poct[PPASS], phalf[PPASS], prow[PPASS], pq[PPASS];
+        f32x4 praw[PPASS][PCH];
+#pragma unroll
+        for (int ps = 0; ps < PPASS; ++ps) {
+            plive[ps] = ct + ps * NCT < PU;
+            const int pu = plive[ps] ? ct + ps * NCT : 0;
+            poct[ps] = pu / (NPR * QPR * PHM); phalf[ps] = PHM == 2 ? (pu / (NPR * QPR)) & 1 : 0; prow[ps] = (pu / QPR) % NPR; pq[ps] = pu % QPR;
+            const int py = ys0 - 1 + prow[ps];
+            pin[ps] = py >= 0 && py < Hs;
+            const mi_gptr<const float> pbase = octet_base(poct[ps]) + (size_t)(PCH * phalf[ps]) * HWs;
+            const unsigned off = pin[ps] ? (unsigned)(py * WS + 4 * pq[ps]) : 0u;
+#pragma unroll
+            for (int j = 0; j < PCH; ++j) praw[ps][j] = *reinterpret_cast<mi_gptr<const f32x4>>(pbase + (size_t)j * HWs + off);
         }
         for (int k = ct; k < KO * RING * 2; k += NCT) {
             const int r = k >> 1, c = DS ? ((k & 1) ? WS / 2 + 1 : PWH) : ((k & 1) ? WS + 1 : 0);
@@ -436,11 +443,12 @@
         if (cw == 0) ST_STAMP(4);
         __syncthreads();
         if (cw == 0) ST_STAMP(5);
-        {
+#pragma unroll
+        for (int ps = 0; ps < PPASS; ++ps) {
             float4 PP[PCH];
 #pragma unroll
-            for (int j = 0; j < PCH; ++j) PP[j] = chP[8 * poct + PCH * phalf + j];
-            transform_quad(std::integral_constant<int, PCH>{}, praw, PP, pin, plive, poct, phalf, prow, pq);
+            for (int j = 0; j < PCH; ++j) PP[j] = chP[8 * poct[ps] + PCH * phalf[ps] + j];
+            transform_quad(std::integral_constant<int, PCH>{}, praw[ps], PP, pin[ps], plive[ps], poct[ps], phalf[ps], prow[ps], pq[ps]);
         }
 
         float bvv[NJ];
@@ -452,12 +460,13 @@
         }
         const int perm = ((lg & 1) << 1) | (lg >> 1);
         const int dy = DS ? 0 : lq >> 3;
-        constexpr bool idres = CFG::OM == 1, MASKC = CFG::OM == 2 || DS;
+        constexpr bool idres2 = CFG::OM == 5, idres = CFG::OM == 1 || idres2, MASKC = CFG::OM == 2 || DS;
         const mi_gptr<float> obuf = mi_global(p.out + (size_t)b * p.Cout * HW);
         const mi_gptr<const float> rbuf = mi_global(idres ? p.res0.data + (size_t)mi_row_of(b, p.res0.bmod) * p.res0.C * HW : p.out);
         const float unscale = ldexpf(1.0f, -sExp[2]);
-        const float rs = idres ? p.res0.scale : 0.0f;
-        f32x4 rv[2][idres ? GPW : 1][idres ? NJ : 1];
+        const mi_gptr<const float> rbuf1 = mi_global(idres2 ? p.res1.data + (size_t)mi_row_of(b, p.res1.bmod) * p.res1.C * HW : p.out);
+        const float rs = idres ? p.res0.scale : 0.0f, rs1 = idres2 ? p.res1.scale : 0.0f;
+        f32x4 rv[2][idres ? GPW : 1][idres ? NJ : 1], rv1[2][idres2 ? GPW : 1][idres2 ? NJ : 1];
         auto issue_res = [&](int it, auto buf_tag) {
             constexpr int buf = decltype(buf_tag)::value;
             if constexpr (idres) {
@@ -469,6 +478,7 @@
                         const int co = 8 * jt + (lq & 7);
                         const int oy = y0 + 2 * itc + dy, ox = 16 * (cw * GPW + g) + 4 * lg;
                         rv[buf][g][jt] = *reinterpret_cast<mi_gptr<const f32x4>>(rbuf + (unsigned)(co * HW + oy * W + ox));
+                        if constexpr (idres2) rv1[buf][g][jt] = *reinterpret_cast<mi_gptr<const f32x4>>(rbuf1 + (unsigned)(co * HW + oy * W + ox));
                     }
             }
         };
@@ -618,6 +628,7 @@
                     y[0] = fmaf(acc[g][jt][0], unscale, bv); y[1] = fmaf(acc[g][jt][1], unscale, bv);
                     y[2] = fmaf(acc[g][jt][2], unscale, bv); y[3] = fmaf(acc[g][jt][3], unscale, bv);
                     if constexpr (idres) { const f32x4 r = rv[buf][g][jt]; y[0] = fmaf(r[0], rs, y[0]); y[1] = fmaf(r[1], rs, y[1]); y[2] = fmaf(r[2], rs, y[2]); y[3] = fmaf(r[3], rs, y[3]); }
+                    if constexpr (idres2) { const f32x4 r = rv1[buf][g][jt]; y[0] = fmaf(r[0], rs1, y[0]); y[1] = fmaf(r[1], rs1, y[1]); y[2] = fmaf(r[2], rs1, y[2]); y[3] = fmaf(r[3], rs1, y[3]); }
                     yv[g] = y;
                 }
                 if (first_of_block) {
@@ -701,7 +712,7 @@
 
 template <int W>
 int launch_stripe_w(const mi_conv_params& p, hipStream_t st, int ko, int nj, bool gn) {
-    const int om = p.ksize == 4 ? 4 : (p.up2 ? 3 : (p.Cout < 8 * nj ? 2 : ((p.res0.data && !p.res_w) ? 1 : 0)));
+    const int om = p.ksize == 4 ? 4 : (p.up2 ? 3 : (p.Cout < 8 * nj ? 2 : ((p.res0.data && !p.res_w) ? (p.res1.data ? 5 : 1) : 0)));
 #define ST_BLOCK(KO, NJ) if (gn && ko == KO && nj == NJ) return om == 1 ? launch_stripe<W, KO, NJ, true, 1>(p, st) : launch_stripe<W, KO, NJ, true, 0>(p, st)
 #define ST_PLAIN(KO, NJ, OMV) if (!gn && ko == KO && nj == NJ && om == OMV) return launch_stripe<W, KO, NJ, false, OMV>(p, st)
     if constexpr (W == 64 || W == 128) {
@@ -709,6 +720,9 @@
     }
     if constexpr (W == 64) {
         if (gn && ko == 2 && nj == 2 && om == 0 && p.res0.data && p.res_w) return launch_stripe<W, 2, 2, true, 0, 4>(p, st);
+    }
+    if constexpr (W == 64 || W == 256) {
+        if (gn && ko == 2 && nj == 1 && om == 5) return launch_stripe<W, 2, 1, true, 5>(p, st);
     }
     if (om <= 1) {
         ST_BLOCK(1, 1);
@@ -740,6 +754,9 @@
         const bool m8 = cres == 16 && C0 + C1 == 8 && p.Cout == 8 && (p.W == 64 || p.W == 128), m16 = ST_RO4 && cres == 32 && C0 + C1 == 16 && p.Cout == 16 && p.W == 64;
         if (!p.res_w_rp || (p.res0.C & 7) || (p.res1.data && (p.res1.C & 7)) || (p.res1.data && p.res1.st) || !(m8 || m16) || !p.gn_groups || p.up2) return 0;
     } else if (p.res0.data && p.res0.C != p.Cout) return 0;
+    const bool res2 = p.res0.data && p.res1.data && !p.res_w;
+    if (res2 && (p.res1.C != p.Cout || p.res1.st || C0 != 8 || C1 != 8 || p.Cout != 8 || !p.gn_groups || p.up2 || ds || !(p.W == 64 || p.W == 256))) return 0;
+    if (p.ss_row1 && !p.in1.data) return 0;
     if (p.gn_groups > MI_MAX_GROUPS || (p.gn_groups > 0 && ((C0 + C1) % p.gn_groups))) return 0;
     if (p.gn_groups > 0 && (!p.in0.stats || (p.in1.data && !p.in1.stats))) return 0;
     const int ko = (C0 + C1) >> 3, nj = ds ? (p.Cout + 15) >> 4 : (p.Cout + 7) >> 3;
@@ -749,14 +766,14 @@
         if (ko_) { *ko_ = ko; *nj_ = nj; }
         return sr0;
     }
-    const int om = p.up2 ? 3 : (p.Cout < 8 * nj ? 2 : ((p.res0.data && !rconv) ? 1 : 0));
+    const int om = p.up2 ? 3 : (p.Cout < 8 * nj ? 2 : ((p.res0.data && !rconv) ? (res2 ? 5 : 1) : 0));
     if (om == 3) {
         if (gn || p.res0.data || nj != 1 || p.Cout != 8 || ko > 2 || p.W < 64 || p.W > 128 || (p.H & 1)) return 0;
         if (ko_) { *ko_ = ko; *nj_ = nj; }
         return sr0;
     }
     if ((om == 1 && !gn) || (om == 2 && (gn || nj != 1))) return 0;
-    const bool common = (ko == 1 && nj == 1) || (p.W <= 128 && ko == 2 && nj == 1 && gn);
+    const bool common = (ko == 1 && nj == 1) || (p.W <= 128 && ko == 2 && nj == 1 && gn && om != 5) || (ko == 2 && nj == 1 && gn && om == 5);
     const bool small = p.W <= 64 && ((ko == 2 && nj == 2 && gn) || (ko == 4 && nj == 2 && gn) || (ko == 1 && nj == 2 && !gn) || (ko == 3 && nj == 2 && gn));
     if (!common && !small) return 0;
     if (ko_) { *ko_ = ko; *nj_ = nj; }
diff --git a/minimagen_amd/engine.py b/minimagen_amd/engine.py
--- a/minimagen_amd/engine.py
+++ b/minimagen_amd/engine.py
@@ -21,6 +21,7 @@
 CE_MFMA = os.environ.get("MINIMAGEN_CE_MFMA", "1") != "0"
 ATTN_COND = os.environ.get("MINIMAGEN_ATTN_COND", "1") != "0"
 INIT_DOWN = os.environ.get("MINIMAGEN_INIT_DOWN", "1") != "0"
+CFG_FOLD = int(os.environ.get("MINIMAGEN_CFG_FOLD", "1"))
 CONV_REVERSE = int(os.environ.get("MINIMAGEN_CONV_REVERSE", "1"))
 RP_NTILE = int(os.environ.get("MINIMAGEN_RP_NTILE", "0"))
 RP_NTILE_BY = {k: int(os.environ.get("MINIMAGEN_RP_NTILE_" + k, "0")) for k in ("L", "M", "S")}
@@ -43,6 +44,11 @@
     @property
     def st(self) -> int:
         return 1 if self.t.dtype == torch.bfloat16 else 0
+
+    def rows(self, lo: int, n: int) -> "Act":
+        a = Act(self.t[lo:lo + n], None if self.stats is None else self.stats[lo:lo + n], self.nt, self.C, self.H, self.W, n)
+        a.rev = self.rev
+        return a
 
     def c(self, consumer_batch: int, scale: float = 1.0) -> L.MiAct:
         bmod = self.batch if self.batch != consumer_batch else 0
@@ -450,12 +456,7 @@
             if not nt_knob and ws.pipelined and RP_NTILE_PIPE[cls] and batch * nt // RP_NTILE_PIPE[cls] >= 256:
                 nt_knob = RP_NTILE_PIPE[cls]
             if stripe:
-                nt_knob = ST_NBLK[cls]
-                if ws.pipelined and ST_NBLK_PIPE[cls] and nt % ST_NBLK_PIPE[cls] == 0 and batch * nt // ST_NBLK_PIPE[cls] >= 128 \
-                        and self.unet.lowres_cond:
-                    nt_knob = ST_NBLK_PIPE[cls]
-                if nt_knob and (nt % nt_knob or nt_knob > 15):
-                    nt_knob = 0
+                nt_knob = self._stripe_nblk(ws, cls, nt, batch)
             p.tile_cfg |= (nt_knob & 0xf) << 12
             frags = pk.conv_ig if gemm else pk.conv_rp
             frag, p.w_rp_exp = frags[id(wpack)]
@@ -471,7 +472,73 @@
         ws.prog.append((lib.mi_conv_fwd, p, "conv"))
         return out
 
-    def _emit_resnet(self, ws, pk, rb: ResnetBlock, in0: Act, in1: Optional[Act]) -> Act:
+    def _stripe_nblk(self, ws, cls, nt, batch) -> int:
+        nt_knob = ST_NBLK[cls]
+        if ws.pipelined and ST_NBLK_PIPE[cls] and nt % ST_NBLK_PIPE[cls] == 0 and batch * nt // ST_NBLK_PIPE[cls] >= 128 \
+                and self.unet.lowres_cond:
+            nt_knob = ST_NBLK_PIPE[cls]
+        if nt_knob and (nt % nt_knob or nt_knob > 15):
+            nt_knob = 0
+        return nt_knob
+
+    def _cfg_fold_rows(self, ws, rb: ResnetBlock, x: Act) -> int:
+        u = self.unet
+        if not CFG_FOLD or ws.B2 != 2 * ws.B or ws.half or u.init_conv_to_final_conv_residual or rb.cross_attn is not None \
+                or isinstance(rb.res_conv, nn.Conv2d) or x.batch != ws.B2 or (CFG_FOLD < 2 and x.H * x.W <= 128 * 128):
+            return 0
+        cls = "L" if x.H * x.W > 128 * 128 else ("M" if x.H * x.W > 64 * 64 else "S")
+        Cout = rb.block2.project.out_channels
+        if not CONV_RP or cls not in CONV_STRIPE or Cout != rb.block2.project.in_channels or Cout != x.C:
+            return 0
+        half = x.rows(0, ws.B)
+        return self._stripe_rows(ws.B, x.H, x.W, half, half, Cout, SimpleNamespace(num_groups=2 * rb.block2.groupnorm.num_groups), (half, half, None, None))
+
+    def _emit_cfg_fold(self, ws, pk, rb: ResnetBlock, h: Act, x: Act, rows: int) -> Act:
+        lib, B = L.lib(), ws.B
+        conv, gn = rb.block2.project, rb.block2.groupnorm
+        Cout, H, W = conv.out_channels, h.H, h.W
+        nt = H // rows
+        out = self._new_act(ws, B, Cout, H, W, nt)
+        if not hasattr(pk, "cfg_fold_gn"):
+            pk.cfg_fold_gn = (torch.cat((gn.weight.detach(), gn.weight.detach())).contiguous(), torch.cat((gn.bias.detach(), gn.bias.detach())).contiguous())
+            pk.cfg_fold_w = {}
+        p = L.MiConvParams()
+        p.B, p.H, p.W = B, H, W
+        p.in0, p.in1 = h.rows(B, B).c(B), h.rows(0, B).c(B)
+        p.Cout, p.ksize, p.stride, p.up2 = Cout, 3, 1, 0
+        p.bias = L.ptr(conv.bias)
+        p.gn_groups, p.gn_gamma, p.gn_beta, p.gn_eps = 2 * gn.num_groups, L.ptr(pk.cfg_fold_gn[0]), L.ptr(pk.cfg_fold_gn[1]), gn.eps
+        ss_off = pk.ss_off.get(id(rb))
+        if ss_off is not None:
+            p.scale_shift, p.ss_stride, p.ss_off, p.ss_row1 = L.ptr(ws.ss[B:]), ws.ss.shape[1], ss_off, -B
+        p.res0, p.res1 = x.rows(B, B).c(B), x.rows(0, B).c(B)
+        cls = "L" if H * W > 128 * 128 else ("M" if H * W > 64 * 64 else "S")
+        p.out, p.out_stats, p.tile_cfg = L.ptr(out.t), L.ptr(out.stats), 12 | 0x100 | ((self._stripe_nblk(ws, cls, nt, B) & 0xf) << 12)
+        out.rev = bool(CONV_REVERSE) and B % 8 == 0 and not h.rev
+        if out.rev:
+            p.tile_cfg |= 0x200
+        ws.cfg_fold = SimpleNamespace(p=p, conv=conv, scale=None)
+        self.set_guidance(ws, 1.0)
+        ws.prog.append((lib.mi_conv_fwd, p, "conv"))
+        return out
+
+    def set_guidance(self, ws, cond_scale: float):
+        fold = getattr(ws, "cfg_fold", None)
+        s = float(cond_scale)
+        if fold is None or fold.scale == s:
+            return
+        pk = self.packed()
+        ent = pk.cfg_fold_w.get(s)
+        if ent is None:
+            while len(pk.cfg_fold_w) >= 16:
+                pk.cfg_fold_w.pop(next(iter(pk.cfg_fold_w)))
+            ent = pk.cfg_fold_w[s] = P.pack_conv_weight_rp(P.compose_cfg_fold(fold.conv.weight, s))
+        p = fold.p
+        p.w_rp, p.w_rp_exp = L.ptr(ent[0]), ent[1]
+        p.res0.scale, p.res1.scale = 1.0 - s, s
+        fold.scale, fold.keep = s, ent
+
+    def _emit_resnet(self, ws, pk, rb: ResnetBlock, in0: Act, in1: Optional[Act], cfg_fold_rows: int = 0) -> Act:
         u = self.unet
         s = u.skip_connect_scale
         Cout = rb.block1.project.out_channels
@@ -480,6 +547,8 @@
                             gn=rb.block1.groupnorm, want_stats=not has_cross, skip_scale=s)
         if has_cross:
             h = self._emit_cross_attn(ws, pk, rb.cross_attn.fn, h)
+        if cfg_fold_rows and h.batch == ws.B2:
+            return self._emit_cfg_fold(ws, pk, rb, h, in0, cfg_fold_rows)
         ss_off = pk.ss_off.get(id(rb))
         if isinstance(rb.res_conv, nn.Conv2d):
             res = (in0, in1, pk.conv[id(rb.res_conv)], rb.res_conv.bias)
@@ -823,9 +892,10 @@
             if isinstance(upsample, nn.Sequential):
                 cv = upsample[1]
                 cur = self._emit_conv(ws, pk, cur, None, wpack=pk.conv[id(cv)], bias=cv.bias, Cout=cv.out_channels, up2=1)
-        cur = self._emit_resnet(ws, pk, u.final_res_block, cur, None)
+        ws.cfg_fold = None
+        cur = self._emit_resnet(ws, pk, u.final_res_block, cur, None, cfg_fold_rows=self._cfg_fold_rows(ws, u.final_res_block, cur))
         out = self._emit_conv(ws, pk, cur, None, wpack=pk.conv[id(u.final_conv)], bias=u.final_conv.bias, Cout=u.channels_out,
-                              want_stats=False, conditioned=True, out_fp32=True)
+                              want_stats=False, conditioned=ws.cfg_fold is None, out_fp32=True)
         ws.pred = out.t
         if (out.H, out.W) != (H, W):
             raise L.MinImagenHipError(f"U-Net output is {out.H}x{out.W} for a {H}x{W} input (image size must be divisible by the down-sampling factor)")
@@ -998,8 +1068,10 @@
         if two:
             keep = torch.cat((torch.ones(B, dtype=torch.bool), torch.zeros(B, dtype=torch.bool)))
         self.set_text(ws, text_embeds, text_mask, keep)
+        if two:
+            self.set_guidance(ws, cond_scale)
         self.run(ws)
-        if not two:
+        if not two or ws.cfg_fold is not None:
             return ws.pred.clone()
         out = torch.empty(B, u.channels_out, H, W, dtype=torch.float32, device=ws.dev)
         p = L.MiCfgX0Params(B, u.channels_out * H * W, L.ptr(ws.pred), 1, float(cond_scale), 0, 0, 0, L.ptr(out), 0)
diff --git a/minimagen_amd/packing.py b/minimagen_amd/packing.py
--- a/minimagen_amd/packing.py
+++ b/minimagen_amd/packing.py
@@ -52,6 +52,12 @@
 def rp_weight_exponent(mx: float) -> int:
     exp = 0 if (mx == 0.0 or not math.isfinite(mx)) else 7 - math.floor(math.log2(mx))
     return max(-100, min(100, exp))
+
+
+def compose_cfg_fold(w2: torch.Tensor, cond_scale: float) -> torch.Tensor:
+    w = w2.detach().double()
+    s = float(cond_scale)
+    return torch.cat(((1.0 - s) * w, s * w), 1).contiguous()
 
 
 def pack_conv_weight_rp(w: torch.Tensor, exp=None):
diff --git a/minimagen_amd/sampler.py b/minimagen_amd/sampler.py
--- a/minimagen_amd/sampler.py
+++ b/minimagen_amd/sampler.py
@@ -183,6 +183,8 @@
     n = Cc * H * W
     T = noise_scheduler.num_timesteps if solver is None else solver[0]
     two = ws.B2 != ws.B
+    eng.set_guidance(ws, cond_scale)
+    combine = two and ws.cfg_fold is None
     if begun is None:
         begun = stage_begin(unet, shape, noise_scheduler=noise_scheduler, ws=ws, noise_fn=noise_fn, seed=seed, sample0=sample0, stage=stage, solver=solver, max_states=max_states,
                             inpaint=inpaint, objective=objective)
@@ -203,7 +205,7 @@
             st.seed_dev = torch.zeros(1, dtype=torch.int64, device=ws.dev)
         st.seed_dev.fill_(seed)
     if entry is None:
-        cp = L.MiCfgX0Params(B, n, L.ptr(ws.pred), 1 if two else 0, float(cond_scale), L.ptr(ws.x), L.ptr(st.coef), L.ptr(st.t_state), 0, L.ptr(st.x0), L.ptr(st.hist))
+        cp = L.MiCfgX0Params(B, n, L.ptr(ws.pred), 1 if combine else 0, float(cond_scale), L.ptr(ws.x), L.ptr(st.coef), L.ptr(st.t_state), 0, L.ptr(st.x0), L.ptr(st.hist))
         qp = L.MiQuantileParams(B, n, L.ptr(st.x0), k_lo, k_hi, w, L.ptr(st.hist), L.ptr(st.s_q), L.ptr(st.v_q), 1, 1)
         pp = L.MiPosteriorParams(B, n, T, L.ptr(st.x0), L.ptr(st.s_q), L.ptr(ws.x), L.ptr(st.coef), L.ptr(st.t_state),
                                  L.ptr(noise_dev), seed, sample0, stage << 20, L.ptr(st.seed_dev) if noise_dev is None else 0)
```

Result: faster. 53960 denoising-steps/s (median of 6 runs) (+1.4%).
